# KushalChaudhari-16/Medical-Image-Denoising-Using-Diffusion

Measured on AMD Instinct MI355X. Metric: denoised images/sec, 256x256 x50 DDIM steps, higher is better.
Workload: dtype f32 (split-fp16 x3 MFMA, fp32 accumulate); 1 GPU; batch=8/GPU 256x256 grayscale, 50-iteration reverse loop (noise_steps=50, inference_steps=50), random-init 12.8M-param UNet (BASELINE.json configs[1]); batch_per_gpu=8, global_batch=8, parallelism=single, collective=none

## Files before the change

include/midd.h:

```cpp
#ifndef MIDD_H
#define MIDD_H

#include <stddef.h>
#include <stdint.h>

#ifdef __cplusplus
extern "C" {
#endif

#define MI_OK            0
#define MI_EINVAL       -1
#define MI_ESTATE       -2
#define MI_EHIP         -3
#define MI_ENOMEM       -4
#define MI_ERANGE       -5

#define MI_STATUS_NONFINITE   1
#define MI_STATUS_FP16_RANGE  2

#define MI_MAX_LEVELS    8

#define MI_VARIANT_DDIM  0
#define MI_VARIANT_CDDPM 1

#define MI_COMPUTE_F32   0
#define MI_COMPUTE_F16X3 1
#define MI_COMPUTE_F16   2
#define MI_COMPUTE_BATCH_INVARIANT 0x100

#define MI_CLAMP_EPS     1
#define MI_NO_SPLIT      2

typedef struct mi_plan mi_plan;

typedef struct mi_unet_cfg {
    int32_t in_channels;
    int32_t model_channels;
    int32_t num_levels;
    int32_t channel_mult[MI_MAX_LEVELS];
    int32_t num_res_blocks;
    int32_t num_attention_levels;
    int32_t attention_levels[MI_MAX_LEVELS];
    int32_t time_emb_dim;
    int32_t variant;
    int32_t compute_mode;
} mi_unet_cfg;

int mi_unet_plan_create(const mi_unet_cfg* cfg, mi_plan** out);

int mi_unet_load_weights(mi_plan* plan, const char* key, const float* data,
                         const int64_t* shape, int ndim);

int mi_unet_num_weights(const mi_plan* plan);
const char* mi_unet_weight_name(const mi_plan* plan, int index);

int mi_unet_finalize(mi_plan* plan, int time_rows);

size_t mi_workspace_bytes(mi_plan* plan, int B, int H, int W);

int mi_unet_forward(mi_plan* plan, const float* x, const float* condition, const int32_t* t,
                    float* eps, int B, int H, int W,
                    void* workspace, size_t workspace_bytes, void* stream);

int mi_denoise(mi_plan* plan, const float* noisy, float* x_out, int B, int H, int W,
               const int32_t* t_list, int n_iters,
               const float* beta, const float* alpha, const float* alpha_hat, int noise_steps,
               const float* step_noise, int flags,
               void* workspace, size_t workspace_bytes, void* stream);

int mi_denoise_seeded(mi_plan* plan, const float* noisy, float* x_out, int B, int H, int W,
                      const int32_t* t_list, int n_iters,
                      const float* beta, const float* alpha, const float* alpha_hat, int noise_steps,
                      uint64_t seed, int64_t sample_offset, int flags,
                      void* workspace, size_t workspace_bytes, void* stream);

int mi_denoise_slots(mi_plan* plan, const float* cond, float* x, int B, int H, int W,
                     const int32_t* t_rows, int n_rows, const int32_t* iter_base, const int64_t* sample_index,
                     const float* beta, const float* alpha, const float* alpha_hat, int noise_steps,
                     const float* step_noise, int seeded, uint64_t seed, int flags,
                     void* workspace, size_t workspace_bytes, void* stream);

int mi_denoise_slots_virtual(mi_plan* plan, const float* cond, float* x, int B, int H, int W,
                             const int32_t* t_rows, int n_rows, const int32_t* iter_base, const int64_t* sample_index,
                             const int64_t* member, const uint32_t* frame,
                             const float* beta, const float* alpha, const float* alpha_hat, int noise_steps,
                             const float* step_noise, int seeded, uint64_t seed, int flags,
                             void* workspace, size_t workspace_bytes, void* stream);

int mi_step_noise_fill(float* dst, int n_iters, int B, int C, int H, int W,
                       uint64_t seed, int64_t sample_offset, void* stream);
int mi_step_noise_fill_member(float* dst, int n_iters, int B, int C, int H, int W,
                              uint64_t seed, int64_t sample_offset, int64_t member, void* stream);

int mi_denoise_ensemble(mi_plan* plan, const float* noisy, float* mean_out, float* std_out, float* samples_out,
                        int B, int members, int H, int W,
                        const int32_t* t_list, int n_iters,
                        const float* beta, const float* alpha, const float* alpha_hat, int noise_steps,
                        uint64_t seed, int64_t sample_offset, int64_t member_offset, int pass_samples, int flags,
                        void* workspace, size_t workspace_bytes, void* stream);

size_t mi_ensemble_workspace_bytes(mi_plan* plan, int B, int members, int H, int W, int pass_samples, int samples_external);

int mi_ensemble_reduce(const float* samples, int B, int members, int64_t chw, float* mean_out, float* std_out, void* stream);

int mi_ensemble_quantiles(const float* samples, int B, int members, int64_t chw,
                          const double* q, int nq, float* out, void* stream);

size_t mi_ensemble_scores_workspace_bytes(int B, int members, int64_t chw);
int mi_ensemble_scores(const float* samples, const float* truth, int B, int members, int64_t chw,
                       const double* q, int nq,
                       double* sums, uint64_t* invalid, uint64_t* rank_hist, uint64_t* counts, float* crps_map,
                       void* workspace, size_t workspace_bytes, void* stream);

#define MI_NPS_DETREND_NONE  0
#define MI_NPS_DETREND_MEAN  1
#define MI_NPS_DETREND_PLANE 2
#define MI_NPS_EXCLUDE_AXES  1
size_t mi_noise_power_spectrum_workspace_bytes(int B, int K, int C, int H, int W, int roi, int step);
int mi_noise_power_spectrum(const float* a, const float* b, int B, int K, int C, int H, int W, int roi, int step, int detrend,
                            const float* window, double scale, int flags,
                            double* nps, double* radial, int64_t* radial_count, int64_t* rois_used, int64_t* rois_skipped,
                            void* workspace, size_t workspace_bytes, void* stream);

int mi_tile_geometry(int L, int T, int O, int* n, int* origins, int cap);

int mi_tile_extract(const float* noisy, int B, int C, int H, int W, int th, int tw, int oy, int ox, int v0, int n,
                    float* dst, void* stream);

int mi_tile_blend(const float* tiles, int B, int C, int H, int W, int th, int tw, int oy, int ox, float* out, void* stream);

int mi_denoise_tiled(mi_plan* plan, const float* noisy, float* image_out, float* tiles_out,
                     int B, int H, int W, int th, int tw, int oy, int ox,
                     const int32_t* t_list, int n_iters,
                     const float* beta, const float* alpha, const float* alpha_hat, int noise_steps,
                     int seeded, uint64_t seed, int64_t sample_offset, int pass_samples, int flags,
                     void* workspace, size_t workspace_bytes, void* stream);

size_t mi_tiled_workspace_bytes(mi_plan* plan, int B, int H, int W, int th, int tw, int oy, int ox, int pass_samples, int tiles_external);

int mi_denoise_tiled_ensemble(mi_plan* plan, const float* noisy, float* mean_out, float* std_out, float* samples_out, float* tiles_out,
                              int B, int members, int H, int W, int th, int tw, int oy, int ox,
                              const int32_t* t_list, int n_iters,
                              const float* beta, const float* alpha, const float* alpha_hat, int noise_steps,
                              uint64_t seed, int64_t sample_offset, int64_t member_offset, int pass_samples, int flags,
                              void* workspace, size_t workspace_bytes, void* stream);

size_t mi_tiled_ensemble_workspace_bytes(mi_plan* plan, int B, int members, int H, int W, int th, int tw, int oy, int ox,
                                         int pass_samples, int tiles_external);

int mi_tile_blend_reduce(const float* tiles, int B, int members, int C, int H, int W, int th, int tw, int oy, int ox,
                         float* mean_out, float* std_out, float* samples_out, void* stream);

int mi_tile_blend_quantiles(const float* tiles, int B, int members, int C, int H, int W, int th, int tw, int oy, int ox,
                            const double* q, int nq, float* out, void* stream);

int mi_dihedral_views(const float* images, int B, int C, int H, int W, const int32_t* views, int n_views,
                      int v0, int n, float* dst, void* stream);
int mi_dihedral_reduce(const float* views_out, int B, int C, int H, int W, const int32_t* views, int n_views,
                       float* mean_out, float* std_out, float* samples_out, void* stream);
int mi_dihedral_quantiles(const float* views_out, int B, int C, int H, int W, const int32_t* views, int n_views,
                          const double* q, int nq, float* out, void* stream);

int mi_denoise_self_ensemble(mi_plan* plan, const float* noisy, float* mean_out, float* std_out, float* samples_out,
                             int B, int H, int W, const int32_t* views, int n_views,
                             const int32_t* t_list, int n_iters,
                             const float* beta, const float* alpha, const float* alpha_hat, int noise_steps,
                             int seeded, uint64_t seed, int64_t sample_offset, int64_t member_offset, int pass_samples, int flags,
                             void* workspace, size_t workspace_bytes, void* stream);

size_t mi_self_ensemble_workspace_bytes(mi_plan* plan, int B, int n_views, int H, int W, int pass_samples, int samples_external);

#define MI_UPDATE_REFERENCE 0
#define MI_UPDATE_DDIM      1
typedef struct mi_update_rule {
    int32_t kind;
    double  eta;
    int32_t clip_x0;
} mi_update_rule;

int mi_ddim_coefficients(const int32_t* t_list, int n_iters, const float* alpha_hat, int noise_steps, double eta, float* out);

int mi_denoise_rule(mi_plan* plan, const float* noisy, float* x_out, int B, int H, int W,
                    const int32_t* t_list, int n_iters,
                    const float* beta, const float* alpha, const float* alpha_hat, int noise_steps,
                    const float* step_noise, int seeded, uint64_t seed, int64_t sample_offset, int flags,
                    const mi_update_rule* rule, void* workspace, size_t workspace_bytes, void* stream);

int mi_denoise_ensemble_rule(mi_plan* plan, const float* noisy, float* mean_out, float* std_out, float* samples_out,
                             int B, int members, int H, int W,
                             const int32_t* t_list, int n_iters,
                             const float* beta, const float* alpha, const float* alpha_hat, int noise_steps,
                             uint64_t seed, int64_t sample_offset, int64_t member_offset, int pass_samples, int flags,
                             const mi_update_rule* rule, void* workspace, size_t workspace_bytes, void* stream);

int mi_denoise_tiled_rule(mi_plan* plan, const float* noisy, float* image_out, float* tiles_out,
                          int B, int H, int W, int th, int tw, int oy, int ox,
                          const int32_t* t_list, int n_iters,
                          const float* beta, const float* alpha, const float* alpha_hat, int noise_steps,
                          int seeded, uint64_t seed, int64_t sample_offset, int pass_samples, int flags,
                          const mi_update_rule* rule, void* workspace, size_t workspace_bytes, void* stream);

#define MI_UPDATE_DPMPP2M   2

int mi_dpm_coefficients(const int32_t* t_list, int n_iters, const float* alpha_hat, int noise_steps, float* out);

int mi_denoise_dpm(mi_plan* plan, const float* noisy, float* x_out, float* x0_buf, int x0_slots, int B, int H, int W,
                   const int32_t* t_list, int n_iters,
                   const float* beta, const float* alpha, const float* alpha_hat, int noise_steps,
                   int flags, int clip_x0, void* workspace, size_t workspace_bytes, void* stream);

int mi_denoise_tiled_dpm(mi_plan* plan, const float* noisy, float* image_out, float* tiles_out, float* x0_hist,
                         int B, int H, int W, int th, int tw, int oy, int ox,
                         const int32_t* t_list, int n_iters,
                         const float* beta, const float* alpha, const float* alpha_hat, int noise_steps,
                         int pass_samples, int flags, int clip_x0, void* workspace, size_t workspace_bytes, void* stream);

int mi_update_row(int32_t t_before, int32_t t, int32_t t_after, const float* alpha_hat, int noise_steps, double eta, float out[8]);

int mi_tile_blend_unview_reduce(const float* tiles, int B, int C, int H, int W, int th, int tw, int oy, int ox,
                                const int32_t* views, int n_views, float* mean_out, float* std_out, float* samples_out, void* stream);
int mi_tile_blend_unview_quantiles(const float* tiles, int B, int C, int H, int W, int th, int tw, int oy, int ox,
                                   const int32_t* views, int n_views, const double* q, int nq, float* out, void* stream);

int mi_denoise_tiled_self_ensemble(mi_plan* plan, const float* noisy, float* mean_out, float* std_out, float* samples_out, float* tiles_out,
                                   int B, int H, int W, int th, int tw, int oy, int ox, const int32_t* views, int n_views,
                                   const int32_t* t_list, int n_iters,
                                   const float* beta, const float* alpha, const float* alpha_hat, int noise_steps,
                                   int seeded, uint64_t seed, int64_t sample_offset, int64_t member_offset, int pass_samples, int flags,
                                   const mi_update_rule* rule, void* workspace, size_t workspace_bytes, void* stream);

size_t mi_tiled_self_ensemble_workspace_bytes(mi_plan* plan, int B, int n_views, int H, int W, int th, int tw, int oy, int ox,
                                              int pass_samples, int tiles_external);

int mi_denoise_slots_rule(mi_plan* plan, const float* cond, float* x, int B, int H, int W,
                          const int32_t* t_rows, int n_rows, const int32_t* iter_base, const int64_t* sample_index,
                          const int64_t* member, const uint32_t* frame,
                          const int32_t* t_before, const int32_t* t_after, float* x0_hist,
                          const float* beta, const float* alpha, const float* alpha_hat, int noise_steps,
                          const float* step_noise, int seeded, uint64_t seed, int flags,
                          const mi_update_rule* rule, void* workspace, size_t workspace_bytes, void* stream);

int mi_status(const void* workspace, void* stream, int* flags);

int mi_debug_fetch(mi_plan* plan, const char* module_name, int B, int H, int W,
                   const void* workspace, float* dst, int* C, int* h, int* w, void* stream);

int mi_debug_attention_split(int N, int B, int* ksplit, int* tiles_per_split);

int mi_debug_plan_dump(mi_plan* plan, int B, int H, int W, int side_by_side, char* buf, size_t cap);

int mi_debug_conv16_geometry(int ks, int stride, int tw, int mt, int nt, int wm, int wn, int cb,
                             int* ring, int* ppw, int* apw, int* lds_bytes);
int mi_debug_conv16_geometry_planes(int ks, int stride, int tw, int mt, int nt, int wm, int wn, int cb, int planes,
                                    int* ring, int* ppw, int* apw, int* lds_bytes);
int mi_debug_conv16_steps(int Cin, int ks, int cb);

const char* mi_source_hash(void);

typedef struct mi_profile_entry {
    char   name[128];
    int64_t launches;
    double total_ms;
    double flops;
    double bytes;
} mi_profile_entry;
int mi_profile_begin(mi_plan* plan);
int mi_profile_end(mi_plan* plan, mi_profile_entry* out, int max_entries, int* n_entries);

int mi_noise_images(const float* clean, const int32_t* t, const float* alpha_hat, int noise_steps,
                    const float* eps, int seeded, uint64_t seed, int64_t sample_offset, int64_t draw,
                    const int64_t* sample_index, const int64_t* draws,
                    float* x_t, float* eps_out, int B, int C, int H, int W, void* stream);
size_t mi_loss_workspace_bytes(int B, int C, int H, int W);
int mi_loss_terms(const float* clean, const float* x_t, const float* eps, const float* eps_pred,
                  const int32_t* t, const float* alpha_hat, int noise_steps,
                  int seeded, uint64_t seed, int64_t sample_offset, int64_t draw,
                  const int64_t* sample_index, const int64_t* draws, int flags, double edge_weight,
                  double* out, float* maps, int B, int C, int H, int W,
                  void* workspace, size_t workspace_bytes, void* stream);
size_t mi_denoising_loss_workspace_bytes(mi_plan* plan, int B, int H, int W);
int mi_denoising_loss(mi_plan* plan, const float* clean, const float* cond, const int32_t* t,
                      const float* alpha_hat, int noise_steps,
                      const float* eps, int seeded, uint64_t seed, int64_t sample_offset, int64_t draw,
                      const int64_t* sample_index, const int64_t* draws, int flags, double edge_weight,
                      double* out, float* maps, int B, int H, int W,
                      void* workspace, size_t workspace_bytes, void* stream);

void mi_plan_destroy(mi_plan* plan);

size_t mi_resize_workspace_bytes(int n, int sw, int sh, int dw, int dh);
int mi_resize_bicubic_u8(const void* src_u8, int n, int sw, int sh, void* dst_u8, int dw, int dh,
                         void* workspace, size_t workspace_bytes, void* stream);
int mi_u8_to_unit_f32(const void* src_u8, void* dst_f32, size_t count, void* stream);
int mi_unit_f32_to_u8(const void* src_f32, void* dst_u8, size_t count, void* stream);
size_t mi_metrics_workspace_bytes(int n, int h);
int mi_image_metrics(const void* target_f32, const void* pred_f32, int n, int h, int w, void* out_f64,
                     void* workspace, size_t workspace_bytes, void* stream);

#define MI_PIX_U8  0
#define MI_PIX_U16 1
#define MI_PIX_F32 2
size_t mi_resize_f32_workspace_bytes(int n, int sw, int sh, int dw, int dh);
int mi_resize_bicubic_f32(const void* src, int src_type, int n, int sw, int sh,
                          void* dst, int dst_type, int dw, int dh, int clamp01,
                          void* workspace, size_t workspace_bytes, void* stream);
int mi_u16_to_unit_f32(const uint16_t* src, float* dst, size_t count, void* stream);
int mi_unit_f32_to_u16(const float* src, uint16_t* dst, size_t count, void* stream);

int mi_histogram_u16(const uint16_t* src, int n, size_t count, uint32_t* hist, void* stream);
int mi_window_levels(const uint32_t* hist, int n, double p_lo, double p_hi, int32_t* levels, void* stream);
int mi_window_u16_to_f32(const uint16_t* src, const int32_t* levels, int n, size_t count, float* dst, void* stream);
int mi_window_f32_to_u16(const float* src, const int32_t* levels, int n, size_t count, uint16_t* dst, void* stream);
int mi_resize_bicubic_f32_window(const void* src, int src_type, int n, int sw, int sh,
                                 void* dst, int dst_type, int dw, int dh, int clamp01, const int32_t* levels,
                                 void* workspace, size_t workspace_bytes, void* stream);

const char* mi_last_error(void);

const char* mi_version(void);

#ifdef __cplusplus
}
#endif
#endif
```

medical-image-denoising-using-diffusion_amd/csrc/conv_mfma_f16x3.hip:

```cpp
#include "f16x3_common.h"
#include <cstdlib>
#include <type_traits>
#ifdef MIDD_CONV_TIMING
#include <cstdio>
#include <cstring>
#include <string>
#include <vector>
#endif

namespace midd {

#ifndef MIDD_LDS_TARGET_KB
#define MIDD_LDS_TARGET_KB 52
#endif
#ifndef MIDD_RING_MAX
#define MIDD_RING_MAX 6
#endif
#ifndef MIDD_LDS_WIDE_KB
#define MIDD_LDS_WIDE_KB 78
#endif
struct Conv16Tile {
    int ks, stride, tw, mt, nt, wm, wn;
    int cbt = 0;
    int pl = 2;
    int nw = wm * wn;
    int nthreads = nw * 64;
    int th = wm * mt * 16 / tw;
    int ih = (th - 1) * stride + ks;
    int iw = (tw - 1) * stride + ks;
    int npix = ih * iw;
    int cb = cbt ? cbt : conv16_cb(ks);
    int qpp = 4 * cb;
    int nslot = npix * qpp;
    int apw = (nslot + nthreads - 1) / nthreads;
    int raw_bytes = apw * nthreads * 16;
    int plane = npix * 32;
    int img_bytes = pl * cb * plane;
    int wpieces = wn * nt * pl;
    int ppw = (wpieces + nw - 1) / nw;
    int wslice = wpieces * 1024;
    int stat_floats = nw * 2 * nt * 16;
    int add_floats = wn * nt * 16;
    static constexpr int NOMINAL_CIN = 384;
    int fixed_bytes = raw_bytes + img_bytes + (stat_floats + add_floats) * 4 + 2 * NOMINAL_CIN * 4 + 64;
    int lds_target = (stride == 2 ? 120 : (ks == 3 && cb == 2) ? MIDD_LDS_WIDE_KB : MIDD_LDS_TARGET_KB) * 1024;
    int ring_fit = (lds_target - fixed_bytes) / wslice;
    int ring = ring_fit < 2 ? 2 : (ring_fit > MIDD_RING_MAX ? MIDD_RING_MAX : ring_fit);
    int lds_nominal = fixed_bytes + ring * wslice;
    bool fits = lds_nominal <= 160 * 1024 && (ring - 2) * ppw + apw <= 60;
    constexpr int lds_bytes(int cin) const { return lds_nominal + 2 * (cin - NOMINAL_CIN) * 4; }
};

template <int KS, int STRIDE, int TW, int MT, int NT, int WM, int WN, int CBT = 0, int PL = 2>
struct Conv16Geom {
    static constexpr Conv16Tile g{KS, STRIDE, TW, MT, NT, WM, WN, CBT, PL};
    static constexpr int NW = g.nw, NTHREADS = g.nthreads, TH = g.th, IH = g.ih, IW = g.iw, CB = g.cb, QPP = g.qpp, NSLOT = g.nslot, APW = g.apw;
    static constexpr int RAW_BYTES = g.raw_bytes, PLANE = g.plane, IMG_BYTES = g.img_bytes, WPIECES = g.wpieces, PPW = g.ppw, WSLICE = g.wslice;
    static constexpr int STAT_FLOATS = g.stat_floats, ADD_FLOATS = g.add_floats, RING = g.ring;
    static_assert((WM * MT * 16) % TW == 0, "tile");
};

#ifdef MIDD_CONV_TIMING
enum { TS_WAIT, TS_ISSUE, TS_MFMA, TS_CHUNK_WAIT, TS_TRANSFORM, TS_EPILOGUE, TS_PROLOGUE, TS_FIRSTWAIT, TS_DMAWAIT, TS_RES, TS_PUBLISH, TS_TOTAL, TS_REAL, TS_WGS, TS_N };
__device__ unsigned long long g_conv_timing[64][TS_N];
__device__ __forceinline__ unsigned long long ts_stamp() {
    unsigned long long t;
    __builtin_amdgcn_sched_barrier(0);
    asm volatile("s_memtime %0\n\ts_waitcnt lgkmcnt(0)" : "=s"(t)::"memory");
    __builtin_amdgcn_sched_barrier(0);
    return t;
}
#define TS_DECL bool ts_after_epi = false; unsigned long long ts_acc[TS_N] = {}; unsigned long long ts_last = ts_stamp(); const unsigned long long ts_t0 = ts_last; const unsigned long long ts_r0 = __builtin_amdgcn_s_memrealtime();
#define TS(k) { const unsigned long long t_ = ts_stamp(); ts_acc[k] += t_ - ts_last; ts_last = t_; }
#else
#define TS_DECL
#define TS(k)
#endif

#ifndef MIDD_CONV16_WAVES_PER_SIMD
#define MIDD_CONV16_WAVES_PER_SIMD 3
#endif
#ifndef MIDD_RES_MT2_WAVES
#define MIDD_RES_MT2_WAVES 2
#endif
#define MIDD_CONV16_BOUNDS __launch_bounds__(WM * WN * 64, (WM * WN == 4 && STRIDE == 1) ? (CBT == 2 ? 2 : (RES && MT == 2) ? MIDD_RES_MT2_WAVES : MIDD_CONV16_WAVES_PER_SIMD) : 1)
#define MIDD_CONV16_KERNEL conv_mfma_f16x3_kernel
#define MIDD_CONV16_PL 2
#include "conv_mfma_f16x3_body.h"
#undef MIDD_CONV16_KERNEL
#undef MIDD_CONV16_PL
#define MIDD_CONV16_KERNEL conv_mfma_f16_kernel
#define MIDD_CONV16_PL 1
#include "conv_mfma_f16x3_body.h"
#undef MIDD_CONV16_KERNEL
#undef MIDD_CONV16_PL

#ifdef MIDD_CONV_TIMING
static std::vector<std::string> g_timing_names;
static int conv_timing_slot(int ks, int st, int tw, int mt, int nt, int wm, int wn, int oh, int cin, int cout, int B, int ring, int wgs) {
    char buf[160];
    snprintf(buf, sizeof buf, "k%d s%d tile(%d,%d,%d,%d,%d) ring%d out%d^2 %d->%d B%d wgs%d", ks, st, tw, mt, nt, wm, wn, ring, oh, cin, cout, B, wgs);
    for (size_t i = 0; i < g_timing_names.size(); ++i) if (g_timing_names[i] == buf) return (int)i;
    if (g_timing_names.size() >= 63) return 63;
    g_timing_names.push_back(buf);
    return (int)g_timing_names.size() - 1;
}
extern "C" __attribute__((visibility("default"))) void mi_debug_conv_timing_dump(void) {
    static unsigned long long h[64][TS_N];
    (void)hipDeviceSynchronize();
    (void)hipMemcpyFromSymbol(h, HIP_SYMBOL(g_conv_timing), sizeof h);
    static const char* names[] = {"barrier", "dma-issue", "frag+mfma", "chunk-wait", "transform", "epilogue", "prologue", "wait-after-epi", "dma-wait", "res-phase", "publish"};
    for (size_t i = 0; i < g_timing_names.size(); ++i) {
        const double tot = (double)h[i][TS_TOTAL], wgs = (double)h[i][TS_WGS];
        if (wgs == 0) continue;
        printf("%-70s cyc/wg %9.0f clk %.2f GHz |", g_timing_names[i].c_str(), tot / wgs, tot / (double)h[i][TS_REAL] * 0.1);
        for (int k = 0; k < 11; ++k) printf(" %s %4.1f%%", names[k], 100.0 * (double)h[i][k] / tot);
        printf("\n");
    }
    memset(h, 0, sizeof h);
    (void)hipMemcpyToSymbol(HIP_SYMBOL(g_conv_timing), h, sizeof h);
    fflush(stdout);
}
#endif
template <int KS, int STRIDE, int TW, int MT, int NT, int WM, int WN, bool RES, int CBT = 0, int PL = 2>
static hipError_t launch16(const ConvArgs& a0, hipStream_t s) {
    using G = Conv16Geom<KS, STRIDE, TW, MT, NT, WM, WN, CBT, PL>;
    ConvArgs a = a0;
    a.tiles_x = (a.OW + TW - 1) / TW;
    a.tiles_y = (a.OH + G::TH - 1) / G::TH;
    const int ny = a.Cout / (WN * NT * 16);
    a.wgs_per_img = conv16_wgs_per_img(a.tiles_x * a.tiles_y, a.B, ny, a.persist_wgs);
    dim3 grid(a.B * a.wgs_per_img, ny);
#ifdef MIDD_CONV_TIMING
    a.dbg_slot = conv_timing_slot(KS, STRIDE, TW, MT * 10 + G::CB, NT, WM, WN, a.OH, a.C0 + a.C1, a.Cout, a.B, G::RING, (int)grid.x * (int)grid.y);
#endif
    if constexpr (G::g.fits) {
        const int lds_bytes = G::g.lds_bytes(a.C0 + a.C1);
        if (lds_bytes > 160 * 1024) return hipErrorInvalidValue;
        {
            static int raised[MIDD_MAX_DEVICES] = {};
            hipError_t e = ensure_dynamic_lds(PL == 2 ? reinterpret_cast<const void*>(&conv_mfma_f16x3_kernel<KS, STRIDE, TW, MT, NT, WM, WN, RES, CBT>)
                                                      : reinterpret_cast<const void*>(&conv_mfma_f16_kernel<KS, STRIDE, TW, MT, NT, WM, WN, RES, CBT>), lds_bytes, raised);
            if (e != hipSuccess) return e;
        }
        if ((double)a.H * a.W * 64.0 >= 4294967296.0) return hipErrorInvalidValue;
        if constexpr (PL == 2) hipLaunchKernelGGL((conv_mfma_f16x3_kernel<KS, STRIDE, TW, MT, NT, WM, WN, RES, CBT>), grid, dim3(G::NTHREADS), lds_bytes, s, a);
        else hipLaunchKernelGGL((conv_mfma_f16_kernel<KS, STRIDE, TW, MT, NT, WM, WN, RES, CBT>), grid, dim3(G::NTHREADS), lds_bytes, s, a);
        return hipGetLastError();
    } else {
        return hipErrorInvalidValue;
    }
}

int conv16_wgs_per_img(int tiles, int B, int ny, int target) {
    const int target_wgs = target ? target : 768;
    int per_img = target_wgs / (B * ny);
    if (per_img < 1) per_img = 1;
    if (per_img > tiles) per_img = tiles;
    const int tiles_per_wg = (tiles + per_img - 1) / per_img;
    return (tiles + tiles_per_wg - 1) / tiles_per_wg;
}

#define MIDD_CONV16_TILES(X)                  \
                        \
    X(16, 2, 3, 4, 1) X(16, 1, 3, 4, 1) X(8, 1, 3, 2, 1) \
    X(16, 2, 3, 2, 2) X(16, 1, 3, 2, 2) X(8, 1, 3, 1, 2) \
    X(16, 2, 3, 1, 3) X(8, 1, 3, 1, 3)                   \
    X(16, 2, 3, 1, 4) X(8, 2, 3, 1, 4) X(8, 1, 3, 1, 4)  \
    X(16, 2, 2, 4, 1) X(8, 1, 2, 2, 1)                   \
    X(16, 2, 2, 2, 2) X(8, 1, 2, 1, 2)                   \
    X(16, 2, 1, 4, 1) X(8, 1, 1, 2, 1)

struct Tile16 { int tw, mt, nt, wm, wn; };
static const Tile16 kTiles16[] = {
#define X(tw, mt, nt, wm, wn) {tw, mt, nt, wm, wn},
    MIDD_CONV16_TILES(X)
#undef X
};

#define X(tw, mt, nt, wm, wn)                                                                                     \
    static_assert(Conv16Geom<3, 1, tw, mt, nt, wm, wn>::RING == Conv16Tile{3, 1, tw, mt, nt, wm, wn}.ring &&         \
                  Conv16Geom<3, 2, tw, mt, nt, wm, wn>::APW == Conv16Tile{3, 2, tw, mt, nt, wm, wn}.apw &&           \
                  Conv16Geom<1, 1, tw, mt, nt, wm, wn>::WSLICE == Conv16Tile{1, 1, tw, mt, nt, wm, wn}.wslice, "Conv16Geom");
MIDD_CONV16_TILES(X)
#undef X
#define X(tw, mt, nt, wm, wn)                                                                                                 \
    static_assert(Conv16Geom<3, 1, tw, mt, nt, wm, wn, 0, 1>::RING == Conv16Tile{3, 1, tw, mt, nt, wm, wn, 0, 1}.ring &&         \
                  Conv16Geom<3, 2, tw, mt, nt, wm, wn, 0, 1>::APW == Conv16Tile{3, 2, tw, mt, nt, wm, wn, 0, 1}.apw &&           \
                  Conv16Geom<1, 1, tw, mt, nt, wm, wn, 0, 1>::WSLICE * 2 == Conv16Tile{1, 1, tw, mt, nt, wm, wn}.wslice, "Conv16Geom, one plane");
MIDD_CONV16_TILES(X)
#undef X

static bool wide16_tile(const ConvTile& t) { return t.ks == 3 && t.stride == 1 && t.tw == 16 && t.nt == 3 && t.wm == 4 && t.wn == 1; }
#ifndef MIDD_WIDE_MAX_WGS
#define MIDD_WIDE_MAX_WGS 512
#endif
bool conv16_pick_tile(int Cin, int Cout, int B, int OH, int OW, int ks, int stride, ConvTile* t, bool allow_wide, int planes) {
    if (Cout % 16) return false;
    if (!((ks == 3 && (stride == 1 || stride == 2)) || (ks == 1 && stride == 1))) return false;
    if (ks == 1 && conv1x1_pick_tile(Cin, Cout, B, OH, OW, t)) { t->pl = planes; return true; }
    const int nt = (Cout % 48 == 0) ? 3 : (Cout % 32 == 0) ? 2 : 1;
    const Tile16* best = nullptr;
    long best_score = -(1L << 60), best_wgs = 0;
    constexpr long min_wgs = 192;
    for (const Tile16& d : kTiles16) {
        if (d.nt != nt) continue;
        const int nn_d = Cout / (16 * d.nt);
        if (nn_d % d.wn) continue;
        if (!Conv16Tile{ks, stride, d.tw, d.mt, d.nt, d.wm, d.wn, 0, planes}.fits) continue;
        const int bm = d.wm * d.mt * 16, th = bm / d.tw;
        const long tiles = (long)((OW + d.tw - 1) / d.tw) * ((OH + th - 1) / th);
        const long wgs = (long)B * tiles * (nn_d / d.wn);
        const long covered = tiles * d.tw * th;
        const bool wasteful = covered * 4 > (long)OH * OW * 5;
        const long share = (long)bm * 8 + d.wn;
        const long score = (wgs >= min_wgs ? 1000000 : wgs * (1000000 / min_wgs)) + share - (wasteful ? 500000 : 0);
        if (score > best_score) { best_score = score; best = &d; best_wgs = wgs; }
    }
    if (!best) return false;
    *t = ConvTile{ks, stride, best->tw, best->mt, best->nt, best->wm, best->wn, 0, planes};
    if (allow_wide && wide16_tile(*t) && Cin >= 32 &&
        best_wgs <= MIDD_WIDE_MAX_WGS && Conv16Tile{ks, stride, best->tw, best->mt, best->nt, best->wm, best->wn, 2, planes}.fits)
        t->cb = 2;
    return true;
}

bool conv16_launch_info(int Cin, int Cout, int B, int OH, int OW, const ConvTile& t, int persist_wgs, ConvLaunchInfo* o) {
    if (t.ks == 1 && t.tw == 0) return conv1x1_launch_info(Cin, Cout, B, OH, OW, t, persist_wgs, ATT_NONE, o);
    bool listed = false;
    if (t.cb == 2 ? wide16_tile(t) : ((t.ks == 3 && (t.stride == 1 || t.stride == 2)) || (t.ks == 1 && t.stride == 1)))
        for (const Tile16& d : kTiles16) listed = listed || (d.tw == t.tw && d.mt == t.mt && d.nt == t.nt && d.wm == t.wm && d.wn == t.wn);
    if (!listed) return false;
    if (t.pl != 1 && t.pl != 2) return false;
    const Conv16Tile g{t.ks, t.stride, t.tw, t.mt, t.nt, t.wm, t.wn, t.cb == 2 ? 2 : 0, t.pl};
    o->tiles_x = (OW + t.tw - 1) / t.tw; o->tiles_y = (OH + g.th - 1) / g.th;
    o->grid_y = Cout / (t.wn * t.nt * 16);
    o->wgs_per_img = conv16_wgs_per_img(o->tiles_x * o->tiles_y, B, o->grid_y, persist_wgs);
    o->grid_x = B * o->wgs_per_img;
    o->ring = g.ring; o->ppw = g.ppw; o->apw = g.apw; o->lds_bytes = g.lds_bytes(Cin);
    return true;
}

template <int PL>
static hipError_t conv16_dispatch(const ConvArgs& a, const ConvTile& t, hipStream_t s) {
    if (t.cb == 2) {
        if (!wide16_tile(t)) return hipErrorInvalidValue;
        if (t.mt == 2) return a.res_steps > 0 ? launch16<3, 1, 16, 2, 3, 4, 1, true, 2, PL>(a, s) : launch16<3, 1, 16, 2, 3, 4, 1, false, 2, PL>(a, s);
        if (t.mt == 1) return a.res_steps > 0 ? launch16<3, 1, 16, 1, 3, 4, 1, true, 2, PL>(a, s) : launch16<3, 1, 16, 1, 3, 4, 1, false, 2, PL>(a, s);
        return hipErrorInvalidValue;
    }
#define X(tw_, mt_, nt_, wm_, wn_)                                                            \
    if (t.tw == tw_ && t.mt == mt_ && t.nt == nt_ && t.wm == wm_ && t.wn == wn_) {           \
        if (t.ks == 3 && t.stride == 1 && a.res_steps > 0) return launch16<3, 1, tw_, mt_, nt_, wm_, wn_, true, 0, PL>(a, s); \
        if (t.ks == 3 && t.stride == 1) return launch16<3, 1, tw_, mt_, nt_, wm_, wn_, false, 0, PL>(a, s); \
        if (t.ks == 3 && t.stride == 2) return launch16<3, 2, tw_, mt_, nt_, wm_, wn_, false, 0, PL>(a, s); \
        if (t.ks == 1 && t.stride == 1) return launch16<1, 1, tw_, mt_, nt_, wm_, wn_, false, 0, PL>(a, s); \
    }
    MIDD_CONV16_TILES(X)
#undef X
    return hipErrorInvalidValue;
}

hipError_t conv16_launch(const ConvArgs& a, const ConvTile& t, hipStream_t s) {
    if (t.ks == 1 && t.tw == 0) return conv1x1_launch(a, t, s);
    if (t.pl == 2) return conv16_dispatch<2>(a, t, s);
    if (t.pl == 1) return conv16_dispatch<1>(a, t, s);
    return hipErrorInvalidValue;
}

}
```

medical-image-denoising-using-diffusion_amd/csrc/conv_mfma_f16x3_body.h:

```cpp
#if !defined(MIDD_CONV16_KERNEL) || !defined(MIDD_CONV16_PL)
#error "include from conv_mfma_f16x3.hip with MIDD_CONV16_KERNEL and MIDD_CONV16_PL defined"
#endif

template <int KS, int STRIDE, int TW, int MT, int NT, int WM, int WN, bool RES, int CBT>
__global__ MIDD_CONV16_BOUNDS void MIDD_CONV16_KERNEL(const ConvArgs a) {
    constexpr int PL = MIDD_CONV16_PL;
    static_assert(PL == 1 || PL == 2, "planes");
    using G = Conv16Geom<KS, STRIDE, TW, MT, NT, WM, WN, CBT, PL>;
    constexpr int NW = G::NW, NTHREADS = G::NTHREADS, TH = G::TH, IW = G::IW;
    constexpr int PAD = (KS == 3) ? 1 : 0;
    constexpr int NSLOT = G::NSLOT, APW = G::APW, PLANE = G::PLANE;
    constexpr int TAPS = KS * KS;
    constexpr int HSTEPS = (TAPS + 1) / 2;
    constexpr int PPW = G::PPW, WSLICE = G::WSLICE, RING = G::RING;

    extern __shared__ __attribute__((aligned(16))) char lds[];
    char* const raw = lds;
    char* const img = lds + G::RAW_BYTES;
    char* const wring = img + G::IMG_BYTES;
    float* const stat_lds = reinterpret_cast<float*>(wring + RING * WSLICE);
    float* const add_lds = stat_lds + G::STAT_FLOATS;
    float* const gnp = add_lds + G::ADD_FLOATS;

    const int tid = threadIdx.x;
    const int lane = tid & 63;
    const int wave = __builtin_amdgcn_readfirstlane(tid >> 6);
    const int wn = wave % WN;
    const int wm = wave / WN;
    const int p16 = lane & 15;
    const int kq = lane >> 4;

    const int tiles_per_img = a.tiles_x * a.tiles_y;
    const int b = blockIdx.x / a.wgs_per_img;
    int trem = blockIdx.x - b * a.wgs_per_img;
    int oy0 = (trem / a.tiles_x) * TH, ox0 = (trem % a.tiles_x) * TW;

    const int Cin = a.C0 + a.C1;
    const int nblk = Cin >> 4;
    constexpr int CB = G::CB, QPP = G::QPP;
    const int nchunks = (nblk + CB - 1) / CB;
    const int ntiles_total = a.Cout >> 4;
    const int ntile_wg = blockIdx.y * (WN * NT);
    const int res_steps = RES ? a.res_steps : 0;
    const int total_steps = conv16_num_steps(Cin, TAPS, G::CB) + res_steps;

    constexpr int WTILE = PL * 1024;
    const char* const wbase = reinterpret_cast<const char*>(a.wpack) + (size_t)ntile_wg * WTILE;
    const size_t wstep_bytes = (size_t)ntiles_total * WTILE;
    const int lane16 = lane * 16;
    int wr_step = 0, wr_slot = 0;
    const char* wr_src = wbase;
#ifdef MIDD_DMA_CHECK
    constexpr unsigned SENT_W = 0x7FFF7FFFu;
    constexpr unsigned SENT_A = 0x7FC0DEADu;
    unsigned dma_bad = 0;
    auto sent4 = [](unsigned v) { typedef unsigned u32x4_ __attribute__((ext_vector_type(4))); return __builtin_bit_cast(f32x4, (u32x4_){v, v, v, v}); };
    auto has_sent = [](const auto& q, unsigned v) {
        typedef unsigned u32x4_ __attribute__((ext_vector_type(4)));
        const u32x4_ u = __builtin_bit_cast(u32x4_, q);
        return (unsigned)((u[0] == v) | (u[1] == v) | (u[2] == v) | (u[3] == v));
    };
#endif
    auto issue_w = [&]() {
        char* slot = wring + wr_slot * WSLICE;
#ifdef MIDD_DMA_CHECK
#pragma unroll
        for (int i = 0; i < PPW; ++i) {
            int piece = (WM == 1) ? wave * PPW + i : wave + i * NW;
            if (piece >= G::WPIECES) piece -= G::WPIECES;
            if constexpr (PL == 1) piece %= G::WPIECES;
            lds_store_raw(slot + piece * 1024 + lane16, sent4(SENT_W));
        }
        asm volatile("s_waitcnt lgkmcnt(0)" ::: "memory");
#endif
#pragma unroll
        for (int i = 0; i < PPW; ++i) {
            int piece = (WM == 1) ? wave * PPW + i : wave + i * NW;
            if (piece >= G::WPIECES) piece -= G::WPIECES;
            if constexpr (PL == 1) piece %= G::WPIECES;
            dma16(wr_src + piece * 1024 + lane16, slot + piece * 1024);
        }
        ++wr_step; wr_src += wstep_bytes;
        if (wr_step == total_steps) { wr_step = 0; wr_src = wbase; }
        wr_slot = (wr_slot + 1 == RING) ? 0 : wr_slot + 1;
    };

    const int q8 = tid % QPP;
    const int sblk = q8 >> 2;
    int g_off[APW];
    bool tile_pad = true;
    auto set_tile = [&](int t) {
        const int iy0 = (t / a.tiles_x) * TH * STRIDE - PAD, ix0 = (t % a.tiles_x) * TW * STRIDE - PAD;
        tile_pad = iy0 < 0 || ix0 < 0 || iy0 + G::IH > a.H || ix0 + IW > a.W;
        int tid_ = tid;
        asm volatile("" : "+v"(tid_));
#pragma unroll
        for (int s = 0; s < APW; ++s) {
            const int slot = tid_ + s * NTHREADS;
            int off = -2;
            if (slot < NSLOT) {
                const int pix = slot / QPP;
                const int iy = pix / IW, ix = pix - iy * IW;
                const int gy = iy0 + iy, gx = ix0 + ix;
                off = (gy >= 0 && gy < a.H && gx >= 0 && gx < a.W) ? gy * a.W + gx : -1;
            }
            g_off[s] = off;
        }
    };
    set_tile(trem);
    auto issue_a = [&](int c) {
        const int blk = min(CB * c + sblk, nblk - 1);
        const float* src; int bsrc, nb;
        if ((blk << 4) < a.C0) { src = a.src0; bsrc = blk; nb = a.C0 >> 4; }
        else                   { src = a.src1; bsrc = blk - (a.C0 >> 4); nb = a.C1 >> 4; }
        const char* base = reinterpret_cast<const char*>(src) + ((size_t)(b * nb + bsrc) * (size_t)(a.H * a.W)) * 64 + (q8 & 3) * 16;
#ifdef MIDD_DMA_CHECK
#pragma unroll
        for (int s = 0; s < APW; ++s) lds_store_raw(raw + (wave + s * NW) * 1024 + lane16, sent4(SENT_A));
        asm volatile("s_waitcnt lgkmcnt(0)" ::: "memory");
#endif
#pragma unroll
        for (int s = 0; s < APW; ++s) {
            const unsigned byte_off = (unsigned)max(g_off[s], 0) * 64u;
            dma16(base + byte_off, raw + (wave + s * NW) * 1024);
        }
    };
    float rscale = RAW_PRESCALE;
    auto transform = [&](int c) {
        const int blk = CB * c + sblk;
        if (blk >= nblk) return;
        const int ch = (blk << 4) + (q8 & 3) * 4;
        f32x4 rq[APW];
#pragma unroll
        for (int s = 0; s < APW; ++s) rq[s] = *reinterpret_cast<const f32x4*>(raw + (tid + s * NTHREADS) * 16);
#ifdef MIDD_DMA_CHECK
#pragma unroll
        for (int s = 0; s < APW; ++s) dma_bad |= has_sent(rq[s], SENT_A);
#endif
        f32x4 sc = {rscale, rscale, rscale, rscale}, sh = {0.f, 0.f, 0.f, 0.f};
        if (a.prologue != PRO_RAW) {
            sc = *reinterpret_cast<const f32x4*>(gnp + ch);
            sh = *reinterpret_cast<const f32x4*>(gnp + Cin + ch);
        }
        char* base = img + sblk * PL * PLANE + (q8 & 3) * 8;
        typedef unsigned u32x2 __attribute__((ext_vector_type(2)));
        if (c == 0 && tile_pad) {
#pragma unroll
            for (int s = 0; s < APW; ++s) {
                const int slot = tid + s * NTHREADS;
                if (g_off[s] == -1) {
                    *reinterpret_cast<u32x2*>(base + (slot / QPP) * 32) = (u32x2){0u, 0u};
                    if constexpr (PL == 2) *reinterpret_cast<u32x2*>(base + PLANE + (slot / QPP) * 32) = (u32x2){0u, 0u};
                }
            }
        }
#pragma unroll
        for (int s = 0; s < APW; ++s) {
            const int slot = tid + s * NTHREADS;
            float v[4];
#pragma unroll
            for (int e = 0; e < 4; ++e) v[e] = __builtin_fmaf(rq[s][e], sc[e], sh[e]);
#if defined(C16_ABL) && C16_ABL == 4
            if (false) {
#else
            if (a.prologue == PRO_GN_SILU) {
#endif
#pragma unroll
                for (int e = 0; e < 4; ++e) {
                    const float d = __builtin_fmaf(__builtin_amdgcn_exp2f(v[e]), 1.0f / ACT_PRESCALE, 1.0f / ACT_PRESCALE);
                    v[e] = v[e] * __builtin_amdgcn_rcpf(d);
                }
            }
            unsigned h01, h23, l01, l23;
            planes_pair<PL>(v[0], v[1], h01, l01);
            planes_pair<PL>(v[2], v[3], h23, l23);
            if (g_off[s] >= 0) {
                const int pix = slot / QPP;
                *reinterpret_cast<u32x2*>(base + pix * 32) = (u32x2){h01, h23};
                if constexpr (PL == 2) *reinterpret_cast<u32x2*>(base + PLANE + pix * 32) = (u32x2){l01, l23};
            }
        }
    };

    int frag_base[MT];
#pragma unroll
    for (int mt = 0; mt < MT; ++mt) {
        const int pp = (wm * MT + mt) * 16 + p16;
        const int py = pp / TW, px = pp - py * TW;
        frag_base[mt] = ((py * STRIDE) * IW + px * STRIDE) * 32 + (kq & 1) * 16;
    }
    int frag_full[MT];
#pragma unroll
    for (int mt = 0; mt < MT; ++mt) frag_full[mt] = frag_base[mt] + (kq >> 1) * PL * PLANE;
    const int wfrag_off = (wn * NT) * WTILE + lane * 16;

    f32x4 acc[MT][NT];
#pragma unroll
    for (int mt = 0; mt < MT; ++mt)
#pragma unroll
        for (int nt = 0; nt < NT; ++nt) acc[mt][nt] = (f32x4){0.f, 0.f, 0.f, 0.f};

    constexpr int D = RING - 1;
    constexpr bool PAIR = conv16_pair_walk(TAPS, CB);
    static_assert(D <= 5, "the chunk-end wait has one arm per after = 1 .. 4 below D (MIDD_RING_MAX 6)");
    constexpr auto cmin = [](int x, int y) { return x < y ? x : y; };
    const int ntile0 = ntile_wg + wn * NT;
    TS_DECL
    issue_a(0);
#pragma unroll
    for (int i = 0; i < D; ++i) issue_w();
#if !(defined(C16_ABL) && C16_ABL == 6)
    if (a.prologue == PRO_GN || a.prologue == PRO_GN_SILU)
        gn_prologue_lds(a.gn_tot0, a.C0, a.gn_bs0, a.gn_tot1, a.C1, a.gn_bs1, a.stat_rep, a.gn_gamma, a.gn_beta, a.gn_eps, a.gn_inv_n, b,
                        (a.prologue == PRO_GN_SILU) ? SILU_ARG_FACTOR : ACT_PRESCALE, gnp, tid, NTHREADS, a.status);
#endif
    stat_word* const raw_acc = reinterpret_cast<stat_word*>(gnp);
    if (a.prologue == PRO_RAW && a.gn_tot0 != nullptr && wave == 0)
        raw_sumsq_lds(a.gn_tot0, a.C0, a.gn_bs0, a.gn_tot1, a.C1, a.gn_bs1, a.stat_rep, b, raw_acc, lane);
    stat_word* const res_acc = reinterpret_cast<stat_word*>(gnp + 2 * Cin);
    if (res_steps > 0 && a.res_tot0 != nullptr && wave == NW - 1)
        raw_sumsq_lds(a.res_tot0, a.res_C0, a.res_bs0, a.res_tot1, a.res_C1, a.res_bs1, a.stat_rep, b, res_acc, lane);
    {
        const int trow = (a.temb != nullptr) ? a.trow[b] : 0;
        for (int i = tid; i < G::ADD_FLOATS; i += NTHREADS) {
            const int co = ntile_wg * 16 + i;
            add_lds[i] = a.bias[co] + (a.temb != nullptr ? a.temb[(size_t)trow * a.temb_stride + co] : 0.f);
        }
    }
    wait_vm_and_barrier<0>();
    float oscale = a.out_scale;
    if (a.prologue == PRO_RAW) {
        rscale = a.raw_scale_fixed;
        if (a.gn_tot0 != nullptr) {
            bool bad;
            const int ex = __builtin_amdgcn_readfirstlane(raw_prescale_exp(raw_acc, &bad));
            rscale = pow2f(ex);
            if (bad && tid == 0 && a.status != nullptr) atomicOr(a.status, (int)STATUS_NONFINITE);
        }
        oscale = a.out_scale / rscale;
    }
    float res_in = 1.0f, res_rescale = 1.0f;
    if (res_steps > 0) {
        if (a.res_tot0 != nullptr) {
            bool bad;
            res_in = pow2f(__builtin_amdgcn_readfirstlane(raw_prescale_exp(res_acc, &bad)));
            if (bad && tid == 0 && a.status != nullptr) atomicOr(a.status, (int)STATUS_NONFINITE);
        }
        res_rescale = a.out_scale * res_in / a.res_scale;
        oscale = a.res_scale / res_in;
    }
    transform(0);
    if constexpr (WM == 1) {
        asm volatile("s_waitcnt lgkmcnt(0)" ::: "memory");
        __builtin_amdgcn_s_barrier();
        asm volatile("" ::: "memory");
    }

    TS(TS_PROLOGUE)
    int frag_next[MT], frag_wrap[MT];
#pragma unroll
    for (int mt = 0; mt < MT; ++mt) {
        frag_next[mt] = frag_base[mt] + (kq >> 1) * 32;
        frag_wrap[mt] = frag_base[mt] + (kq >> 1) * ((IW - KS + 1) * 32);
    }
    int rd_slot = 0;
    half8 xh[MT], xl[MT];
    auto load_x = [&](const int (&xo)[MT], int off) {
#pragma unroll
        for (int mt = 0; mt < MT; ++mt) {
            xh[mt] = *reinterpret_cast<const half8*>(img + xo[mt] + off);
            if constexpr (PL == 2) xl[mt] = *reinterpret_cast<const half8*>(img + xo[mt] + off + PLANE);
        }
    };
    auto tap_off = [](int t) { return ((t / KS) * IW + (t % KS)) * 32; };
    auto kill_x = [&]() {
        if constexpr (PAIR) {
#pragma unroll
            for (int mt = 0; mt < MT; ++mt) {
                asm volatile("" : "=v"(xh[mt]));
                if constexpr (PL == 2) asm volatile("" : "=v"(xl[mt]));
            }
        }
    };
    auto load_stash = [&]() {
        constexpr int T8 = (((TAPS - 1) / KS) * IW + (TAPS - 1) % KS) * 32;
        if constexpr (MT == 2) {
            const int so = (kq >> 1) ? frag_base[1] : frag_base[0];
            xh[0] = *reinterpret_cast<const half8*>(img + so + T8);
            if constexpr (PL == 2) xl[0] = *reinterpret_cast<const half8*>(img + so + T8 + PLANE);
        } else {
            load_x(frag_base, T8);
        }
    };
    auto unpack_stash = [&]() {
        if constexpr (MT == 2) {
            typedef unsigned u32x4_ __attribute__((ext_vector_type(4)));
            auto unpack = [](half8& lo, half8& hi) {
                u32x4_ a = __builtin_bit_cast(u32x4_, lo), b = __builtin_bit_cast(u32x4_, hi);
#pragma unroll
                for (int r = 0; r < 4; ++r) {
                    const auto sw = __builtin_amdgcn_permlane32_swap(a[r], b[r], false, false);
                    a[r] = sw[0]; b[r] = sw[1];
                }
                lo = __builtin_bit_cast(half8, a); hi = __builtin_bit_cast(half8, b);
            };
            unpack(xh[0], xh[1]);
            if constexpr (PL == 2) unpack(xl[0], xl[1]);
        }
    };
    auto mfma_step = [&]() {
        const char* wslot = wring + rd_slot * WSLICE + wfrag_off;
        rd_slot = (rd_slot + 1 == RING) ? 0 : rd_slot + 1;
        half8 wh[NT], wl[NT];
#pragma unroll
        for (int nt = 0; nt < NT; ++nt) {
            wh[nt] = *reinterpret_cast<const half8*>(wslot + nt * WTILE);
            if constexpr (PL == 2) wl[nt] = *reinterpret_cast<const half8*>(wslot + nt * WTILE + 1024);
        }
#ifdef MIDD_DMA_CHECK
#pragma unroll
        for (int nt = 0; nt < NT; ++nt) {
            dma_bad |= has_sent(wh[nt], SENT_W);
            if constexpr (PL == 2) dma_bad |= has_sent(wl[nt], SENT_W);
        }
#endif
#pragma unroll
        for (int mt = 0; mt < MT; ++mt)
#pragma unroll
            for (int nt = 0; nt < NT; ++nt)
                acc[mt][nt] = __builtin_amdgcn_mfma_f32_16x16x32_f16(wh[nt], xh[mt], acc[mt][nt], 0, 0, 0);
#if !(defined(C16_ABL) && C16_ABL == 8)
        if constexpr (PL == 2) {
#pragma unroll
            for (int mt = 0; mt < MT; ++mt)
#pragma unroll
                for (int nt = 0; nt < NT; ++nt)
                    acc[mt][nt] = __builtin_amdgcn_mfma_f32_16x16x32_f16(wh[nt], xl[mt], acc[mt][nt], 0, 0, 0);
#pragma unroll
            for (int mt = 0; mt < MT; ++mt)
#pragma unroll
                for (int nt = 0; nt < NT; ++nt)
                    acc[mt][nt] = __builtin_amdgcn_mfma_f32_16x16x32_f16(wl[nt], xh[mt], acc[mt][nt], 0, 0, 0);
        }
#endif
    };

    auto k_step = [&](auto with_a, auto merge, bool first, bool first_with_more, int next_chunk, const int (&xo)[MT], int xoff) {
        constexpr bool WITH_A = decltype(with_a)::value;
        constexpr bool MERGE = decltype(merge)::value;
        auto load_frag = [&]() {
            if constexpr (MERGE) { unpack_stash(); if (kq >= 2) load_x(xo, xoff); }
            else load_x(xo, xoff);
        };
#ifdef MIDD_DMA_CHECK_BREAK
        constexpr int N = D * PPW + (WITH_A ? APW : 0);
#else
        constexpr int N = (D - 1) * PPW + (WITH_A ? APW : 0);
#endif
        const bool early = (WM == 1) || !first;
        if (early) {
            if constexpr (PL == 1) __builtin_amdgcn_sched_barrier(0);
            load_frag();
            asm volatile("s_waitcnt vmcnt(%0) lgkmcnt(%1)" ::"n"(N), "n"(PL * MT) : "memory");
        } else {
            asm volatile("s_waitcnt vmcnt(%0) lgkmcnt(0)" ::"n"(N) : "memory");
        }
        TS(TS_DMAWAIT)
        if constexpr (WM != 1) {
            __builtin_amdgcn_s_barrier();
            asm volatile("" ::: "memory");
        }
#ifdef MIDD_CONV_TIMING
        if (ts_after_epi) { TS(TS_FIRSTWAIT) ts_after_epi = false; } else { TS(TS_WAIT) }
#endif
        if (!early) load_frag();
        issue_w();
        if (first_with_more) issue_a(next_chunk);
        TS(TS_ISSUE)
        mfma_step();
        TS(TS_MFMA)
    };

    constexpr int RL = 2 * MT;
    constexpr int RG = (MT == 1) ? 2 : 1;
    static_assert((D - 1) * PPW + APW <= 63 && D * PPW <= 63 && (D - 1) * PPW + RG * RL <= 63 && RG * PPW <= 63, "vmcnt immediate beyond 63");
    auto res_load = [&](int r, f32x4 (&dst)[MT][2]) {
        const int rc = a.res_C0 + a.res_C1;
        int ch = r * 32 + kq * 8;
        if (ch >= rc) ch = rc - 8;
        const float* src; int nb, cc;
        if (ch < a.res_C0) { src = a.res_src0; nb = a.res_C0 >> 4; cc = ch; } else { src = a.res_src1; nb = a.res_C1 >> 4; cc = ch - a.res_C0; }
        src += ((size_t)(b * nb + (cc >> 4)) * (size_t)(a.OH * a.OW)) * 16 + (cc & 15);
#pragma unroll
        for (int mt = 0; mt < MT; ++mt) {
            const int pp = (wm * MT + mt) * 16 + p16;
            const int py = pp / TW, px = pp - py * TW;
            const int oy = min(oy0 + py, a.OH - 1), ox = min(ox0 + px, a.OW - 1);
            const float* q = src + (size_t)(oy * a.OW + ox) * 16;
#ifdef MIDD_DMA_CHECK
            dst[mt][0] = sent4(SENT_A); dst[mt][1] = sent4(SENT_A);
            asm volatile("global_load_dwordx4 %0, %1, off" : "+v"(dst[mt][0]) : "v"(q) : "memory");
            asm volatile("global_load_dwordx4 %0, %1, off offset:16" : "+v"(dst[mt][1]) : "v"(q) : "memory");
#else
            asm volatile("global_load_dwordx4 %0, %1, off" : "=&v"(dst[mt][0]) : "v"(q) : "memory");
            asm volatile("global_load_dwordx4 %0, %1, off offset:16" : "=&v"(dst[mt][1]) : "v"(q) : "memory");
#endif
        }
    };
    auto res_wait = [&](f32x4 (&r)[RG][MT][2], auto n_t) {
        constexpr int N = decltype(n_t)::value;
        if constexpr (MT == 2) asm volatile("s_waitcnt vmcnt(%4) ; asm-loads-landed" : "+v"(r[0][0][0]), "+v"(r[0][0][1]), "+v"(r[0][1][0]), "+v"(r[0][1][1]) : "n"(N) : "memory");
        else asm volatile("s_waitcnt vmcnt(%4) ; asm-loads-landed" : "+v"(r[0][0][0]), "+v"(r[0][0][1]), "+v"(r[1][0][0]), "+v"(r[1][0][1]) : "n"(N) : "memory");
    };
    static_assert((MT == 2 && RG == 1) || (MT == 1 && RG == 2), "res_wait names exactly the registers of one group");
    half8 rxh[RG][MT], rxl[RG][MT];
    auto res_split = [&](int r, f32x4 (&ra)[MT][2], half8 (&oh)[MT], half8 (&ol)[MT]) {
        const bool valid = r * 32 + kq * 8 < a.res_C0 + a.res_C1;
#pragma unroll
        for (int mt = 0; mt < MT; ++mt) {
#ifdef MIDD_DMA_CHECK
            dma_bad |= has_sent(ra[mt][0], SENT_A) | has_sent(ra[mt][1], SENT_A);
#endif
            f32x4 v0 = ra[mt][0] * res_in, v1 = ra[mt][1] * res_in;
            if (!valid) { v0 = (f32x4){0.f, 0.f, 0.f, 0.f}; v1 = v0; }
            typedef unsigned u32x4 __attribute__((ext_vector_type(4)));
            u32x4 hw, lw;
            unsigned hh, ll;
            planes_pair<PL>(v0[0], v0[1], hh, ll); hw[0] = hh; lw[0] = ll;
            planes_pair<PL>(v0[2], v0[3], hh, ll); hw[1] = hh; lw[1] = ll;
            planes_pair<PL>(v1[0], v1[1], hh, ll); hw[2] = hh; lw[2] = ll;
            planes_pair<PL>(v1[2], v1[3], hh, ll); hw[3] = hh; lw[3] = ll;
            oh[mt] = __builtin_bit_cast(half8, hw);
            ol[mt] = __builtin_bit_cast(half8, lw);
        }
    };
    auto res_mfma = [&](auto in_flight, half8 (&oh)[MT], half8 (&ol)[MT]) {
        constexpr int N = (D - 1) * PPW + (decltype(in_flight)::value ? RG * RL : 0);
        asm volatile("s_waitcnt vmcnt(%0) lgkmcnt(0)" ::"n"(N) : "memory");
        if constexpr (WM != 1) {
            __builtin_amdgcn_s_barrier();
            asm volatile("" ::: "memory");
        }
        issue_w();
#pragma unroll
        for (int mt = 0; mt < MT; ++mt) { xh[mt] = oh[mt]; xl[mt] = ol[mt]; }
        mfma_step();
    };
    auto res_phase = [&]() {
        if constexpr (RES) {
            if (res_steps == 0) return;
#pragma unroll
            for (int mt = 0; mt < MT; ++mt)
#pragma unroll
                for (int nt = 0; nt < NT; ++nt) acc[mt][nt] *= res_rescale;
            {
                f32x4 ra[RG][MT][2];
#pragma unroll
                for (int i = 0; i < RG; ++i) res_load(min(i, res_steps - 1), ra[i]);
                res_wait(ra, std::integral_constant<int, 0>{});
#pragma unroll
                for (int i = 0; i < RG; ++i) res_split(i, ra[i], rxh[i], rxl[i]);
            }
            for (int r = 0; r < res_steps; r += RG) {
                const bool more = r + RG < res_steps;
                if (more) {
                    f32x4 ra[RG][MT][2];
#pragma unroll
                    for (int i = 0; i < RG; ++i) res_load(min(r + RG + i, res_steps - 1), ra[i]);
                    res_mfma(std::true_type{}, rxh[0], rxl[0]);
                    if constexpr (RG == 2) {
#ifdef MIDD_DMA_CHECK_OLD_RES
                        if (r + 1 < res_steps) res_mfma(std::true_type{}, rxh[1], rxl[1]);
#else
                        if (r + 1 < res_steps) res_mfma(std::integral_constant<bool, (1 < D)>{}, rxh[1], rxl[1]);
#endif
                    }
                    res_wait(ra, std::integral_constant<int, RG * PPW>{});
#pragma unroll
                    for (int i = 0; i < RG; ++i) res_split(r + RG + i, ra[i], rxh[i], rxl[i]);
                } else {
#pragma unroll
                    for (int i = 0; i < RG; ++i)
                        if (r + i < res_steps) res_mfma(std::false_type{}, rxh[i], rxl[i]);
                }
            }
            kill_x();
        }
    };

    f32x4 ssum[NT], ssq[NT];
#pragma unroll
    for (int nt = 0; nt < NT; ++nt) { ssum[nt] = (f32x4){0.f, 0.f, 0.f, 0.f}; ssq[nt] = (f32x4){0.f, 0.f, 0.f, 0.f}; }
    auto epilogue = [&]() {
        f32x4 rres[MT][NT];
        size_t obase[MT];
        bool rowok[MT];
        const size_t ohw = (size_t)a.OH * a.OW;
#pragma unroll
        for (int mt = 0; mt < MT; ++mt) {
            const int pp = (wm * MT + mt) * 16 + p16;
            const int py = pp / TW, px = pp - py * TW;
            const int oy = oy0 + py, ox = ox0 + px;
            rowok[mt] = oy < a.OH && ox < a.OW;
            obase[mt] = (((size_t)b * (a.Cout >> 4) + ntile0) * ohw + (size_t)(min(oy, a.OH - 1) * a.OW + min(ox, a.OW - 1))) * 16 + kq * 4;
        }
        if (a.resid != nullptr) {
#pragma unroll
            for (int mt = 0; mt < MT; ++mt)
#pragma unroll
                for (int nt = 0; nt < NT; ++nt) {
#ifdef MIDD_DMA_CHECK
                    rres[mt][nt] = sent4(SENT_A);
                    asm volatile("global_load_dwordx4 %0, %1, off" : "+v"(rres[mt][nt]) : "v"(a.resid + obase[mt] + nt * ohw * 16) : "memory");
#else
                    asm volatile("global_load_dwordx4 %0, %1, off" : "=&v"(rres[mt][nt]) : "v"(a.resid + obase[mt] + nt * ohw * 16) : "memory");
#endif
                }
            if constexpr (MT == 2 && NT == 3) asm volatile("s_waitcnt vmcnt(0) ; asm-loads-landed" : "+v"(rres[0][0]), "+v"(rres[0][1]), "+v"(rres[0][2]), "+v"(rres[1][0]), "+v"(rres[1][1]), "+v"(rres[1][2]) :: "memory");
            else if constexpr (MT == 2 && NT == 2) asm volatile("s_waitcnt vmcnt(0) ; asm-loads-landed" : "+v"(rres[0][0]), "+v"(rres[0][1]), "+v"(rres[1][0]), "+v"(rres[1][1]) :: "memory");
            else if constexpr (MT == 2 && NT == 1) asm volatile("s_waitcnt vmcnt(0) ; asm-loads-landed" : "+v"(rres[0][0]), "+v"(rres[1][0]) :: "memory");
            else if constexpr (MT == 1 && NT == 3) asm volatile("s_waitcnt vmcnt(0) ; asm-loads-landed" : "+v"(rres[0][0]), "+v"(rres[0][1]), "+v"(rres[0][2]) :: "memory");
            else if constexpr (MT == 1 && NT == 2) asm volatile("s_waitcnt vmcnt(0) ; asm-loads-landed" : "+v"(rres[0][0]), "+v"(rres[0][1]) :: "memory");
            else asm volatile("s_waitcnt vmcnt(0) ; asm-loads-landed" : "+v"(rres[0][0]) :: "memory");
        }
#pragma unroll
        for (int mt = 0; mt < MT; ++mt) {
            if (rowok[mt]) {
#pragma unroll
                for (int nt = 0; nt < NT; ++nt) {
                    const f32x4 add = *reinterpret_cast<const f32x4*>(add_lds + (wn * NT + nt) * 16 + kq * 4);
                    f32x4 v = acc[mt][nt] * oscale + add;
#ifdef MIDD_DMA_CHECK
                    if (a.resid != nullptr) dma_bad |= has_sent(rres[mt][nt], SENT_A);
#endif
                    if (a.resid != nullptr) v += rres[mt][nt];
                    *reinterpret_cast<f32x4*>(a.out + obase[mt] + nt * ohw * 16) = v;
#if !(defined(C16_ABL) && C16_ABL == 1)
                    ssum[nt] += v; ssq[nt] += v * v;
#endif
                }
            }
#pragma unroll
            for (int nt = 0; nt < NT; ++nt) acc[mt][nt] = (f32x4){0.f, 0.f, 0.f, 0.f};
        }
    };
    auto publish_stats = [&]() {
        if (a.stat_tot == nullptr) return;
#if defined(C16_ABL) && (C16_ABL == 1 || C16_ABL == 9)
        return;
#endif
        float* const my_stat = stat_lds + wave * (2 * NT * 16) + kq * 4;
#pragma unroll
        for (int nt = 0; nt < NT; ++nt) {
#pragma unroll
            for (int e = 0; e < 4; ++e) { ssum[nt][e] = row16_sum(ssum[nt][e]); ssq[nt][e] = row16_sum(ssq[nt][e]); }
            if (p16 == 0) {
                lds_store_raw(my_stat + nt * 16, ssum[nt]);
                lds_store_raw(my_stat + NT * 16 + nt * 16, ssq[nt]);
            }
        }
        constexpr int ROWF = 2 * NT * 16;
        constexpr int NCOL = WN * NT * 16;
        auto fold = [&](int i) {
            const int which = i / NCOL, col = i - which * NCOL;
            const int wn_i = col / (NT * 16), c = col - wn_i * (NT * 16);
            float t = 0.f;
#pragma unroll
            for (int m = 0; m < WM; ++m) t += stat_lds[(m * WN + wn_i) * ROWF + which * (NT * 16) + c];
            return t;
        };
        static_assert(G::RAW_BYTES + G::IMG_BYTES + RING * WSLICE >= (NCOL + 2) * STAT_WORDS * 8, "block accumulators in the staging buffers (raw, image, ring: contiguous, idle here)");
        if constexpr (G::RAW_BYTES < (NCOL + 2) * STAT_WORDS * 8) {
            asm volatile("s_waitcnt lgkmcnt(0)" ::: "memory");
            __builtin_amdgcn_s_barrier();
            asm volatile("" ::: "memory");
        }
        stat_publish(a.stat_tot, b, a.Cout, a.stat_bs, a.stat_rep, (blockIdx.x - b * a.wgs_per_img) % a.stat_rep, ntile_wg * 16, NCOL,
                     fold, reinterpret_cast<stat_word*>(raw), tid, NTHREADS);
    };

    for (;;) {
        const int next_tile = trem + a.wgs_per_img;
        const bool has_next_tile = next_tile < tiles_per_img;
        for (int c = 0; c < nchunks; ++c) {
            const bool more_in_tile = (c + 1 < nchunks);
            const bool more = more_in_tile || has_next_tile;
            const int next_chunk = more_in_tile ? c + 1 : 0;
            const bool full = (CB == 2) && (2 * c + 1 < nblk);
            if (!more_in_tile && has_next_tile) set_tile(next_tile);
            const int walk = !PAIR ? 0 : (c & 1) ? 2 : more_in_tile ? 1 : 0;
            auto run_chunk = [&](auto more_t, auto walk_t) {
                constexpr bool MORE = decltype(more_t)::value;
                constexpr int WALK = decltype(walk_t)::value;
                if constexpr (WALK != 0) {
#pragma unroll
                    for (int j = 0; j < (WALK == 1 ? HSTEPS - 1 : HSTEPS); ++j) {
                        const int t0 = (WALK == 1) ? 2 * j : 2 * j - 1;
                        if (j == 0 && WALK == 2)         k_step(std::false_type{}, std::true_type{}, true, MORE, next_chunk, frag_base, tap_off(0));
                        else if (MORE && j >= 1 && j <= D) k_step(std::true_type{}, std::false_type{}, false, false, next_chunk, t0 % KS == KS - 1 ? frag_wrap : frag_next, tap_off(t0));
                        else                             k_step(std::false_type{}, std::false_type{}, j == 0, MORE && j == 0, next_chunk, t0 % KS == KS - 1 ? frag_wrap : frag_next, tap_off(t0));
                    }
                    if constexpr (WALK == 1) {
                        load_stash();
                    }
                    if constexpr (WALK == 2) kill_x();
                    return;
                }
                if (full) {
#pragma unroll
                    for (int tap = 0; tap < TAPS; ++tap) {
                        const int dy = tap / KS, dx = tap - dy * KS;
                        const int xoff = (dy * IW + dx) * 32;
                        if (MORE && tap >= 1 && tap <= D) k_step(std::true_type{}, std::false_type{}, false, false, next_chunk, frag_full, xoff);
                        else                              k_step(std::false_type{}, std::false_type{}, tap == 0, MORE && tap == 0, next_chunk, frag_full, xoff);
                    }
                } else {
#pragma unroll
                    for (int hs = 0; hs < HSTEPS; ++hs) {
                        const int t0 = 2 * hs;
                        const int (&xb)[MT] = (t0 + 1 >= TAPS) ? frag_base : (t0 % KS == KS - 1) ? frag_wrap : frag_next;
                        if (MORE && hs >= 1 && hs <= D) k_step(std::true_type{}, std::false_type{}, false, false, next_chunk, xb, tap_off(t0));
                        else                            k_step(std::false_type{}, std::false_type{}, hs == 0, MORE && hs == 0, next_chunk, xb, tap_off(t0));
                    }
                }
                kill_x();
            };
            if (more) {
                if constexpr (PAIR) {
                    if (walk == 1)      run_chunk(std::true_type{}, std::integral_constant<int, 1>{});
                    else if (walk == 2) run_chunk(std::true_type{}, std::integral_constant<int, 2>{});
                    else                run_chunk(std::true_type{}, std::integral_constant<int, 0>{});
                } else {
                    run_chunk(std::true_type{}, std::integral_constant<int, 0>{});
                }
                if (!more_in_tile) { res_phase(); TS(TS_RES) }
                const int after = (full ? TAPS : walk == 1 ? HSTEPS - 1 : HSTEPS) - 1 + (more_in_tile ? 0 : res_steps);
                if (after >= D) wait_vm_and_barrier<D * PPW>();
                else if (after == 4) wait_vm_and_barrier<cmin(4, D) * PPW>();
                else if (after == 3) wait_vm_and_barrier<cmin(3, D) * PPW>();
                else if (after == 2) wait_vm_and_barrier<cmin(2, D) * PPW>();
                else if (after == 1) wait_vm_and_barrier<cmin(1, D) * PPW>();
                else wait_vm_and_barrier<0>();
                TS(TS_CHUNK_WAIT)
                if (!more_in_tile) {
                    epilogue();
                    trem = next_tile;
                    oy0 = (trem / a.tiles_x) * TH; ox0 = (trem % a.tiles_x) * TW;
                    TS(TS_EPILOGUE)
#ifdef MIDD_CONV_TIMING
                    ts_after_epi = true;
#endif
                }
#if !(defined(C16_ABL) && C16_ABL == 5)
                transform(next_chunk);
#endif
                TS(TS_TRANSFORM)
                if constexpr (WM == 1) {
                    asm volatile("s_waitcnt lgkmcnt(0)" ::: "memory");
                    __builtin_amdgcn_s_barrier();
                    asm volatile("" ::: "memory");
                }
            } else {
                if constexpr (PAIR) {
                    if (walk == 2) run_chunk(std::false_type{}, std::integral_constant<int, 2>{});
                    else           run_chunk(std::false_type{}, std::integral_constant<int, 0>{});
                } else {
                    run_chunk(std::false_type{}, std::integral_constant<int, 0>{});
                }
                res_phase();
                TS(TS_RES)
            }
        }
        if (!has_next_tile) break;
    }
    asm volatile("s_waitcnt vmcnt(0)" ::: "memory");
    TS(TS_CHUNK_WAIT)
    epilogue();
    TS(TS_EPILOGUE)
    publish_stats();
#ifdef MIDD_DMA_CHECK
    if (dma_bad && a.status != nullptr) atomicOr(a.status, (int)STATUS_DMA_EARLY);
#endif
    TS(TS_PUBLISH)
#ifdef MIDD_CONV_TIMING
    if (tid == 0) {
        ts_acc[TS_TOTAL] = ts_last - ts_t0;
        ts_acc[TS_REAL] = __builtin_amdgcn_s_memrealtime() - ts_r0;
        ts_acc[TS_WGS] = 1;
        for (int k = 0; k < TS_N; ++k) atomicAdd(&g_conv_timing[a.dbg_slot][k], ts_acc[k]);
    }
#endif
}
```

medical-image-denoising-using-diffusion_amd/csrc/midd_abi.hip:

```cpp
#include "midd_host.h"

using namespace midd;

static thread_local char g_err[512] = "";

int midd::fail(int code, const char* fmt, ...) {
    va_list ap;
    va_start(ap, fmt);
    vsnprintf(g_err, sizeof(g_err), fmt, ap);
    va_end(ap);
    return code;
}

extern "C" size_t mi_resize_workspace_bytes(int n, int sw, int sh, int dw, int dh) {
    if (n < 1 || sw < 1 || sh < 1 || dw < 1 || dh < 1) return 0;
    return resize_workspace_bytes(n, sw, sh, dw, dh);
}
extern "C" int mi_resize_bicubic_u8(const void* src, int n, int sw, int sh, void* dst, int dw, int dh,
                                    void* workspace, size_t workspace_bytes, void* stream) {
    if (!src || !dst || !workspace) return fail(MI_EINVAL, "null argument");
    if (n < 1 || sw < 1 || sh < 1 || dw < 1 || dh < 1) return fail(MI_EINVAL, "image sizes must be positive");
    if (reinterpret_cast<uintptr_t>(workspace) & 255) return fail(MI_EINVAL, "workspace must be 256-byte aligned");
    if (workspace_bytes < resize_workspace_bytes(n, sw, sh, dw, dh))
        return fail(MI_EINVAL, "workspace too small: %zu < %zu", workspace_bytes, resize_workspace_bytes(n, sw, sh, dw, dh));
    HIPCHK(resize_bicubic_u8_launch(static_cast<const unsigned char*>(src), n, sw, sh, static_cast<unsigned char*>(dst), dw, dh,
                                    workspace, static_cast<hipStream_t>(stream)));
    return MI_OK;
}
extern "C" int mi_u8_to_unit_f32(const void* src, void* dst, size_t count, void* stream) {
    if (!src || !dst) return fail(MI_EINVAL, "null argument");
    HIPCHK(u8_to_unit_launch(static_cast<const unsigned char*>(src), static_cast<float*>(dst), count, static_cast<hipStream_t>(stream)));
    return MI_OK;
}
extern "C" int mi_unit_f32_to_u8(const void* src, void* dst, size_t count, void* stream) {
    if (!src || !dst) return fail(MI_EINVAL, "null argument");
    HIPCHK(unit_to_u8_launch(static_cast<const float*>(src), static_cast<unsigned char*>(dst), count, static_cast<hipStream_t>(stream)));
    return MI_OK;
}
static bool resize_f32_fits(int n, int sw, int sh, int dw, int dh) {
    const long long lim = 1LL << 31;
    return (long long)n * sh * sw < lim && (long long)n * sh * dw < lim && (long long)n * dh * dw < lim;
}
extern "C" size_t mi_resize_f32_workspace_bytes(int n, int sw, int sh, int dw, int dh) {
    if (n < 1 || sw < 1 || sh < 1 || dw < 1 || dh < 1 || !resize_f32_fits(n, sw, sh, dw, dh)) return 0;
    return resize_f32_workspace_bytes(n, sw, sh, dw, dh);
}
static int resize_f32_args(const void* src, int src_type, int n, int sw, int sh, void* dst, int dst_type, int dw, int dh,
                           void* workspace, size_t workspace_bytes) {
    if (!src || !dst || !workspace) return fail(MI_EINVAL, "null argument");
    if (n < 1 || sw < 1 || sh < 1 || dw < 1 || dh < 1) return fail(MI_EINVAL, "image sizes must be positive");
    if (src_type != MI_PIX_U8 && src_type != MI_PIX_U16 && src_type != MI_PIX_F32)
        return fail(MI_EINVAL, "unknown source element type %d (MI_PIX_U8, MI_PIX_U16 or MI_PIX_F32)", src_type);
    if (dst_type == MI_PIX_U8)
        return fail(MI_EINVAL, "destination element type MI_PIX_U8: the 8-bit destination is mi_resize_bicubic_u8 (fixed-point arithmetic)");
    if (dst_type != MI_PIX_U16 && dst_type != MI_PIX_F32)
        return fail(MI_EINVAL, "unknown destination element type %d (MI_PIX_U16 or MI_PIX_F32)", dst_type);
    if (!resize_f32_fits(n, sw, sh, dw, dh)) return fail(MI_EINVAL, "too many pixels: n * height * width must stay below 2^31");
    if (reinterpret_cast<uintptr_t>(workspace) & 255) return fail(MI_EINVAL, "workspace must be 256-byte aligned");
    if (workspace_bytes < resize_f32_workspace_bytes(n, sw, sh, dw, dh))
        return fail(MI_EINVAL, "workspace too small: %zu < %zu", workspace_bytes, resize_f32_workspace_bytes(n, sw, sh, dw, dh));
    return MI_OK;
}
extern "C" int mi_resize_bicubic_f32(const void* src, int src_type, int n, int sw, int sh, void* dst, int dst_type, int dw, int dh,
                                     int clamp01, void* workspace, size_t workspace_bytes, void* stream) {
    if (const int rc = resize_f32_args(src, src_type, n, sw, sh, dst, dst_type, dw, dh, workspace, workspace_bytes)) return rc;
    HIPCHK(resize_bicubic_f32_launch(src, src_type, n, sw, sh, dst, dst_type, dw, dh, clamp01, workspace, static_cast<hipStream_t>(stream)));
    return MI_OK;
}
extern "C" int mi_u16_to_unit_f32(const uint16_t* src, float* dst, size_t count, void* stream) {
    if (!src || !dst) return fail(MI_EINVAL, "null argument");
    if (count >= ((size_t)1 << 40)) return fail(MI_EINVAL, "count must stay below 2^40");
    HIPCHK(u16_to_unit_launch(src, dst, count, static_cast<hipStream_t>(stream)));
    return MI_OK;
}
extern "C" int mi_unit_f32_to_u16(const float* src, uint16_t* dst, size_t count, void* stream) {
    if (!src || !dst) return fail(MI_EINVAL, "null argument");
    if (count >= ((size_t)1 << 40)) return fail(MI_EINVAL, "count must stay below 2^40");
    HIPCHK(unit_to_u16_launch(src, dst, count, static_cast<hipStream_t>(stream)));
    return MI_OK;
}
static int window_counts(int n, size_t count) {
    if (n < 1 || n > 65535) return fail(MI_EINVAL, "n must be in [1, 65535], got %d", n);
    if (count < 1 || count > 0xffffffffull) return fail(MI_EINVAL, "count must be in [1, 2^32), got %zu", count);
    return MI_OK;
}
extern "C" int mi_histogram_u16(const uint16_t* src, int n, size_t count, uint32_t* hist, void* stream) {
    if (!src || !hist) return fail(MI_EINVAL, "null argument");
    if (const int rc = window_counts(n, count)) return rc;
    if (reinterpret_cast<uintptr_t>(src) & 1) return fail(MI_EINVAL, "src must be 2-byte aligned");
    if (reinterpret_cast<uintptr_t>(hist) & 15) return fail(MI_EINVAL, "hist must be 16-byte aligned");
    HIPCHK(histogram_u16_launch(src, n, count, hist, static_cast<hipStream_t>(stream)));
    return MI_OK;
}
extern "C" int mi_window_levels(const uint32_t* hist, int n, double p_lo, double p_hi, int32_t* levels, void* stream) {
    if (!hist || !levels) return fail(MI_EINVAL, "null argument");
    if (n < 1 || n > 65535) return fail(MI_EINVAL, "n must be in [1, 65535], got %d", n);
    if (!std::isfinite(p_lo) || !std::isfinite(p_hi)) return fail(MI_EINVAL, "percentiles must be finite");
    if (!(0.0 <= p_lo && p_lo < p_hi && p_hi <= 100.0))
        return fail(MI_EINVAL, "percentiles must satisfy 0 <= p_lo < p_hi <= 100, got (%g, %g)", p_lo, p_hi);
    if (reinterpret_cast<uintptr_t>(hist) & 15) return fail(MI_EINVAL, "hist must be 16-byte aligned");
    HIPCHK(window_levels_launch(hist, n, p_lo, p_hi, levels, static_cast<hipStream_t>(stream)));
    return MI_OK;
}
extern "C" int mi_window_u16_to_f32(const uint16_t* src, const int32_t* levels, int n, size_t count, float* dst, void* stream) {
    if (!src || !levels || !dst) return fail(MI_EINVAL, "null argument");
    if (const int rc = window_counts(n, count)) return rc;
    HIPCHK(window_u16_to_f32_launch(src, levels, n, count, dst, static_cast<hipStream_t>(stream)));
    return MI_OK;
}
extern "C" int mi_window_f32_to_u16(const float* src, const int32_t* levels, int n, size_t count, uint16_t* dst, void* stream) {
    if (!src || !levels || !dst) return fail(MI_EINVAL, "null argument");
    if (const int rc = window_counts(n, count)) return rc;
    HIPCHK(window_f32_to_u16_launch(src, levels, n, count, dst, static_cast<hipStream_t>(stream)));
    return MI_OK;
}
extern "C" int mi_resize_bicubic_f32_window(const void* src, int src_type, int n, int sw, int sh, void* dst, int dst_type, int dw, int dh,
                                            int clamp01, const int32_t* levels, void* workspace, size_t workspace_bytes, void* stream) {
    if (!levels) return mi_resize_bicubic_f32(src, src_type, n, sw, sh, dst, dst_type, dw, dh, clamp01, workspace, workspace_bytes, stream);
    if (const int rc = resize_f32_args(src, src_type, n, sw, sh, dst, dst_type, dw, dh, workspace, workspace_bytes)) return rc;
    if (n > 65535) return fail(MI_EINVAL, "n must be in [1, 65535] under a window, got %d", n);
    if (src_type != MI_PIX_U16 && dst_type != MI_PIX_U16)
        return fail(MI_EINVAL, "levels given, but neither side is MI_PIX_U16: the window acts on 16-bit elements only");
    HIPCHK(resize_bicubic_f32_window_launch(src, src_type, n, sw, sh, dst, dst_type, dw, dh, clamp01, levels, workspace,
                                            static_cast<hipStream_t>(stream)));
    return MI_OK;
}
extern "C" size_t mi_metrics_workspace_bytes(int n, int h) { return (n < 1 || h < 1) ? 0 : metrics_workspace_bytes(n, h); }
extern "C" int mi_image_metrics(const void* target, const void* pred, int n, int h, int w, void* out,
                                void* workspace, size_t workspace_bytes, void* stream) {
    if (!target || !pred || !out || !workspace) return fail(MI_EINVAL, "null argument");
    if (n < 1 || h < 7 || w < 7) return fail(MI_EINVAL, "images must be at least 7x7 (SSIM window), got %dx%d", h, w);
    if (workspace_bytes < metrics_workspace_bytes(n, h)) return fail(MI_EINVAL, "workspace too small");
    HIPCHK(metrics_launch(static_cast<const float*>(target), static_cast<const float*>(pred), n, h, w, static_cast<double*>(out),
                          workspace, static_cast<hipStream_t>(stream)));
    return MI_OK;
}

extern "C" const char* mi_last_error(void) { return g_err; }
extern "C" const char* mi_version(void) { return "midd 0.4 gfx950 (fp32 MFMA | split-fp16 x3 MFMA | fp16 MFMA; GroupNorm statistics in the producers; device pre/post-processing)"; }

#ifndef MIDD_SOURCE_HASH
#define MIDD_SOURCE_HASH "unknown"
#endif
extern "C" const char* mi_source_hash(void) { return MIDD_SOURCE_HASH; }

extern "C" int mi_debug_attention_split(int N, int B, int* ksplit, int* tiles_per_split) {
    if (N < 1 || B < 1 || !ksplit || !tiles_per_split) return fail(MI_EINVAL, "N and B must be positive");
    attention16_split(N, ATTN_HEADS_ABI, B, ksplit, tiles_per_split);
    return MI_OK;
}

extern "C" int mi_unet_plan_create(const mi_unet_cfg* cfg, mi_plan** out) {
    if (!cfg || !out) return fail(MI_EINVAL, "null argument");
    if (cfg->num_levels < 1 || cfg->num_levels > MI_MAX_LEVELS) return fail(MI_EINVAL, "num_levels out of range");
    if (cfg->num_attention_levels < 0 || cfg->num_attention_levels > MI_MAX_LEVELS) return fail(MI_EINVAL, "num_attention_levels out of range");
    if (cfg->model_channels < 16 || cfg->model_channels % 16) return fail(MI_EINVAL, "model_channels must be a multiple of 16 (MFMA K-chunk), got %d", cfg->model_channels);
    if (cfg->in_channels < 1 || cfg->in_channels > 4) return fail(MI_EINVAL, "in_channels must be 1..4");
    if (cfg->num_res_blocks < 1) return fail(MI_EINVAL, "num_res_blocks must be >= 1");
    if (cfg->time_emb_dim < 1) return fail(MI_EINVAL, "time_emb_dim must be >= 1");
    if (cfg->variant != MI_VARIANT_DDIM && cfg->variant != MI_VARIANT_CDDPM) return fail(MI_EINVAL, "unknown variant %d", cfg->variant);
    const int arith = cfg->compute_mode & ~MI_COMPUTE_BATCH_INVARIANT;
    if (arith != MI_COMPUTE_F32 && arith != MI_COMPUTE_F16X3 && arith != MI_COMPUTE_F16) return fail(MI_EINVAL, "unknown compute_mode %d", cfg->compute_mode);
    for (int i = 0; i < cfg->num_levels; ++i)
        if (cfg->channel_mult[i] < 1) return fail(MI_EINVAL, "channel_mult[%d] must be >= 1", i);
    {
        const int ic = cfg->in_channels, mc = cfg->model_channels;
        const long long fc = (long long)mc * cfg->channel_mult[0];
        if (mc > (1 << 20)) return fail(MI_EINVAL, "model_channels %d is out of range", mc);
        if (!(ic == 1 && in_conv1_width(mc)) && in_conv_lds_bytes(ic, mc) > POINTWISE_LDS_LIMIT)
            return fail(MI_EINVAL, "in_channels %d with model_channels %d: in_conv needs %zu bytes of LDS, the limit is %zu bytes",
                        ic, mc, in_conv_lds_bytes(ic, mc), POINTWISE_LDS_LIMIT);
        if (fc > (1 << 20) || out_conv_lds_bytes(ic, (int)fc) > POINTWISE_LDS_LIMIT)
            return fail(MI_EINVAL, "in_channels %d with %lld channels into out_conv (model_channels * channel_mult[0]): out_conv needs more than the "
                        "limit of %zu bytes of LDS (%zu bytes of tile, %d bytes per channel)",
                        ic, fc, POINTWISE_LDS_LIMIT, out_conv_static_lds_bytes(), (int)out_conv_dynamic_lds_bytes(ic, 1));
    }
    for (int i = 0; i < cfg->num_attention_levels; ++i) {
        const int lv = cfg->attention_levels[i];
        if (lv >= 0 && lv < cfg->num_levels) {
            const int c = cfg->model_channels * cfg->channel_mult[lv];
            if (c % ATTN_HEADS_ABI || !attention_supported(c / 2))
                return fail(MI_EINVAL, "attention head_dim %d unsupported (32/64/96/128)", c / 2);
        }
    }
    std::unique_ptr<mi_plan> p(new mi_plan());
    p->cfg = *cfg;
    p->cfg.compute_mode = arith;
    p->batch_invariant = (cfg->compute_mode & MI_COMPUTE_BATCH_INVARIANT) != 0;
    int rc = build_topology(p.get());
    if (rc) return rc;
    *out = p.release();
    return MI_OK;
}

extern "C" int mi_unet_num_weights(const mi_plan* plan) { return plan ? (int)plan->expected.size() : 0; }
extern "C" const char* mi_unet_weight_name(const mi_plan* plan, int i) {
    if (!plan || i < 0 || i >= (int)plan->expected.size()) return nullptr;
    return plan->expected[i].c_str();
}

extern "C" int mi_unet_load_weights(mi_plan* plan, const char* key, const float* data, const int64_t* shape, int ndim) {
    if (!plan || !key || !data || !shape) return fail(MI_EINVAL, "null argument");
    auto it = plan->expected_shape.find(key);
    if (it == plan->expected_shape.end()) return fail(MI_EINVAL, "unexpected key in state_dict: \"%s\"", key);
    const std::vector<int64_t>& want = it->second;
    bool ok = (int)want.size() == ndim;
    for (int i = 0; ok && i < ndim; ++i) ok = want[i] == shape[i];
    if (!ok) return fail(MI_EINVAL, "size mismatch for %s", key);
    size_t n = 1;
    for (int i = 0; i < ndim; ++i) n *= (size_t)shape[i];
    std::lock_guard<std::mutex> lk(plan->mu);
    HostWeight& hw = plan->host[key];
    hw.shape.assign(shape, shape + ndim);
    hw.data.assign(data, data + n);
    hw.loaded = true;
    plan->finalized = false;
    return MI_OK;
}

extern "C" int mi_status(const void* workspace, void* stream, int* flags) {
    if (!workspace || !flags) return fail(MI_EINVAL, "null argument");
    int host = 0;
    HIPCHK(hipMemcpyAsync(&host, workspace, sizeof(int), hipMemcpyDeviceToHost, (hipStream_t)stream));
    HIPCHK(hipStreamSynchronize((hipStream_t)stream));
    *flags = host;
    if (host & ~(MI_STATUS_NONFINITE | MI_STATUS_FP16_RANGE))
        return fail(MI_ERANGE, "status word 0x%x (bit 4: a -DMIDD_DMA_CHECK build saw an operand that had not landed when its counted wait returned)", host);
    if (host & MI_STATUS_FP16_RANGE)
        return fail(MI_ERANGE, "an attention operand exceeds the split-fp16 range (|q|, |k| or |v| >= 4094, or not finite): use compute=\"f32\"%s",
                    (host & MI_STATUS_NONFINITE) ? "; non-finite values reached later statistics" : "");
    if (host & MI_STATUS_NONFINITE) return fail(MI_ERANGE, "non-finite activations (NaN / Inf) reached a GroupNorm statistic or a raw operand");
    return MI_OK;
}

extern "C" int mi_debug_conv16_geometry(int ks, int stride, int tw, int mt, int nt, int wm, int wn, int cb, int* ring, int* ppw, int* apw, int* lds_bytes) {
    if (!ring || !ppw || !apw || !lds_bytes) return fail(MI_EINVAL, "null argument");
    ConvTile t{ks, stride, tw, mt, nt, wm, wn, cb};
    ConvLaunchInfo li{};
    if (!conv16_launch_info(384, 16 * nt * wn, 1, 64, 64, t, 0, &li)) return fail(MI_EINVAL, "tile (%d,%d,%d,%d,%d) ks %d stride %d cb %d is not instantiated", tw, mt, nt, wm, wn, ks, stride, cb);
    *ring = li.ring; *ppw = li.ppw; *apw = li.apw; *lds_bytes = li.lds_bytes;
    return MI_OK;
}
extern "C" int mi_debug_conv16_geometry_planes(int ks, int stride, int tw, int mt, int nt, int wm, int wn, int cb, int planes,
                                               int* ring, int* ppw, int* apw, int* lds_bytes) {
    if (!ring || !ppw || !apw || !lds_bytes) return fail(MI_EINVAL, "null argument");
    if (planes != 1 && planes != 2) return fail(MI_EINVAL, "planes must be 1 (f16) or 2 (f16x3), got %d", planes);
    ConvTile t{ks, stride, tw, mt, nt, wm, wn, cb, planes};
    ConvLaunchInfo li{};
    if (!conv16_launch_info(384, 16 * nt * wn, 1, 64, 64, t, 0, &li)) return fail(MI_EINVAL, "tile (%d,%d,%d,%d,%d) ks %d stride %d cb %d is not instantiated", tw, mt, nt, wm, wn, ks, stride, cb);
    *ring = li.ring; *ppw = li.ppw; *apw = li.apw; *lds_bytes = li.lds_bytes;
    return MI_OK;
}
extern "C" int mi_debug_conv16_steps(int Cin, int ks, int cb) {
    if (Cin < 16 || Cin % 16) return fail(MI_EINVAL, "Cin %d: a positive multiple of 16", Cin);
    if (ks != 1 && ks != 3) return fail(MI_EINVAL, "ks %d: 1 or 3", ks);
    if (cb < 0 || cb > 2 || (ks == 1 && cb == 1)) return fail(MI_EINVAL, "cb %d: 0 (default), 1 (3x3) or 2", cb);
    return conv16_num_steps(Cin, ks * ks, cb);
}
extern "C" int mi_debug_plan_dump(mi_plan* plan, int B, int H, int W, int side_by_side, char* buf, size_t cap) {
    if (!plan) return fail(MI_EINVAL, "null plan");
    std::string text;
    int rc = dump_program(plan, B, H, W, side_by_side != 0, &text);
    if (rc) return rc;
    if (buf && cap) { snprintf(buf, cap, "%s", text.c_str()); }
    return (int)text.size();
}

extern "C" void mi_plan_destroy(mi_plan* plan) {
    if (!plan) return;
    for (auto& sp : plan->spans) { (void)hipEventDestroy(sp.a); (void)hipEventDestroy(sp.b); }
    for (hipEvent_t ev : plan->event_pool) (void)hipEventDestroy(ev);
    if (plan->sev_fork) (void)hipEventDestroy(plan->sev_fork);
    for (int i = 0; i < mi_plan::MAX_PARTS; ++i) {
        if (plan->sev_phase[i]) (void)hipEventDestroy(plan->sev_phase[i]);
        if (plan->sev_join[i]) (void)hipEventDestroy(plan->sev_join[i]);
        if (plan->sstream[i]) (void)hipStreamDestroy(plan->sstream[i]);
    }
    if (plan->wdev) (void)hipFree(plan->wdev);
    if (plan->ttab) (void)hipFree(plan->ttab);
    delete plan;
}
```

medical-image-denoising-using-diffusion_amd/csrc/midd_exec.hip:

```cpp
#include "midd_sampler.h"

using namespace midd;

int midd::run_program(mi_plan* p, Program* g, const StepIO& io, char* ws, int* status, hipStream_t s, hipEvent_t mid_event, int mid_div) {
    const float* wd = p->wdev;
    auto F = [&](size_t off) { return reinterpret_cast<float*>(ws + off); };
    const int B = g->B;
    auto T = [&](size_t off) { return reinterpret_cast<stat_word*>(ws + off); };
    if (hipMemsetAsync(ws + g->stats_off, 0, g->stats_bytes, s) != hipSuccess) return fail(MI_EHIP, "clearing the statistics arena failed");
    const int blocked = fp16_mfma(p->cfg) ? 1 : 0;
    const int planes = operand_planes(p->cfg);
    for (const Op& o : g->ops) {
        hipError_t e = hipSuccess;
        const char* out_symbol = nullptr;
        hipEvent_t ev_a = nullptr, ev_b = nullptr;
        if (p->profiling) {
            auto take = [&]() -> hipEvent_t {
                hipEvent_t ev = nullptr;
                if (!p->event_pool.empty()) { ev = p->event_pool.back(); p->event_pool.pop_back(); }
                else if (hipEventCreate(&ev) != hipSuccess) ev = nullptr;
                return ev;
            };
            ev_a = take(); ev_b = take();
            if (!ev_a || !ev_b) return fail(MI_EHIP, "hipEventCreate failed");
            (void)hipEventRecord(ev_a, s);
        }
        switch (o.kind) {
            case OP_IN_CONV:
                e = in_conv_launch(io.x, io.cond, wd + p->w_in, wd + p->b_in, F(o.dst.off), T(o.dst.tot_off), g->stat_rep, o.dst.stat_bs,
                                   B, p->cfg.in_channels, g->H, g->W, o.dst.C, blocked, s);
                break;
            case OP_CHAN_TOT:
                e = chan_total_launch(F(o.s0.off), T(o.s0.tot_off), g->stat_rep, o.s0.stat_bs, B, o.s0.H * o.s0.W, o.s0.C, o.stat_rows, blocked, s);
                break;
            case OP_CONV: {
                ConvArgs a{};
                a.src0 = F(o.s0.off); a.C0 = o.s0.C;
                a.src1 = o.has_s1 ? F(o.s1.off) : nullptr; a.C1 = o.has_s1 ? o.s1.C : 0;
                a.B = B; a.H = o.s0.H; a.W = o.s0.W; a.OH = o.dst.H; a.OW = o.dst.W;
                a.wpack = wd + o.w; a.bias = wd + o.b; a.Cout = o.dst.C;
                a.prologue = o.prologue; a.stat_rep = g->stat_rep;
                a.raw_scale_fixed = o.raw_scale_fixed; a.status = status;
                if (o.res_steps > 0) {
                    a.res_steps = o.res_steps; a.res_scale = o.res_scale;
                    a.res_src0 = F(o.res0.off); a.res_C0 = o.res0.C;
                    a.res_src1 = o.has_res1 ? F(o.res1.off) : nullptr; a.res_C1 = o.has_res1 ? o.res1.C : 0;
                    if (o.res0.stat_id >= 0 && (!o.has_res1 || o.res1.stat_id >= 0)) {
                        a.res_tot0 = T(o.res0.tot_off); a.res_bs0 = o.res0.stat_bs;
                        a.res_tot1 = o.has_res1 ? T(o.res1.tot_off) : T(o.res0.tot_off); a.res_bs1 = o.has_res1 ? o.res1.stat_bs : 1;
                    }
                }
                if (o.att_mode != ATT_NONE) {
                    const Att16Layout lay = attention16_layout(B, o.dst.H * o.dst.W, o.att_mode == ATT_QKV_OUT ? o.dst.C / 3 : o.dst.C, planes);
                    a.att_mode = o.att_mode; a.att_heads = ATTN_HEADS_ABI; a.att_D = (o.att_mode == ATT_QKV_OUT ? o.dst.C / 3 : o.dst.C) / ATTN_HEADS_ABI;
                    a.att_npad = lay.npad; a.att_ksplit = o.att_ksplit;
                    a.att_k = reinterpret_cast<_Float16*>(ws + o.partial_off + lay.k_off); a.att_v = reinterpret_cast<_Float16*>(ws + o.partial_off + lay.v_off);
                    a.att_ml = reinterpret_cast<const float*>(ws + o.partial_off + lay.ml_off);
                }
                if (o.gn.on || o.raw_stats) {
                    a.gn_tot0 = T(o.s0.tot_off); a.gn_bs0 = o.s0.stat_bs;
                    a.gn_tot1 = o.has_s1 ? T(o.s1.tot_off) : T(o.s0.tot_off); a.gn_bs1 = o.has_s1 ? o.s1.stat_bs : 1;
                }
                if (o.gn.on) {
                    a.gn_gamma = wd + o.gn.gamma; a.gn_beta = wd + o.gn.beta; a.gn_eps = 1e-5f;
                    a.gn_inv_n = 1.0 / ((double)o.s0.H * o.s0.W * ((a.C0 + a.C1) / GN_GROUPS_));
                }
                if (o.temb_col >= 0) { a.temb = p->ttab + o.temb_col; a.temb_stride = p->temb_cols; a.trow = reinterpret_cast<const int*>(ws + g->trow_off); }
                a.resid = o.has_resid ? F(o.resid.off) : nullptr;
                a.out = F(o.dst.off); a.out_scale = o.out_scale;
                if (o.want_stats) { a.stat_tot = T(o.dst.tot_off); a.stat_bs = o.dst.stat_bs; }
                a.persist_wgs = g->persist_wgs;
                e = fp16_mfma(p->cfg) ? conv16_launch(a, o.tile, s) : conv_launch(a, o.tile, s);
                break;
            }
            case OP_ATTN:
                if (fp16_mfma(p->cfg)) {
                    const int N = o.dst.H * o.dst.W, C = o.dst.C;
                    const Att16Layout lay = attention16_layout(B, N, C, planes);
                    char* sc = ws + o.partial_off;
                    e = attention16_launch(F(o.s0.off), reinterpret_cast<const _Float16*>(sc + lay.k_off), reinterpret_cast<const _Float16*>(sc + lay.v_off),
                                           reinterpret_cast<float*>(sc + lay.po_off), reinterpret_cast<float*>(sc + lay.ml_off),
                                           B, o.att_ksplit, o.att_tps, N, C, ATTN_HEADS_ABI, s, planes);
                } else {
                    e = attention_launch(F(o.s0.off), F(o.dst.off), B, o.dst.H * o.dst.W, o.dst.C, 2, s);
                }
                break;
            case OP_RESIZE:
                e = resize_bilinear_launch(F(o.s0.off), F(o.dst.off), T(o.dst.tot_off), g->stat_rep, o.dst.stat_bs, B, o.s0.H, o.s0.W, o.s0.C, o.dst.H, o.dst.W, blocked, s);
                break;
            case OP_CONVT:
                e = conv_transpose_launch(F(o.s0.off), wd + o.w, wd + o.b, F(o.dst.off), B, o.s0.H, o.s0.W, o.s0.C, o.dst.C, blocked, s);
                break;
            case OP_OUT: {
                OutConvArgs a{};
                a.src = F(o.s0.off); a.blocked = blocked; a.gn_tot = T(o.s0.tot_off); a.stat_rep = g->stat_rep; a.gn_bs = o.s0.stat_bs; a.gn_gamma = wd + o.gn.gamma; a.gn_beta = wd + o.gn.beta; a.gn_eps = 1e-5f;
                a.w = wd + p->w_out; a.bias = wd + p->b_out;
                a.B = B; a.H = g->H; a.W = g->W; a.C = o.s0.C; a.ic = p->cfg.in_channels;
                a.eps_out = io.eps_out; a.x = io.x_update; a.noise = io.noise;
                a.clamp_eps = io.clamp_eps;
                const StepNoise& n = io.sn;
                a.seeded = n.seeded; a.iter = io.iter; a.seed = n.seed; a.sample_offset = n.sample_offset;
                a.v0 = n.v0; a.members = n.members > 0 ? n.members : 1; a.member_offset = n.member_offset;
                a.tiles_x = n.tiles_x; a.tiles_y = n.tiles_y; a.img_H = n.img_H; a.img_W = n.img_W;
                e = out_conv_launch(a, io.update, s);
                out_symbol = out_conv_symbol(io.update, a.seeded);
                break;
            }
        }
        if (e != hipSuccess) return fail(MI_EHIP, "kernel launch (op kind %d) failed: %s", (int)o.kind, hipGetErrorString(e));
        const size_t mid_at = g->ops.size() / (2 * (size_t)mid_div);
        if (mid_event && (size_t)(&o - g->ops.data()) == mid_at) (void)hipEventRecord(mid_event, s);
        if (p->profiling) {
            (void)hipEventRecord(ev_b, s);
            mi_plan::Span sp; sp.a = ev_a; sp.b = ev_b;
            op_work(p, g, o, &sp.name, &sp.flops, &sp.bytes);
            const size_t oc_at = out_symbol ? sp.name.find("out_conv_kernel") : std::string::npos;
            if (oc_at != std::string::npos) sp.name.replace(oc_at, 15, out_symbol);
            static const bool per_op = getenv("MIDD_PROFILE_PER_OP") != nullptr;
            if (per_op) {
                char tag[96];
                snprintf(tag, sizeof(tag), "op%03d %dx%d c%d+%d->%d k%d s%d | ", (int)(&o - g->ops.data()), o.dst.H, o.dst.W,
                         o.s0.C, o.has_s1 ? o.s1.C : 0, o.dst.C, o.ks, o.stride);
                sp.name = std::string(tag) + sp.name;
            }
            p->spans.push_back(std::move(sp));
        }
    }
    return MI_OK;
}

int midd::check_device(mi_plan* plan) {
    int dev = -1;
    if (hipGetDevice(&dev) != hipSuccess || dev != plan->device)
        return fail(MI_ESTATE, "plan was finalized on device %d but current device is %d", plan->device, dev);
    return MI_OK;
}

int midd::check_finalized(mi_plan* plan) {
    return plan->finalized ? MI_OK : fail(MI_ESTATE, "mi_unet_finalize has not been called (or weights changed since)");
}

int midd::check_workspace(const void* ws, size_t got, size_t need) {
    if (!ws || got < need) return fail(MI_ENOMEM, "workspace too small: need %zu bytes, got %zu", need, got);
    if (((uintptr_t)ws) & 255) return fail(MI_EINVAL, "workspace must be 256-byte aligned");
    return MI_OK;
}

int midd::check_call(mi_plan* plan, int B, int H, int W, void* ws, size_t ws_bytes, Program** g) {
    if (!plan) return fail(MI_EINVAL, "null plan");
    if (int rc = get_program(plan, B, H, W, g)) return rc;
    if (int rc = check_workspace(ws, ws_bytes, (*g)->bytes)) return rc;
    return check_device(plan);
}

extern "C" int mi_unet_forward(mi_plan* plan, const float* x, const float* condition, const int32_t* t, float* eps,
                               int B, int H, int W, void* workspace, size_t workspace_bytes, void* stream) {
    Program* g = nullptr;
    int rc = check_call(plan, B, H, W, workspace, workspace_bytes, &g);
    if (rc) return rc;
    if (!x || !condition || !t || !eps) return fail(MI_EINVAL, "null argument");
    for (int i = 0; i < B; ++i)
        if (t[i] < 0 || t[i] >= plan->time_rows) return fail(MI_EINVAL, "timestep %d outside the precomputed table [0,%d)", t[i], plan->time_rows);
    hipStream_t s = (hipStream_t)stream;
    char* ws = (char*)workspace;
    HIPCHK(hipMemsetAsync(ws, 0, 256, s));
    if ((rc = launched(fill_i32_launch(reinterpret_cast<int*>(ws + g->trow_off), t, B, s), "fill timesteps"))) return rc;
    StepIO io{};
    io.x = x; io.cond = condition; io.eps_out = eps;
    return run_program(plan, g, io, ws, reinterpret_cast<int*>(ws), s);
}

extern "C" int mi_debug_fetch(mi_plan* plan, const char* module_name, int B, int H, int W, const void* workspace,
                              float* dst, int* C, int* h, int* w, void* stream) {
    if (!plan || !module_name) return fail(MI_EINVAL, "null argument");
    Program* g = nullptr;
    int rc = get_program(plan, B, H, W, &g);
    if (rc) return rc;
    auto it = g->outputs.find(module_name);
    if (it == g->outputs.end()) return fail(MI_EINVAL, "module \"%s\" has no materialised output in this plan", module_name);
    const TensorRef& t = it->second;
    if (C) *C = t.C; if (h) *h = t.H; if (w) *w = t.W;
    if (dst) {
        if (!workspace) return fail(MI_EINVAL, "null workspace");
        return launched(nhwc_to_nchw_launch(reinterpret_cast<const float*>((const char*)workspace + t.off), dst, B, t.H, t.W, t.C,
                                            fp16_mfma(plan->cfg) ? 1 : 0, (hipStream_t)stream), "nhwc_to_nchw");
    }
    return MI_OK;
}

extern "C" int mi_profile_begin(mi_plan* plan) {
    if (!plan) return fail(MI_EINVAL, "null plan");
    for (auto& sp : plan->spans) { plan->event_pool.push_back(sp.a); plan->event_pool.push_back(sp.b); }
    plan->spans.clear();
    plan->profiling = true;
    return MI_OK;
}

extern "C" int mi_profile_end(mi_plan* plan, mi_profile_entry* out, int max_entries, int* n_entries) {
    if (!plan || !n_entries) return fail(MI_EINVAL, "null argument");
    plan->profiling = false;
    std::map<std::string, mi_profile_entry> agg;
    std::vector<std::string> order;
    for (auto& sp : plan->spans) {
        HIPCHK(hipEventSynchronize(sp.b));
        float ms = 0.f;
        HIPCHK(hipEventElapsedTime(&ms, sp.a, sp.b));
        auto it = agg.find(sp.name);
        if (it == agg.end()) {
            mi_profile_entry e{};
            snprintf(e.name, sizeof(e.name), "%s", sp.name.c_str());
            it = agg.emplace(sp.name, e).first;
            order.push_back(sp.name);
        }
        it->second.launches += 1; it->second.total_ms += ms; it->second.flops += sp.flops; it->second.bytes += sp.bytes;
        plan->event_pool.push_back(sp.a); plan->event_pool.push_back(sp.b);
    }
    plan->spans.clear();
    *n_entries = (int)order.size();
    for (int i = 0; i < (int)order.size() && i < max_entries && out; ++i) out[i] = agg[order[i]];
    if ((int)order.size() > max_entries) *n_entries = max_entries;
    return MI_OK;
}
```

medical-image-denoising-using-diffusion_amd/csrc/midd_host.h:

```cpp
#pragma once
#include "../../include/midd.h"
#include "midd_internal.h"

#include <cmath>
#include <cstdarg>
#include <cstdio>
#include <cstring>
#include <map>
#include <memory>
#include <mutex>
#include <string>
#include <vector>

namespace midd {

constexpr int ATTN_HEADS_ABI = 2;
constexpr float ACT_PRESCALE_H = 16.0f;

int fail(int code, const char* fmt, ...) __attribute__((format(printf, 2, 3)));
#define HIPCHK(expr)                                                                           \
    do {                                                                                       \
        hipError_t e_ = (expr);                                                                \
        if (e_ != hipSuccess) return fail(MI_EHIP, "%s failed: %s", #expr, hipGetErrorString(e_)); \
    } while (0)

enum ModKind { MOD_RB, MOD_ATTN, MOD_DOWN, MOD_UP };
struct Mod {
    ModKind kind;
    std::string name;
    int in_c, out_c;
    int temb_col = -1;
    size_t w1 = 0, b1 = 0, w2 = 0, b2 = 0, wr = 0, br = 0;
    size_t w1x = (size_t)-1, w2x = (size_t)-1, wcx = (size_t)-1;
    size_t b2r = 0;
    size_t g1 = 0, be1 = 0, g2 = 0, be2 = 0;
    size_t wq = 0, bq = 0, wp = 0, bp = 0;
    size_t wc = 0, bc = 0, wt = 0;
    float s1 = 1.f, s2 = 1.f, sr = 1.f, sq = 1.f, sp = 1.f, sc = 1.f;
};

struct HostWeight { std::vector<int64_t> shape; std::vector<float> data; bool loaded = false; };

struct TensorRef {
    size_t off = 0; int C = 0, H = 0, W = 0;
    size_t tot_off = (size_t)-1; int stat_id = -1, stat_bs = 0;
};

struct GnRef { size_t gamma = 0, beta = 0; bool on = false; };

enum OpKind { OP_IN_CONV, OP_CONV, OP_ATTN, OP_RESIZE, OP_CONVT, OP_OUT, OP_CHAN_TOT };
struct Op {
    OpKind kind;
    TensorRef s0, s1, dst, resid;
    bool has_s1 = false, has_resid = false;
    GnRef gn;
    size_t partial_off = 0;
    int att_mode = ATT_NONE, att_ksplit = 1, att_tps = 1;
    int stat_rows = 0;
    size_t w = 0, b = 0;
    int prologue = PRO_RAW, temb_col = -1;
    ConvTile tile{};
    int stride = 1, ks = 3;
    bool want_stats = false;
    TensorRef res0, res1;
    bool has_res1 = false; int res_steps = 0; float res_scale = 1.f;
    bool raw_stats = false;
    float raw_scale_fixed = 1.f;
    float out_scale = 1.f;
};

constexpr int INVARIANT_B = 4;

struct Program {
    int B, H, W;
    int persist_wgs = 0;
    bool wide_chunks = false;
    std::vector<Op> ops;
    size_t bytes = 0, trow_off = 0;
    size_t slot_off = 0;
    size_t stats_off = 0, stats_bytes = 0;
    int stat_rep = 1;
    std::map<std::string, TensorRef> outputs;
};

inline bool packs_wide_copy(const mi_unet_cfg& cfg, int Cin) { return cfg.compute_mode != MI_COMPUTE_F32 && Cin >= 32; }
inline bool fp16_mfma(const mi_unet_cfg& cfg) { return cfg.compute_mode == MI_COMPUTE_F16X3 || cfg.compute_mode == MI_COMPUTE_F16; }
inline int operand_planes(const mi_unet_cfg& cfg) { return cfg.compute_mode == MI_COMPUTE_F16 ? 1 : 2; }

int build_topology(mi_plan* p);
int get_program(mi_plan* p, int B, int H, int W, Program** out, bool side_by_side = false);
int split_parts(int B);
void op_work(mi_plan* p, Program* g, const Op& o, std::string* name, double* flops, double* bytes);
int dump_program(mi_plan* p, int B, int H, int W, bool side_by_side, std::string* out);
struct EnsembleLayout { int pass, tail; size_t run_bytes, cond_off, samples_off, bytes; };
int ensemble_layout(mi_plan* p, int B, int members, int H, int W, int pass_samples, bool samples_external, EnsembleLayout* L);
int check_ensemble_args(mi_plan* p, int B, int members, int H, int W, int64_t sample_offset, int64_t member_offset, int pass_samples);
int check_tiled_args(mi_plan* p, int B, int H, int W, int th, int tw, int oy, int ox, int64_t sample_offset, int pass_samples, TileGeom* g);
int check_tiled_ensemble_args(mi_plan* p, int B, int members, int H, int W, int th, int tw, int oy, int ox, int64_t sample_offset,
                              int64_t member_offset, int pass_samples, TileGeom* g);
int tiled_ensemble_layout(mi_plan* p, int B, int members, int tiles, int th, int tw, int pass_samples, bool tiles_external, EnsembleLayout* L);
int tiled_self_ensemble_layout(mi_plan* p, int B, int n_views, int tiles, int H, int W, int th, int tw, int pass_samples, bool tiles_external,
                               EnsembleLayout* L, size_t* view_off);
}

struct mi_plan {
    mi_unet_cfg cfg{};
    bool batch_invariant = false;
    std::vector<midd::Mod> downs, mid, ups;
    int final_c = 0, temb_cols = 0, levels = 0;
    std::vector<std::string> expected;
    std::map<std::string, std::vector<int64_t>> expected_shape;
    std::map<std::string, midd::HostWeight> host;
    float* wdev = nullptr;
    float* ttab = nullptr; int time_rows = 0;
    size_t w_in = 0, b_in = 0, g_out = 0, be_out = 0, w_out = 0, b_out = 0;
    bool finalized = false;
    int device = -1;
    std::mutex mu;
    std::map<uint64_t, std::unique_ptr<midd::Program>> programs;
    static const int MAX_PARTS = 4;
    hipStream_t sstream[MAX_PARTS] = {nullptr, nullptr, nullptr, nullptr};
    hipEvent_t sev_fork = nullptr, sev_phase[MAX_PARTS] = {nullptr, nullptr, nullptr, nullptr},
               sev_join[MAX_PARTS] = {nullptr, nullptr, nullptr, nullptr};
    std::mutex side_mu;
    bool profiling = false;
    struct Span { hipEvent_t a, b; std::string name; double flops, bytes; };
    std::vector<Span> spans;
    std::vector<hipEvent_t> event_pool;
};
```

medical-image-denoising-using-diffusion_amd/csrc/midd_internal.h:

```cpp
#pragma once
#include <hip/hip_runtime.h>
#include <stdint.h>
#include "stats_common.h"

namespace midd {

constexpr int MIDD_MAX_DEVICES = 64;
inline hipError_t ensure_dynamic_lds(const void* kernel, int bytes, int (&raised)[MIDD_MAX_DEVICES]) {
    if (bytes <= 64 * 1024) return hipSuccess;
    int dev = 0;
    hipError_t e = hipGetDevice(&dev);
    if (e != hipSuccess) return e;
    if (dev < 0 || dev >= MIDD_MAX_DEVICES) return hipErrorInvalidDevice;
    if (bytes > raised[dev]) {
        e = hipFuncSetAttribute(kernel, hipFuncAttributeMaxDynamicSharedMemorySize, bytes);
        if (e != hipSuccess) return e;
        raised[dev] = bytes;
    }
    return hipSuccess;
}

enum Prologue { PRO_RAW = 0, PRO_GN = 1, PRO_GN_SILU = 2 };

__host__ __device__ inline size_t act_index(int blocked, int b, int C, int HW, int pix, int ch) {
    return blocked ? (((size_t)b * (C >> 4) + (ch >> 4)) * HW + pix) * 16 + (ch & 15) : ((size_t)b * HW + pix) * C + ch;
}

struct ConvArgs {
    const float* src0;
    const float* src1;
    int C0, C1;
    int B, H, W;
    int OH, OW;
    const float* wpack;
    const float* bias;
    int Cout;
    const stat_word* gn_tot0; const stat_word* gn_tot1;
    int gn_bs0, gn_bs1;
    float raw_scale_fixed;
    int* status;
    const float* gn_gamma; const float* gn_beta; float gn_eps; double gn_inv_n;
    int prologue;
    const float* temb;
    int temb_stride;
    const int* trow;
    const float* resid;
    float* out;
    float out_scale;
    stat_word* stat_tot;
    int stat_rep;
    int stat_bs;
    const float* res_src0; const float* res_src1;
    int res_C0, res_C1, res_steps;
    float res_scale;
    const stat_word* res_tot0; const stat_word* res_tot1;
    int res_bs0, res_bs1;
    int att_mode;
    _Float16* att_k; _Float16* att_v;
    const float* att_ml;
    int att_heads, att_D, att_npad, att_ksplit;
    int tiles_x, tiles_y;
    int wgs_per_img;
    int persist_wgs;
#ifdef MIDD_CONV_TIMING
    int dbg_slot;
#endif
};

struct ConvTile {
    int ks, stride, tw, mt, nt, wm, wn;
    int cb = 0;
    int pl = 2;
};

enum AttMode { ATT_NONE = 0, ATT_QKV_OUT = 1, ATT_PART_IN = 2 };
enum StatusBits { STATUS_NONFINITE = 1, STATUS_FP16_RANGE = 2,
                  STATUS_DMA_EARLY = 4 };

bool conv_pick_tile(int Cout, int B, int OH, int OW, int ks, int stride, ConvTile* t);
hipError_t conv_launch(const ConvArgs& a, const ConvTile& t, hipStream_t s);

bool conv16_pick_tile(int Cin, int Cout, int B, int OH, int OW, int ks, int stride, ConvTile* t, bool allow_wide = false, int planes = 2);
int conv16_wgs_per_img(int tiles, int B, int ny, int target = 0);
bool conv1x1_pick_tile(int Cin, int Cout, int B, int OH, int OW, ConvTile* t);
hipError_t conv1x1_launch(const ConvArgs& a, const ConvTile& t, hipStream_t s);
hipError_t conv16_launch(const ConvArgs& a, const ConvTile& t, hipStream_t s);
struct ConvLaunchInfo { int grid_x, grid_y, wgs_per_img, tiles_x, tiles_y, ring, ppw, apw, lds_bytes; };
bool conv16_launch_info(int Cin, int Cout, int B, int OH, int OW, const ConvTile& t, int persist_wgs, ConvLaunchInfo* out);
bool conv1x1_launch_info(int Cin, int Cout, int B, int OH, int OW, const ConvTile& t, int persist_wgs, int att_mode, ConvLaunchInfo* out);
__host__ __device__ constexpr int conv16_cb(int ks) { return ks == 1 ? 2 : 1; }
__host__ __device__ constexpr bool conv16_pair_walk(int taps, int cb) { return cb == 1 && taps == 9; }
__host__ __device__ inline int conv16_num_steps(int Cin, int taps, int cb = 0) {
    const int nblk = Cin / 16;
    if (cb == 0) cb = conv16_cb(taps == 1 ? 1 : 3);
    const int full = nblk / 2, half = nblk & 1;
    return full * taps + half * ((taps + 1) / 2);
}

constexpr int GN_GROUPS_ = 8;
hipError_t chan_total_launch(const float* src, stat_word* tot, int rep, int bs, int B, int HW, int C, int rows, int blocked, hipStream_t s);
int chan_partial_rows(int HW, int C);
constexpr size_t CHAN_TOTAL_LDS_LIMIT = 64 * 1024;
inline size_t chan_total_lds_bytes(int C) {
    if (C < 4 || C % 4 || C / 4 > 256) return 0;
    const int ppi = 256 / (C / 4);
    return (size_t)ppi * C * 2 * sizeof(double) + (size_t)(C + 2) * STAT_WORDS * sizeof(stat_word);
}

size_t resize_workspace_bytes(int n, int sw, int sh, int dw, int dh);
hipError_t resize_bicubic_u8_launch(const unsigned char* src, int n, int sw, int sh, unsigned char* dst, int dw, int dh, void* ws, hipStream_t s);
hipError_t u8_to_unit_launch(const unsigned char* src, float* dst, size_t count, hipStream_t s);
hipError_t unit_to_u8_launch(const float* src, unsigned char* dst, size_t count, hipStream_t s);
size_t resize_f32_workspace_bytes(int n, int sw, int sh, int dw, int dh);
hipError_t resize_bicubic_f32_launch(const void* src, int src_type, int n, int sw, int sh, void* dst, int dst_type, int dw, int dh,
                                     int clamp, void* ws, hipStream_t s);
hipError_t u16_to_unit_launch(const uint16_t* src, float* dst, size_t count, hipStream_t s);
hipError_t unit_to_u16_launch(const float* src, uint16_t* dst, size_t count, hipStream_t s);
hipError_t histogram_u16_launch(const uint16_t* src, int n, size_t count, uint32_t* hist, hipStream_t s);
hipError_t window_levels_launch(const uint32_t* hist, int n, double p_lo, double p_hi, int32_t* levels, hipStream_t s);
hipError_t window_u16_to_f32_launch(const uint16_t* src, const int32_t* levels, int n, size_t count, float* dst, hipStream_t s);
hipError_t window_f32_to_u16_launch(const float* src, const int32_t* levels, int n, size_t count, uint16_t* dst, hipStream_t s);
hipError_t resize_bicubic_f32_window_launch(const void* src, int src_type, int n, int sw, int sh, void* dst, int dst_type, int dw, int dh,
                                            int clamp, const int32_t* levels, void* ws, hipStream_t s);
size_t metrics_workspace_bytes(int n, int h);
hipError_t metrics_launch(const float* target, const float* pred, int n, int h, int w, double* out, void* ws, hipStream_t s);

hipError_t attention_launch(const float* qkv, float* out, int B, int N, int C, int heads, hipStream_t s);
struct Att16Layout { size_t k_off, v_off, po_off, ml_off, bytes; int npad; };
Att16Layout attention16_layout(int B, int N, int C, int planes = 2);
hipError_t attention16_launch(const float* q, const _Float16* Kp, const _Float16* Vp, float* part_o, float* part_ml,
                              int B, int ksplit, int tiles_per_split, int N, int C, int heads, hipStream_t s, int planes = 2);
void attention16_split(int N, int heads, int split_B, int* ksplit, int* tiles_per_split);
bool attention_supported(int head_dim);

hipError_t in_conv_launch(const float* x, const float* cond, const float* w , const float* bias,
                          float* out, stat_word* tot, int rep, int bs, int B, int ic, int H, int W, int Cout, int blocked, hipStream_t s);
constexpr size_t POINTWISE_LDS_LIMIT = 64 * 1024;
__host__ __device__ constexpr bool in_conv1_width(int Cout) { return Cout == 32 || Cout == 48 || Cout == 64; }
__host__ __device__ inline size_t in_conv_lds_bytes(int ic, int Cout) {
    const int ppi = 256 / (Cout / 16);
    return (size_t)(9 * 2 * ic * Cout + Cout + 2 * Cout * ppi + 2) * sizeof(float) + (size_t)(Cout + 2) * STAT_WORDS * sizeof(stat_word);
}
constexpr int OC_T = 16;
constexpr int OC_I = OC_T + 2;
constexpr int OC_PS = 20;
__host__ __device__ constexpr size_t out_conv_static_lds_bytes() { return (size_t)OC_I * OC_I * OC_PS * sizeof(float); }
__host__ __device__ inline size_t out_conv_dynamic_lds_bytes(int ic, int C) { return ((size_t)ic * 9 * C + 2 * (size_t)C) * sizeof(float); }
__host__ __device__ inline size_t out_conv_lds_bytes(int ic, int C) { return out_conv_static_lds_bytes() + out_conv_dynamic_lds_bytes(ic, C); }

struct OutConvArgs {
    const float* src;
    int blocked;
    const stat_word* gn_tot; int stat_rep, gn_bs; const float* gn_gamma; const float* gn_beta; float gn_eps;
    const float* w;
    const float* bias;
    int B, H, W, C, ic;
    float* eps_out;
    float* x;
    const float* noise;
    float c1, c2, c3;
    int clamp_eps;
    int seeded;
    int iter;
    unsigned long long seed;
    long long sample_offset;
    int v0;
    int members;
    unsigned member_offset;
    int tiles_x, tiles_y, img_H, img_W;
};
enum SlotBits { SLOT_ACTIVE = 1, SLOT_NOISE = 2 };
struct alignas(16) SlotRec {
    float c1, c2, c3;
    int active;
    unsigned iter;
    unsigned image;
    int trow;
    unsigned member;
    unsigned pitch, plane, origin;
    int pad;
};
static_assert(sizeof(SlotRec) == 48, "out_conv_slots_kernel reads a record as 12 words");
constexpr int SLOTS_PER_LAUNCH = 32;
struct SlotRecs { SlotRec v[SLOTS_PER_LAUNCH]; };
hipError_t slot_fill_launch(int* trow, SlotRec* dst, const SlotRecs& recs, int n, hipStream_t s);
enum SlotRuleBits { SLOT_LAST = 4, SLOT_HIST = 8 };
struct alignas(16) SlotRuleRec {
    int active;
    int trow;
    unsigned iter;
    unsigned image;
    float k0, k1, r0, r1;
    float a, b, s, g;
    unsigned member;
    unsigned pitch, plane, origin;
};
static_assert(sizeof(SlotRuleRec) == 64, "out_conv_slots_rule_kernel reads a record as 16 words");
struct SlotRuleRecs { SlotRuleRec v[SLOTS_PER_LAUNCH]; };
hipError_t slot_rule_fill_launch(int* trow, SlotRuleRec* dst, const SlotRuleRecs& recs, int n, hipStream_t s);
struct DdimCoef {
    float k0, k1, r0, r1, a, b, s;
    int clip_x0;
    int last;
};
struct DpmCoef {
    float k0, k1, r0, r1, a, b;
    float g;
    int clip_x0;
    int last;
};
enum OutUpdateKind { OUT_FORWARD, OUT_REFERENCE, OUT_DDIM, OUT_DPM, OUT_SLOTS, OUT_SLOTS_RULE };
struct RefCoef { float c1, c2, c3; };
struct DpmStep { DpmCoef k; const float* x0_prev; float* x0_out; };
struct SlotRuleStep { const SlotRuleRec* recs; int clip_x0; float* x0_hist; };
struct OutUpdate {
    OutUpdateKind kind;
    union { RefCoef ref; DdimCoef ddim; DpmStep dpm; const SlotRec* slots; SlotRuleStep slots_rule; };
};
hipError_t out_conv_launch(const OutConvArgs& a, const OutUpdate& u, hipStream_t s);
const char* out_conv_symbol(const OutUpdate& u, int seeded);
hipError_t step_noise_fill_launch(float* dst, int n_iters, int B, unsigned long long chw, unsigned long long seed, long long sample_offset,
                                  unsigned member, hipStream_t s);
struct alignas(16) LossRec { float a, s; uint32_t sample; uint32_t draw; };
constexpr int LOSS_RECS_PER_LAUNCH = 32;
struct LossRecs { LossRec v[LOSS_RECS_PER_LAUNCH]; };
constexpr int LOSS_PATCH = 32;
constexpr int LOSS_MAX_SIDE = 1 << 30;
inline int loss_tiles(int H, int W) { return ((H + LOSS_PATCH - 1) / LOSS_PATCH) * ((W + LOSS_PATCH - 1) / LOSS_PATCH); }
hipError_t noise_images_launch(const float* clean, const float* eps, float* x_t, float* eps_out, const LossRec* recs, int B,
                               unsigned long long chw, int seeded, unsigned long long seed, hipStream_t s);
size_t loss_partials_bytes(int B, int C, int H, int W);
hipError_t loss_terms_launch(const float* clean, const float* x_t, const float* eps, const float* eps_pred, const LossRec* recs,
                             int B, int C, int H, int W, int seeded, unsigned long long seed, int clamp_eps,
                             double edge_weight, double* out, float* maps, double* part, hipStream_t s);

hipError_t ensemble_reduce_launch(const float* samples, int B, int K, unsigned long long chw, float* mean, float* std, hipStream_t s);
hipError_t ensemble_broadcast_launch(const float* noisy, float* dst, int v0, int n, int K, unsigned long long chw, hipStream_t s);

struct TileGeom { int C, H, W, th, tw, oy, ox, ny, nx; };
hipError_t tile_extract_launch(const float* noisy, float* dst, const TileGeom& g, int v0, int n, hipStream_t s);
hipError_t tile_blend_launch(const float* tiles, float* out, int B, const TileGeom& g, hipStream_t s);
hipError_t tile_blend_reduce_launch(const float* tiles, int B, int M, const TileGeom& g, float* mean, float* std, float* samples, hipStream_t s);

constexpr int QUANTILE_MAX_MEMBERS = 64, QUANTILE_MAX_LEVELS = 8;
struct QuantileLevels { double q[QUANTILE_MAX_LEVELS]; int nq; };
hipError_t ensemble_quantiles_launch(const float* samples, int B, int K, unsigned long long chw, const QuantileLevels& ql, float* out, hipStream_t s);
hipError_t tile_blend_quantiles_launch(const float* tiles, int B, int M, const TileGeom& g, const QuantileLevels& ql, float* out, hipStream_t s);

size_t ensemble_scores_partials_bytes(int B, unsigned long long chw);
hipError_t ensemble_scores_launch(const float* samples, const float* truth, int B, int K, unsigned long long chw, const QuantileLevels& ql,
                                  double* sums, unsigned long long* invalid, unsigned long long* rank_hist, unsigned long long* counts,
                                  float* crps_map, double* part, hipStream_t s);

constexpr int NPS_CHUNK = 16;
struct NpsTables { float tc[64]; float ts[64]; float w[128]; };
unsigned long long nps_chunks(int K, int H, int W, int R, int S);
size_t nps_workspace_bytes(int groups, int K, int H, int W, int R, int S);
hipError_t nps_launch(const float* a, const float* b, int B, int K, int C, int H, int W, int R, int S, int detrend, const float* window,
                      double scale, int exclude_axes, double* nps, double* radial, long long* radial_count, long long* rois_used,
                      long long* rois_skipped, void* ws, hipStream_t s);

constexpr int DIHEDRAL_MAX_VIEWS = 8;
struct DihedralViews { int n; uint8_t code[DIHEDRAL_MAX_VIEWS]; };
hipError_t dihedral_views_launch(const float* images, float* dst, const DihedralViews& dv, int C, int H, int W, int v0, int n, hipStream_t s);
hipError_t dihedral_reduce_launch(const float* views_out, int B, const DihedralViews& dv, int C, int H, int W,
                                  float* mean, float* std, float* samples, hipStream_t s);
hipError_t dihedral_quantiles_launch(const float* views_out, int B, const DihedralViews& dv, int C, int H, int W,
                                     const QuantileLevels& ql, float* out, hipStream_t s);

hipError_t plane_view_launch(const float* images, float* dst, int code, int B, int C, int H, int W, hipStream_t s);
hipError_t tile_blend_unview_reduce_launch(const float* tiles, int B, const DihedralViews& dv, const TileGeom& g,
                                           float* mean, float* std, float* samples, hipStream_t s);
hipError_t tile_blend_unview_quantiles_launch(const float* tiles, int B, const DihedralViews& dv, const TileGeom& g,
                                              const QuantileLevels& ql, float* out, hipStream_t s);

hipError_t resize_bilinear_launch(const float* src, float* dst, stat_word* tot, int rep, int bs, int B, int H, int W, int C, int OH, int OW, int blocked, hipStream_t s);
hipError_t conv_transpose_launch(const float* src, const float* w , const float* bias, float* dst,
                                 int B, int H, int W, int Cin, int Cout, int blocked, hipStream_t s);
hipError_t nhwc_to_nchw_launch(const float* src, float* dst, int B, int H, int W, int C, int blocked, hipStream_t s);
hipError_t fill_i32_launch(int* dst, const int* host_vals, int n, hipStream_t s);

}
```

medical-image-denoising-using-diffusion_amd/csrc/midd_planner.hip:

```cpp
#include "midd_host.h"

using namespace midd;

struct ConvSpec {
    const TensorRef* s0; const TensorRef* s1;
    TensorRef* dst;
    size_t w, b; float wscale;
    bool wide = false; size_t w_wide = 0;
    int ks = 3, stride = 1, temb_col = -1;
    int prologue = PRO_RAW; GnRef gn{};
    const TensorRef* resid = nullptr;
    bool want_stats = true;
    float raw_scale_fixed = 1.0f;
    int att_mode = ATT_NONE; size_t att_scratch = 0; int att_ksplit = 1;
    const TensorRef* res0 = nullptr; const TensorRef* res1 = nullptr; float res_wscale = 1.f;
};

struct Builder {
    mi_plan* p; Program* g; int B;
    size_t cur = 0;
    size_t take(size_t bytes) { size_t o = (cur + 255) & ~(size_t)255; cur = o + bytes; return o; }
    TensorRef alloc(int C, int H, int W) {
        TensorRef t; t.C = C; t.H = H; t.W = W;
        t.off = take((size_t)B * H * W * C * sizeof(float));
        return t;
    }
    struct StatInfo { int C, bs; size_t off; };
    std::vector<StatInfo> stats;
    static int gcd(int a, int b) { while (b) { const int t = a % b; a = b; b = t; } return a; }
    void alloc_stats(TensorRef& t) { t.stat_id = (int)stats.size(); stats.push_back(StatInfo{t.C, t.C, 0}); }
    int gn_consumer(const TensorRef& s0, const TensorRef* s1) {
        if (s0.stat_id < 0 || (s1 && s1->stat_id < 0)) return fail(MI_EINVAL, "internal: GroupNorm input without statistics");
        const int cg = (s0.C + (s1 ? s1->C : 0)) / GN_GROUPS_;
        stats[s0.stat_id].bs = gcd(stats[s0.stat_id].bs, cg);
        if (s1) stats[s1->stat_id].bs = gcd(gcd(stats[s1->stat_id].bs, cg), s0.C % cg);
        return MI_OK;
    }
    void ensure_stats(TensorRef& t) {
        if (t.stat_id >= 0) return;
        alloc_stats(t);
        Op o{}; o.kind = OP_CHAN_TOT; o.s0 = t; o.stat_rows = chan_partial_rows(t.H * t.W, t.C); g->ops.push_back(o);
    }
    int conv(const ConvSpec& c) {
        const TensorRef &s0 = *c.s0, *s1 = c.s1; TensorRef& dst = *c.dst;
        const int cin = s0.C + (s1 ? s1->C : 0);
        const bool f16 = fp16_mfma(p->cfg);
        Op o{}; o.kind = OP_CONV; o.att_mode = c.att_mode; o.partial_off = c.att_scratch; o.att_ksplit = c.att_ksplit; o.s0 = s0; if (s1) { o.s1 = *s1; o.has_s1 = true; }
        o.out_scale = (c.prologue == PRO_RAW && f16) ? c.wscale * ACT_PRESCALE_H : c.wscale;
        o.raw_scale_fixed = c.raw_scale_fixed;
        o.raw_stats = c.prologue == PRO_RAW && s0.stat_id >= 0 && (!s1 || s1->stat_id >= 0);
        o.w = c.w; o.b = c.b; o.ks = c.ks; o.stride = c.stride; o.prologue = c.prologue; o.temb_col = c.temb_col; o.gn = c.gn;
        if (c.gn.on) { if (int rcg = gn_consumer(s0, s1)) return rcg; }
        if (c.resid) { o.resid = *c.resid; o.has_resid = true; }
        if (c.res0) {
            o.res0 = *c.res0; if (c.res1) { o.res1 = *c.res1; o.has_res1 = true; }
            o.res_steps = (c.res0->C + (c.res1 ? c.res1->C : 0) + 31) / 32;
            o.res_scale = c.res_wscale * ACT_PRESCALE_H;
        }
        const int Bp = p->batch_invariant ? INVARIANT_B : B;
        const bool ok = f16 ? conv16_pick_tile(cin, dst.C, Bp, dst.H, dst.W, c.ks, c.stride, &o.tile, g->wide_chunks && c.wide && packs_wide_copy(p->cfg, cin), operand_planes(p->cfg))
                            : conv_pick_tile(dst.C, Bp, dst.H, dst.W, c.ks, c.stride, &o.tile);
        if (!ok) return fail(MI_EINVAL, "no conv tile for Cout=%d ks=%d stride=%d", dst.C, c.ks, c.stride);
        if (o.tile.cb == 2) o.w = c.w_wide;
        if (c.att_mode == ATT_PART_IN) o.tile.mt = 1;
        if (c.want_stats) { alloc_stats(dst); o.want_stats = true; }
        o.dst = dst;
        g->ops.push_back(o);
        return MI_OK;
    }
};

static int build_program(mi_plan* p, int B, int H, int W, Program* g) {
    const mi_unet_cfg& c = p->cfg;
    const int div = 1 << (p->levels - 1);
    if (B < 1 || H < div || W < div || H % div || W % div)
        return fail(MI_EINVAL, "H and W must be positive multiples of %d (got %dx%d), B >= 1", div, H, W);
    g->B = B; g->H = H; g->W = W;
    g->stat_rep = (640 / B + 47) / 48;
    if (g->stat_rep < 1) g->stat_rep = 1;
    if (g->stat_rep > STAT_MAX_REPLICAS) g->stat_rep = STAT_MAX_REPLICAS;
    Builder bld{p, g, B};
    (void)bld.take(256);
    g->trow_off = bld.take((size_t)B * sizeof(int));
    g->slot_off = bld.take((size_t)B * sizeof(SlotRuleRec));
    int rc;

    auto run_rb = [&](const Mod& m, const TensorRef& s0, const TensorRef* s1, TensorRef* out) -> int {
        const int cin = s0.C + (s1 ? s1->C : 0);
        if (cin != m.in_c) return fail(MI_EINVAL, "%s: expected %d input channels, graph provides %d", m.name.c_str(), m.in_c, cin);
        TensorRef h1 = bld.alloc(m.out_c, s0.H, s0.W);
        TensorRef o = bld.alloc(m.out_c, s0.H, s0.W), acc;
        ConvSpec c1{&s0, s1, &h1, m.w1, m.b1, m.s1};
        c1.wide = true; c1.w_wide = m.w1x; c1.prologue = PRO_GN_SILU; c1.gn = GnRef{m.g1, m.be1, true}; c1.temb_col = m.temb_col;
        if ((rc = bld.conv(c1))) return rc;
        ConvSpec c2{&h1, nullptr, &o, m.w2, m.b2, m.s2};
        c2.wide = true; c2.w_wide = m.w2x; c2.prologue = PRO_GN_SILU; c2.gn = GnRef{m.g2, m.be2, true};
        if (m.in_c != m.out_c && fp16_mfma(p->cfg)) {
            c2.b = m.b2r; c2.res0 = &s0; c2.res1 = s1; c2.res_wscale = m.sr;
        } else if (m.in_c != m.out_c) {
            ConvSpec cr{&s0, s1, &o, m.wr, m.br, m.sr};
            cr.ks = 1; cr.want_stats = false;
            if ((rc = bld.conv(cr))) return rc;
            acc = o; c2.resid = &acc;
        } else {
            if (s1) return fail(MI_EINVAL, "%s: identity residual over a concatenated input", m.name.c_str());
            c2.resid = &s0;
        }
        if ((rc = bld.conv(c2))) return rc;
        *out = o;
        return MI_OK;
    };
    auto run_attn = [&](const Mod& m, const TensorRef& x, TensorRef* out) -> int {
        const int C = x.C, N = x.H * x.W;
        const bool f16 = fp16_mfma(p->cfg);
        TensorRef y = bld.alloc(C, x.H, x.W);
        const Att16Layout lay = attention16_layout(B, N, C, operand_planes(p->cfg));
        const size_t scratch = f16 ? bld.take(lay.bytes) : 0;
        int ksplit = 1, tps = 1;
        if (f16) attention16_split(N, ATTN_HEADS_ABI, p->batch_invariant ? INVARIANT_B : B, &ksplit, &tps);
        TensorRef qkv = bld.alloc(3 * C, x.H, x.W);
        ConvSpec cq{&x, nullptr, &qkv, m.wq, m.bq, m.sq};
        cq.ks = 1; cq.prologue = PRO_GN; cq.gn = GnRef{m.g1, m.be1, true}; cq.want_stats = false;
        if (f16) { cq.att_mode = ATT_QKV_OUT; cq.att_scratch = scratch; cq.att_ksplit = ksplit; }
        if ((rc = bld.conv(cq))) return rc;
        TensorRef att{}; att.off = scratch + lay.po_off; att.C = C; att.H = x.H; att.W = x.W;
        if (!f16) att = bld.alloc(C, x.H, x.W);
        Op o{}; o.kind = OP_ATTN; o.s0 = qkv; o.dst = f16 ? y : att; o.partial_off = scratch; o.att_ksplit = ksplit; o.att_tps = tps;
        g->ops.push_back(o);
        ConvSpec cp{&att, nullptr, &y, m.wp, m.bp, m.sp};
        cp.ks = 1; cp.resid = &x;
        if (f16) { cp.raw_scale_fixed = ACT_PRESCALE_H; cp.att_mode = ATT_PART_IN; cp.att_scratch = scratch; cp.att_ksplit = ksplit; }
        if ((rc = bld.conv(cp))) return rc;
        *out = y;
        return MI_OK;
    };

    TensorRef h = bld.alloc(c.model_channels, H, W);
    { Op o{}; o.kind = OP_IN_CONV; bld.alloc_stats(h); o.dst = h; g->ops.push_back(o); }
    g->outputs["in_conv"] = h;
    std::vector<TensorRef> skips;
    auto run_block = [&](const Mod& m) -> int {
        TensorRef o;
        if ((rc = m.kind == MOD_RB ? run_rb(m, h, nullptr, &o) : run_attn(m, h, &o))) return rc;
        h = o; g->outputs[m.name] = h;
        return MI_OK;
    };
    for (const Mod& m : p->downs) {
        if (m.kind == MOD_DOWN) {
            TensorRef o = bld.alloc(m.out_c, h.H / 2, h.W / 2);
            ConvSpec cd{&h, nullptr, &o, m.wc, m.bc, m.sc};
            cd.stride = 2;
            if ((rc = bld.conv(cd))) return rc;
            h = o; g->outputs[m.name] = h;
        } else if ((rc = run_block(m))) return rc;
        skips.push_back(h);
    }
    for (const Mod& m : p->mid) if ((rc = run_block(m))) return rc;
    const Mod* pending_up = nullptr;
    auto flush_up = [&]() -> int {
        if (!pending_up) return MI_OK;
        const size_t tot_lds = chan_total_lds_bytes(pending_up->out_c);
        if (!tot_lds)
            return fail(MI_EINVAL, "%s: an unfolded ConvTranspose of %d channels: chan_total takes a multiple of 4 channels, at most 1024",
                        pending_up->name.c_str(), pending_up->out_c);
        if (tot_lds > CHAN_TOTAL_LDS_LIMIT)
            return fail(MI_EINVAL, "%s: an unfolded ConvTranspose of %d channels: chan_total needs %zu bytes of LDS for its output, the limit is %zu bytes",
                        pending_up->name.c_str(), pending_up->out_c, tot_lds, CHAN_TOTAL_LDS_LIMIT);
        TensorRef o = bld.alloc(pending_up->out_c, h.H * 2, h.W * 2);
        Op op{}; op.kind = OP_CONVT; op.s0 = h; op.dst = o; op.w = pending_up->wt; op.b = pending_up->bc;
        g->ops.push_back(op);
        bld.ensure_stats(o);
        g->outputs[pending_up->name] = o;
        h = o; pending_up = nullptr;
        return MI_OK;
    };
    for (const Mod& m : p->ups) {
        if (m.kind == MOD_UP) { if ((rc = flush_up())) return rc; pending_up = &m; continue; }
        if (m.kind == MOD_ATTN) { if ((rc = flush_up()) || (rc = run_block(m))) return rc; continue; }
        if (skips.empty()) return fail(MI_EINVAL, "%s: skip stack empty", m.name.c_str());
        TensorRef skip = skips.back(); skips.pop_back();
        if (pending_up) {
            if (skip.H == h.H && skip.W == h.W) {
                TensorRef o = bld.alloc(pending_up->out_c, h.H, h.W);
                ConvSpec cu{&h, nullptr, &o, pending_up->wc, pending_up->bc, pending_up->sc};
                cu.wide = true; cu.w_wide = pending_up->wcx;
                if ((rc = bld.conv(cu))) return rc;
                h = o; pending_up = nullptr;
            } else if ((rc = flush_up())) return rc;
        }
        if (h.H != skip.H || h.W != skip.W) {
            TensorRef o = bld.alloc(h.C, skip.H, skip.W);
            bld.alloc_stats(o);
            Op op{}; op.kind = OP_RESIZE; op.s0 = h; op.dst = o; g->ops.push_back(op);
            h = o;
        }
        TensorRef o; if ((rc = run_rb(m, h, &skip, &o))) return rc;
        h = o; g->outputs[m.name] = h;
    }
    if ((rc = flush_up())) return rc;
    if (h.H != H || h.W != W) return fail(MI_EINVAL, "network output is %dx%d for a %dx%d input", h.H, h.W, H, W);
    if ((rc = bld.gn_consumer(h, nullptr))) return rc;
    { Op o{}; o.kind = OP_OUT; o.s0 = h; o.gn = GnRef{p->g_out, p->be_out, true}; g->ops.push_back(o); }
    size_t cur = 0;
    for (auto& st : bld.stats) {
        st.off = cur;
        cur += ((size_t)B * (st.C / st.bs) * g->stat_rep * STAT_WORDS * sizeof(stat_word) + 255) & ~(size_t)255;
    }
    g->stats_bytes = cur;
    g->stats_off = bld.take(g->stats_bytes);
    auto resolve = [&](TensorRef& t) {
        if (t.stat_id >= 0) { t.tot_off = g->stats_off + bld.stats[t.stat_id].off; t.stat_bs = bld.stats[t.stat_id].bs; }
    };
    for (Op& o : g->ops) for (TensorRef* t : {&o.s0, &o.s1, &o.dst, &o.resid, &o.res0, &o.res1}) resolve(*t);
    for (auto& kv : g->outputs) resolve(kv.second);
    g->bytes = (bld.cur + 255) & ~(size_t)255;
    return MI_OK;
}

static void setup_program(const mi_plan* p, int B, bool side_by_side, Program* g) {
    g->persist_wgs = side_by_side ? 640 : 0;
    if (p->batch_invariant) g->persist_wgs = 640 / INVARIANT_B * B;
    g->wide_chunks = !side_by_side && !p->batch_invariant;
}

static bool plan_as_side() {
    static const bool on = getenv("MIDD_PLAN_AS_SIDE") != nullptr;
    return on;
}

int midd::get_program(mi_plan* p, int B, int H, int W, Program** out, bool side_by_side) {
    if (!p->finalized) return fail(MI_ESTATE, "mi_unet_finalize has not been called (or weights changed since)");
    side_by_side = side_by_side || plan_as_side();
    const uint64_t key = ((uint64_t)(side_by_side ? 1 : 0) << 63) ^ ((uint64_t)B << 40) ^ ((uint64_t)H << 20) ^ (uint64_t)W;
    std::lock_guard<std::mutex> lk(p->mu);
    auto it = p->programs.find(key);
    if (it == p->programs.end()) {
        std::unique_ptr<Program> g(new Program());
        setup_program(p, B, side_by_side, g.get());
        int rc = build_program(p, B, H, W, g.get());
        if (rc) return rc;
        it = p->programs.emplace(key, std::move(g)).first;
    }
    *out = it->second.get();
    return MI_OK;
}

int midd::split_parts(int B) {
    static const int want = getenv("MIDD_SPLIT") ? atoi(getenv("MIDD_SPLIT")) : 2;
    int parts = (want >= 4) ? 4 : (want >= 2 ? 2 : 1);
    while (parts > 1 && (B % parts || B / parts < 2)) parts /= 2;
    return parts;
}

static size_t sampler_bytes(mi_plan* p, int B, int H, int W) {
    auto bytes_of = [&](int b, bool side) -> size_t {
        if (p->finalized) { Program* g = nullptr; return get_program(p, b, H, W, &g, side) ? 0 : g->bytes; }
        Program g;
        setup_program(p, b, side || plan_as_side(), &g);
        std::lock_guard<std::mutex> lk(p->mu);
        return build_program(p, b, H, W, &g) ? 0 : g.bytes;
    };
    size_t need = bytes_of(B, false);
    const int parts = split_parts(B);
    if (need && parts > 1) {
        const size_t part = bytes_of(B / parts, true);
        if (!part) return 0;
        if (parts * part > need) need = parts * part;
    }
    return need;
}

extern "C" size_t mi_workspace_bytes(mi_plan* plan, int B, int H, int W) {
    Program* g = nullptr;
    if (!plan || get_program(plan, B, H, W, &g)) return 0;
    return sampler_bytes(plan, B, H, W);
}

int midd::ensemble_layout(mi_plan* p, int B, int members, int H, int W, int pass_samples, bool samples_external, EnsembleLayout* L) {
    auto round256 = [](size_t v) { return (v + 255) & ~(size_t)255; };
    const int64_t V = (int64_t)B * members;
    L->pass = (int)(V < pass_samples ? V : pass_samples);
    if (L->pass > 65535) L->pass = 65535;
    L->tail = (int)(V % L->pass);
    L->run_bytes = sampler_bytes(p, L->pass, H, W);
    if (!L->run_bytes) return MI_EINVAL;
    if (L->tail) {
        const size_t t = sampler_bytes(p, L->tail, H, W);
        if (!t) return MI_EINVAL;
        if (t > L->run_bytes) L->run_bytes = t;
    }
    const size_t chw = (size_t)p->cfg.in_channels * H * W;
    L->cond_off = round256(L->run_bytes);
    L->samples_off = L->cond_off + round256((size_t)L->pass * chw * sizeof(float));
    L->bytes = L->samples_off + (samples_external ? 0 : (size_t)V * chw * sizeof(float));
    return MI_OK;
}

extern "C" size_t mi_ensemble_workspace_bytes(mi_plan* plan, int B, int members, int H, int W, int pass_samples, int samples_external) {
    if (check_ensemble_args(plan, B, members, H, W, 0, 0, pass_samples)) return 0;
    EnsembleLayout L{};
    if (ensemble_layout(plan, B, members, H, W, pass_samples, samples_external != 0, &L)) return 0;
    return L.bytes;
}

extern "C" size_t mi_self_ensemble_workspace_bytes(mi_plan* plan, int B, int n_views, int H, int W, int pass_samples, int samples_external) {
    (void)samples_external;
    if (n_views < 1 || n_views > DIHEDRAL_MAX_VIEWS) {
        fail(MI_EINVAL, "n_views %d outside [1, %d]: a view list holds 1 to 8 distinct view codes (limit: 1 <= n_views <= %d)", n_views,
             DIHEDRAL_MAX_VIEWS, DIHEDRAL_MAX_VIEWS);
        return 0;
    }
    if (check_ensemble_args(plan, B, n_views, H, W, 0, 0, pass_samples)) return 0;
    EnsembleLayout L{};
    if (ensemble_layout(plan, B, n_views, H, W, pass_samples, false, &L)) return 0;
    return L.bytes;
}

extern "C" size_t mi_tiled_workspace_bytes(mi_plan* plan, int B, int H, int W, int th, int tw, int oy, int ox, int pass_samples, int tiles_external) {
    TileGeom g{};
    if (check_tiled_args(plan, B, H, W, th, tw, oy, ox, 0, pass_samples, &g)) return 0;
    EnsembleLayout L{};
    if (ensemble_layout(plan, B, g.ny * g.nx, th, tw, pass_samples, tiles_external != 0, &L)) return 0;
    return L.bytes;
}

int midd::tiled_ensemble_layout(mi_plan* p, int B, int members, int tiles, int th, int tw, int pass_samples, bool tiles_external, EnsembleLayout* L) {
    if (int rc = ensemble_layout(p, B, tiles, th, tw, pass_samples, true, L)) return rc;
    if (!tiles_external) L->bytes += (size_t)members * B * tiles * p->cfg.in_channels * th * tw * sizeof(float);
    return MI_OK;
}

extern "C" size_t mi_tiled_ensemble_workspace_bytes(mi_plan* plan, int B, int members, int H, int W, int th, int tw, int oy, int ox,
                                                    int pass_samples, int tiles_external) {
    TileGeom g{};
    if (check_tiled_ensemble_args(plan, B, members, H, W, th, tw, oy, ox, 0, 0, pass_samples, &g)) return 0;
    EnsembleLayout L{};
    if (tiled_ensemble_layout(plan, B, members, g.ny * g.nx, th, tw, pass_samples, tiles_external != 0, &L)) return 0;
    return L.bytes;
}

int midd::tiled_self_ensemble_layout(mi_plan* p, int B, int n_views, int tiles, int H, int W, int th, int tw, int pass_samples, bool tiles_external,
                                     EnsembleLayout* L, size_t* view_off) {
    if (int rc = ensemble_layout(p, B, tiles, th, tw, pass_samples, true, L)) return rc;
    const size_t C = (size_t)p->cfg.in_channels;
    *view_off = L->samples_off;
    L->samples_off += ((size_t)B * C * H * W * sizeof(float) + 255) & ~(size_t)255;
    L->bytes = L->samples_off + (tiles_external ? 0 : (size_t)n_views * B * tiles * C * th * tw * sizeof(float));
    return MI_OK;
}

void midd::op_work(mi_plan* p, Program* g, const Op& o, std::string* name, double* flops, double* bytes) {
    const double B = g->B;
    char buf[128];
    auto elems = [&](const TensorRef& t) { return B * t.H * t.W * t.C; };
    switch (o.kind) {
        case OP_IN_CONV:
            *name = p->cfg.in_channels == 1 ? "midd::in_conv1_kernel" : "midd::in_conv_kernel";
            *flops = 2.0 * B * g->H * g->W * o.dst.C * 9 * 2 * p->cfg.in_channels;
            *bytes = 4.0 * (2.0 * B * p->cfg.in_channels * g->H * g->W + elems(o.dst));
            break;
        case OP_CHAN_TOT: *name = "midd::chan_total_kernel"; *flops = 0; *bytes = 4.0 * elems(o.s0); break;
        case OP_CONV: {
            const char* mode = p->cfg.compute_mode == MI_COMPUTE_F16X3 ? "f16x3" : p->cfg.compute_mode == MI_COMPUTE_F16 ? "f16" : "f32";
            if (fp16_mfma(p->cfg) && o.tile.ks == 1 && o.tile.tw == 0)
                snprintf(buf, sizeof(buf), "midd::conv1x1_%s_kernel<%d, %d, %d>", mode, o.tile.mt, o.tile.nt, o.att_mode);
            else {
                char tail[32] = "";
                if (fp16_mfma(p->cfg))
                    snprintf(tail, sizeof(tail), ", %s, %d", (o.res_steps > 0 && o.tile.stride == 1 && o.tile.ks == 3) ? "true" : "false", o.tile.cb);
                snprintf(buf, sizeof(buf), "midd::conv_mfma_%s_kernel<%d, %d, %d, %d, %d, %d, %d%s>",
                         mode, o.tile.ks, o.tile.stride,
                         o.tile.tw, o.tile.mt, o.tile.nt, o.tile.wm, o.tile.wn, tail);
            }
            *name = buf;
            const double cin = o.s0.C + (o.has_s1 ? o.s1.C : 0);
            const double res_cin = o.res_steps > 0 ? o.res0.C + (o.has_res1 ? o.res1.C : 0) : 0;
            *flops = 2.0 * elems(o.dst) * (cin * o.ks * o.ks + res_cin);
            *bytes = 4.0 * (elems(o.s0) + (o.has_s1 ? elems(o.s1) : 0) + elems(o.dst) + (o.has_resid ? elems(o.resid) : 0)
                            + (o.res_steps > 0 ? elems(o.res0) + (o.has_res1 ? elems(o.res1) : 0) : 0)
                            + (double)o.dst.C * (cin * o.ks * o.ks + res_cin));
            break;
        }
        case OP_ATTN: {
            const double N = (double)o.dst.H * o.dst.W;
            snprintf(buf, sizeof(buf), "midd::attention_%s_kernel<%d>", p->cfg.compute_mode == MI_COMPUTE_F16X3 ? "f16x3" : p->cfg.compute_mode == MI_COMPUTE_F16 ? "f16" : "f32", o.dst.C / 2);
            *name = buf;
            *flops = 4.0 * B * N * N * o.dst.C;
            *bytes = 4.0 * (elems(o.s0) + elems(o.dst));
            break;
        }
        case OP_RESIZE: *name = "midd::resize_bilinear_kernel"; *flops = 0; *bytes = 4.0 * (elems(o.s0) + elems(o.dst)); break;
        case OP_CONVT:
            *name = "midd::conv_transpose_kernel";
            *flops = 2.0 * elems(o.s0) * o.dst.C * 16; *bytes = 4.0 * (elems(o.s0) + elems(o.dst));
            break;
        case OP_OUT:
            *name = p->cfg.in_channels == 1 ? "midd::out_conv_kernel<1>" : "midd::out_conv_kernel<0>";
            *flops = 2.0 * B * g->H * g->W * o.s0.C * 9 * p->cfg.in_channels;
            *bytes = 4.0 * (elems(o.s0) + 3.0 * B * p->cfg.in_channels * g->H * g->W);
            break;
    }
}

int midd::dump_program(mi_plan* p, int B, int H, int W, bool side_by_side, std::string* out) {
    Program g;
    setup_program(p, B, side_by_side, &g);
    auto appendf = [out](const char* fmt, auto... v) {
        const size_t at = out->size(), n = snprintf(nullptr, 0, fmt, v...);
        out->resize(at + n + 1);
        snprintf(&(*out)[at], n + 1, fmt, v...);
        out->resize(at + n);
    };
    {
        std::lock_guard<std::mutex> lk(p->mu);
        if (int rc = build_program(p, B, H, W, &g)) return rc;
    }
    appendf("program B=%d %dx%d side=%d bytes=%zu stats_off=%zu stats_bytes=%zu stat_rep=%d persist_wgs=%d wide=%d ops=%zu\n",
            B, H, W, (int)side_by_side, g.bytes, g.stats_off, g.stats_bytes, g.stat_rep, g.persist_wgs, (int)g.wide_chunks, g.ops.size());
    static const char* kinds[] = {"in_conv", "conv", "attn", "resize", "convT", "out", "chan_tot"};
    for (const Op& o : g.ops) {
        std::string name; double fl, by;
        op_work(p, &g, o, &name, &fl, &by);
        appendf("op%03d %-8s %dx%d c%d+%d->%d k%d s%d pro%d res_steps%d att%d ksplit%d tps%d bs(in %d,%d out %d) | %s",
                (int)(&o - g.ops.data()), kinds[o.kind], o.dst.H ? o.dst.H : H, o.dst.W ? o.dst.W : W, o.s0.C, o.has_s1 ? o.s1.C : 0, o.dst.C, o.ks, o.stride,
                o.prologue, o.res_steps, o.att_mode, o.att_ksplit, o.att_tps, o.s0.stat_bs, o.has_s1 ? o.s1.stat_bs : 0, o.dst.stat_bs, name.c_str());
        ConvLaunchInfo li{};
        if (o.kind == OP_CONV && fp16_mfma(p->cfg) &&
            conv16_launch_info(o.s0.C + (o.has_s1 ? o.s1.C : 0), o.dst.C, B, o.dst.H, o.dst.W, o.tile, g.persist_wgs, &li))
            appendf(" | grid %dx%d wgs/img %d tiles %dx%d ring %d ppw %d apw %d lds %d", li.grid_x, li.grid_y, li.wgs_per_img,
                    li.tiles_x, li.tiles_y, li.ring, li.ppw, li.apw, li.lds_bytes);
        *out += '\n';
    }
    return MI_OK;
}
```

medical-image-denoising-using-diffusion_amd/native.py:

```python
from __future__ import annotations

import ctypes as C
import os
import threading

_HERE = os.path.dirname(os.path.abspath(__file__))
LIB_PATH = os.environ.get("MIDD_LIBRARY") or os.path.join(_HERE, "libmidd.so")

MI_MAX_LEVELS = 8
MI_VARIANT = {"ddim": 0, "cddpm": 1}
MI_CLAMP_EPS = 1
MI_NO_SPLIT = 2
MI_COMPUTE = {"f32": 0, "f16x3": 1, "f16": 2}
MI_STATUS_NONFINITE, MI_STATUS_FP16_RANGE = 1, 2
MI_COMPUTE_BATCH_INVARIANT = 0x100
MI_UPDATE = {"reference": 0, "ddim": 1, "dpmpp2m": 2}
MI_PIX_U8, MI_PIX_U16, MI_PIX_F32 = 0, 1, 2


class NativeLibraryError(RuntimeError):
    pass


class MiddError(RuntimeError):
    def __init__(self, code: int, message: str):
        super().__init__(f"libmidd error {code}: {message}")
        self.code = code


class UNetCfg(C.Structure):
    _fields_ = [("in_channels", C.c_int32), ("model_channels", C.c_int32), ("num_levels", C.c_int32),
                ("channel_mult", C.c_int32 * MI_MAX_LEVELS), ("num_res_blocks", C.c_int32),
                ("num_attention_levels", C.c_int32), ("attention_levels", C.c_int32 * MI_MAX_LEVELS),
                ("time_emb_dim", C.c_int32), ("variant", C.c_int32), ("compute_mode", C.c_int32)]


class UpdateRule(C.Structure):
    _fields_ = [("kind", C.c_int32), ("eta", C.c_double), ("clip_x0", C.c_int32)]


class ProfileEntry(C.Structure):
    _fields_ = [("name", C.c_char * 128), ("launches", C.c_int64), ("total_ms", C.c_double),
                ("flops", C.c_double), ("bytes", C.c_double)]


SYMBOLS = [
    ("mi_unet_plan_create", C.c_int, [C.POINTER(UNetCfg), C.POINTER(C.c_void_p)]),
    ("mi_unet_load_weights", C.c_int, [C.c_void_p, C.c_char_p, C.c_void_p, C.POINTER(C.c_int64), C.c_int]),
    ("mi_unet_num_weights", C.c_int, [C.c_void_p]),
    ("mi_unet_weight_name", C.c_char_p, [C.c_void_p, C.c_int]),
    ("mi_unet_finalize", C.c_int, [C.c_void_p, C.c_int]),
    ("mi_workspace_bytes", C.c_size_t, [C.c_void_p, C.c_int, C.c_int, C.c_int]),
    ("mi_unet_forward", C.c_int, [C.c_void_p, C.c_void_p, C.c_void_p, C.POINTER(C.c_int32), C.c_void_p,
                                  C.c_int, C.c_int, C.c_int, C.c_void_p, C.c_size_t, C.c_void_p]),
    ("mi_denoise", C.c_int, [C.c_void_p, C.c_void_p, C.c_void_p, C.c_int, C.c_int, C.c_int,
                             C.POINTER(C.c_int32), C.c_int, C.POINTER(C.c_float), C.POINTER(C.c_float),
                             C.POINTER(C.c_float), C.c_int, C.c_void_p, C.c_int, C.c_void_p, C.c_size_t, C.c_void_p]),
    ("mi_denoise_seeded", C.c_int, [C.c_void_p, C.c_void_p, C.c_void_p, C.c_int, C.c_int, C.c_int,
                                    C.POINTER(C.c_int32), C.c_int, C.POINTER(C.c_float), C.POINTER(C.c_float),
                                    C.POINTER(C.c_float), C.c_int, C.c_uint64, C.c_int64, C.c_int, C.c_void_p, C.c_size_t,
                                    C.c_void_p]),
    ("mi_denoise_slots", C.c_int, [C.c_void_p, C.c_void_p, C.c_void_p, C.c_int, C.c_int, C.c_int,
                                   C.POINTER(C.c_int32), C.c_int, C.POINTER(C.c_int32), C.POINTER(C.c_int64),
                                   C.POINTER(C.c_float), C.POINTER(C.c_float), C.POINTER(C.c_float), C.c_int,
                                   C.c_void_p, C.c_int, C.c_uint64, C.c_int, C.c_void_p, C.c_size_t, C.c_void_p]),
    ("mi_denoise_slots_virtual", C.c_int, [C.c_void_p, C.c_void_p, C.c_void_p, C.c_int, C.c_int, C.c_int,
                                           C.POINTER(C.c_int32), C.c_int, C.POINTER(C.c_int32), C.POINTER(C.c_int64),
                                           C.POINTER(C.c_int64), C.POINTER(C.c_uint32),
                                           C.POINTER(C.c_float), C.POINTER(C.c_float), C.POINTER(C.c_float), C.c_int,
                                           C.c_void_p, C.c_int, C.c_uint64, C.c_int, C.c_void_p, C.c_size_t, C.c_void_p]),
    ("mi_step_noise_fill", C.c_int, [C.c_void_p, C.c_int, C.c_int, C.c_int, C.c_int, C.c_int, C.c_uint64, C.c_int64,
                                     C.c_void_p]),
    ("mi_step_noise_fill_member", C.c_int, [C.c_void_p, C.c_int, C.c_int, C.c_int, C.c_int, C.c_int, C.c_uint64, C.c_int64,
                                            C.c_int64, C.c_void_p]),
    ("mi_denoise_ensemble", C.c_int, [C.c_void_p, C.c_void_p, C.c_void_p, C.c_void_p, C.c_void_p, C.c_int, C.c_int, C.c_int, C.c_int,
                                      C.POINTER(C.c_int32), C.c_int, C.POINTER(C.c_float), C.POINTER(C.c_float),
                                      C.POINTER(C.c_float), C.c_int, C.c_uint64, C.c_int64, C.c_int64, C.c_int, C.c_int,
                                      C.c_void_p, C.c_size_t, C.c_void_p]),
    ("mi_ensemble_workspace_bytes", C.c_size_t, [C.c_void_p, C.c_int, C.c_int, C.c_int, C.c_int, C.c_int, C.c_int]),
    ("mi_ensemble_reduce", C.c_int, [C.c_void_p, C.c_int, C.c_int, C.c_int64, C.c_void_p, C.c_void_p, C.c_void_p]),
    ("mi_ensemble_quantiles", C.c_int, [C.c_void_p, C.c_int, C.c_int, C.c_int64, C.POINTER(C.c_double), C.c_int, C.c_void_p, C.c_void_p]),
    ("mi_ensemble_scores_workspace_bytes", C.c_size_t, [C.c_int, C.c_int, C.c_int64]),
    ("mi_ensemble_scores", C.c_int, [C.c_void_p, C.c_void_p, C.c_int, C.c_int, C.c_int64, C.POINTER(C.c_double), C.c_int] +
                                    [C.c_void_p] * 5 + [C.c_void_p, C.c_size_t, C.c_void_p]),
    ("mi_noise_power_spectrum_workspace_bytes", C.c_size_t, [C.c_int] * 7),
    ("mi_noise_power_spectrum", C.c_int, [C.c_void_p, C.c_void_p] + [C.c_int] * 8 + [C.POINTER(C.c_float), C.c_double, C.c_int] +
                                         [C.c_void_p] * 5 + [C.c_void_p, C.c_size_t, C.c_void_p]),
    ("mi_tile_geometry", C.c_int, [C.c_int, C.c_int, C.c_int, C.POINTER(C.c_int), C.POINTER(C.c_int), C.c_int]),
    ("mi_tile_extract", C.c_int, [C.c_void_p] + [C.c_int] * 10 + [C.c_void_p, C.c_void_p]),
    ("mi_tile_blend", C.c_int, [C.c_void_p] + [C.c_int] * 8 + [C.c_void_p, C.c_void_p]),
    ("mi_denoise_tiled", C.c_int, [C.c_void_p, C.c_void_p, C.c_void_p, C.c_void_p] + [C.c_int] * 7 +
                                  [C.POINTER(C.c_int32), C.c_int, C.POINTER(C.c_float), C.POINTER(C.c_float), C.POINTER(C.c_float), C.c_int,
                                   C.c_int, C.c_uint64, C.c_int64, C.c_int, C.c_int, C.c_void_p, C.c_size_t, C.c_void_p]),
    ("mi_tiled_workspace_bytes", C.c_size_t, [C.c_void_p] + [C.c_int] * 9),
    ("mi_denoise_tiled_ensemble", C.c_int, [C.c_void_p] * 6 + [C.c_int] * 8 +
                                           [C.POINTER(C.c_int32), C.c_int, C.POINTER(C.c_float), C.POINTER(C.c_float), C.POINTER(C.c_float), C.c_int,
                                            C.c_uint64, C.c_int64, C.c_int64, C.c_int, C.c_int, C.c_void_p, C.c_size_t, C.c_void_p]),
    ("mi_tiled_ensemble_workspace_bytes", C.c_size_t, [C.c_void_p] + [C.c_int] * 10),
    ("mi_tile_blend_reduce", C.c_int, [C.c_void_p] + [C.c_int] * 9 + [C.c_void_p] * 4),
    ("mi_tile_blend_quantiles", C.c_int, [C.c_void_p] + [C.c_int] * 9 + [C.POINTER(C.c_double), C.c_int, C.c_void_p, C.c_void_p]),
    ("mi_dihedral_views", C.c_int, [C.c_void_p] + [C.c_int] * 4 + [C.POINTER(C.c_int32), C.c_int, C.c_int, C.c_int, C.c_void_p, C.c_void_p]),
    ("mi_dihedral_reduce", C.c_int, [C.c_void_p] + [C.c_int] * 4 + [C.POINTER(C.c_int32), C.c_int] + [C.c_void_p] * 4),
    ("mi_dihedral_quantiles", C.c_int, [C.c_void_p] + [C.c_int] * 4 + [C.POINTER(C.c_int32), C.c_int, C.POINTER(C.c_double), C.c_int,
                                        C.c_void_p, C.c_void_p]),
    ("mi_denoise_self_ensemble", C.c_int, [C.c_void_p] * 5 + [C.c_int] * 3 + [C.POINTER(C.c_int32), C.c_int] +
                                          [C.POINTER(C.c_int32), C.c_int, C.POINTER(C.c_float), C.POINTER(C.c_float), C.POINTER(C.c_float), C.c_int,
                                           C.c_int, C.c_uint64, C.c_int64, C.c_int64, C.c_int, C.c_int, C.c_void_p, C.c_size_t, C.c_void_p]),
    ("mi_self_ensemble_workspace_bytes", C.c_size_t, [C.c_void_p] + [C.c_int] * 6),
    ("mi_tile_blend_unview_reduce", C.c_int, [C.c_void_p] + [C.c_int] * 8 + [C.POINTER(C.c_int32), C.c_int] + [C.c_void_p] * 4),
    ("mi_tile_blend_unview_quantiles", C.c_int, [C.c_void_p] + [C.c_int] * 8 + [C.POINTER(C.c_int32), C.c_int, C.POINTER(C.c_double), C.c_int,
                                                 C.c_void_p, C.c_void_p]),
    ("mi_denoise_tiled_self_ensemble", C.c_int, [C.c_void_p] * 6 + [C.c_int] * 7 + [C.POINTER(C.c_int32), C.c_int] +
                                                [C.POINTER(C.c_int32), C.c_int, C.POINTER(C.c_float), C.POINTER(C.c_float), C.POINTER(C.c_float), C.c_int,
                                                 C.c_int, C.c_uint64, C.c_int64, C.c_int64, C.c_int, C.c_int, C.POINTER(UpdateRule),
                                                 C.c_void_p, C.c_size_t, C.c_void_p]),
    ("mi_tiled_self_ensemble_workspace_bytes", C.c_size_t, [C.c_void_p] + [C.c_int] * 10),
    ("mi_ddim_coefficients", C.c_int, [C.POINTER(C.c_int32), C.c_int, C.POINTER(C.c_float), C.c_int, C.c_double, C.POINTER(C.c_float)]),
    ("mi_denoise_rule", C.c_int, [C.c_void_p, C.c_void_p, C.c_void_p, C.c_int, C.c_int, C.c_int,
                                  C.POINTER(C.c_int32), C.c_int, C.POINTER(C.c_float), C.POINTER(C.c_float),
                                  C.POINTER(C.c_float), C.c_int, C.c_void_p, C.c_int, C.c_uint64, C.c_int64, C.c_int,
                                  C.POINTER(UpdateRule), C.c_void_p, C.c_size_t, C.c_void_p]),
    ("mi_denoise_ensemble_rule", C.c_int, [C.c_void_p, C.c_void_p, C.c_void_p, C.c_void_p, C.c_void_p, C.c_int, C.c_int, C.c_int, C.c_int,
                                           C.POINTER(C.c_int32), C.c_int, C.POINTER(C.c_float), C.POINTER(C.c_float),
                                           C.POINTER(C.c_float), C.c_int, C.c_uint64, C.c_int64, C.c_int64, C.c_int, C.c_int,
                                           C.POINTER(UpdateRule), C.c_void_p, C.c_size_t, C.c_void_p]),
    ("mi_denoise_tiled_rule", C.c_int, [C.c_void_p, C.c_void_p, C.c_void_p, C.c_void_p] + [C.c_int] * 7 +
                                       [C.POINTER(C.c_int32), C.c_int, C.POINTER(C.c_float), C.POINTER(C.c_float), C.POINTER(C.c_float), C.c_int,
                                        C.c_int, C.c_uint64, C.c_int64, C.c_int, C.c_int, C.POINTER(UpdateRule), C.c_void_p, C.c_size_t, C.c_void_p]),
    ("mi_dpm_coefficients", C.c_int, [C.POINTER(C.c_int32), C.c_int, C.POINTER(C.c_float), C.c_int, C.POINTER(C.c_float)]),
    ("mi_denoise_dpm", C.c_int, [C.c_void_p, C.c_void_p, C.c_void_p, C.c_void_p, C.c_int, C.c_int, C.c_int, C.c_int,
                                 C.POINTER(C.c_int32), C.c_int, C.POINTER(C.c_float), C.POINTER(C.c_float),
                                 C.POINTER(C.c_float), C.c_int, C.c_int, C.c_int, C.c_void_p, C.c_size_t, C.c_void_p]),
    ("mi_denoise_tiled_dpm", C.c_int, [C.c_void_p, C.c_void_p, C.c_void_p, C.c_void_p, C.c_void_p] + [C.c_int] * 7 +
                                      [C.POINTER(C.c_int32), C.c_int, C.POINTER(C.c_float), C.POINTER(C.c_float), C.POINTER(C.c_float), C.c_int,
                                       C.c_int, C.c_int, C.c_int, C.c_void_p, C.c_size_t, C.c_void_p]),
    ("mi_update_row", C.c_int, [C.c_int32, C.c_int32, C.c_int32, C.POINTER(C.c_float), C.c_int, C.c_double, C.POINTER(C.c_float)]),
    ("mi_denoise_slots_rule", C.c_int, [C.c_void_p, C.c_void_p, C.c_void_p, C.c_int, C.c_int, C.c_int,
                                        C.POINTER(C.c_int32), C.c_int, C.POINTER(C.c_int32), C.POINTER(C.c_int64),
                                        C.POINTER(C.c_int64), C.POINTER(C.c_uint32),
                                        C.POINTER(C.c_int32), C.POINTER(C.c_int32), C.c_void_p,
                                        C.POINTER(C.c_float), C.POINTER(C.c_float), C.POINTER(C.c_float), C.c_int,
                                        C.c_void_p, C.c_int, C.c_uint64, C.c_int, C.POINTER(UpdateRule), C.c_void_p, C.c_size_t, C.c_void_p]),
    ("mi_debug_fetch", C.c_int, [C.c_void_p, C.c_char_p, C.c_int, C.c_int, C.c_int, C.c_void_p, C.c_void_p,
                                 C.POINTER(C.c_int), C.POINTER(C.c_int), C.POINTER(C.c_int), C.c_void_p]),
    ("mi_status", C.c_int, [C.c_void_p, C.c_void_p, C.POINTER(C.c_int)]),
    ("mi_debug_attention_split", C.c_int, [C.c_int, C.c_int, C.POINTER(C.c_int), C.POINTER(C.c_int)]),
    ("mi_debug_plan_dump", C.c_int, [C.c_void_p, C.c_int, C.c_int, C.c_int, C.c_int, C.c_char_p, C.c_size_t]),
    ("mi_debug_conv16_geometry", C.c_int, [C.c_int] * 8 + [C.POINTER(C.c_int)] * 4),
    ("mi_debug_conv16_geometry_planes", C.c_int, [C.c_int] * 9 + [C.POINTER(C.c_int)] * 4),
    ("mi_debug_conv16_steps", C.c_int, [C.c_int] * 3),
    ("mi_source_hash", C.c_char_p, []),
    ("mi_profile_begin", C.c_int, [C.c_void_p]),
    ("mi_profile_end", C.c_int, [C.c_void_p, C.POINTER(ProfileEntry), C.c_int, C.POINTER(C.c_int)]),
    ("mi_resize_workspace_bytes", C.c_size_t, [C.c_int, C.c_int, C.c_int, C.c_int, C.c_int]),
    ("mi_resize_bicubic_u8", C.c_int, [C.c_void_p, C.c_int, C.c_int, C.c_int, C.c_void_p, C.c_int, C.c_int,
                                       C.c_void_p, C.c_size_t, C.c_void_p]),
    ("mi_u8_to_unit_f32", C.c_int, [C.c_void_p, C.c_void_p, C.c_size_t, C.c_void_p]),
    ("mi_unit_f32_to_u8", C.c_int, [C.c_void_p, C.c_void_p, C.c_size_t, C.c_void_p]),
    ("mi_resize_f32_workspace_bytes", C.c_size_t, [C.c_int, C.c_int, C.c_int, C.c_int, C.c_int]),
    ("mi_resize_bicubic_f32", C.c_int, [C.c_void_p, C.c_int, C.c_int, C.c_int, C.c_int, C.c_void_p, C.c_int, C.c_int, C.c_int, C.c_int,
                                        C.c_void_p, C.c_size_t, C.c_void_p]),
    ("mi_u16_to_unit_f32", C.c_int, [C.c_void_p, C.c_void_p, C.c_size_t, C.c_void_p]),
    ("mi_unit_f32_to_u16", C.c_int, [C.c_void_p, C.c_void_p, C.c_size_t, C.c_void_p]),
    ("mi_histogram_u16", C.c_int, [C.c_void_p, C.c_int, C.c_size_t, C.c_void_p, C.c_void_p]),
    ("mi_window_levels", C.c_int, [C.c_void_p, C.c_int, C.c_double, C.c_double, C.c_void_p, C.c_void_p]),
    ("mi_window_u16_to_f32", C.c_int, [C.c_void_p, C.c_void_p, C.c_int, C.c_size_t, C.c_void_p, C.c_void_p]),
    ("mi_window_f32_to_u16", C.c_int, [C.c_void_p, C.c_void_p, C.c_int, C.c_size_t, C.c_void_p, C.c_void_p]),
    ("mi_resize_bicubic_f32_window", C.c_int, [C.c_void_p, C.c_int, C.c_int, C.c_int, C.c_int, C.c_void_p, C.c_int, C.c_int, C.c_int,
                                               C.c_int, C.c_void_p, C.c_void_p, C.c_size_t, C.c_void_p]),
    ("mi_metrics_workspace_bytes", C.c_size_t, [C.c_int, C.c_int]),
    ("mi_image_metrics", C.c_int, [C.c_void_p, C.c_void_p, C.c_int, C.c_int, C.c_int, C.c_void_p,
                                   C.c_void_p, C.c_size_t, C.c_void_p]),
    ("mi_noise_images", C.c_int, [C.c_void_p, C.POINTER(C.c_int32), C.POINTER(C.c_float), C.c_int, C.c_void_p, C.c_int, C.c_uint64, C.c_int64,
                                  C.c_int64, C.POINTER(C.c_int64), C.POINTER(C.c_int64), C.c_void_p, C.c_void_p] + [C.c_int] * 4 + [C.c_void_p]),
    ("mi_loss_workspace_bytes", C.c_size_t, [C.c_int] * 4),
    ("mi_loss_terms", C.c_int, [C.c_void_p] * 4 + [C.POINTER(C.c_int32), C.POINTER(C.c_float), C.c_int, C.c_int, C.c_uint64, C.c_int64, C.c_int64,
                                C.POINTER(C.c_int64), C.POINTER(C.c_int64), C.c_int, C.c_double, C.c_void_p, C.c_void_p] + [C.c_int] * 4 + [C.c_void_p, C.c_size_t, C.c_void_p]),
    ("mi_denoising_loss_workspace_bytes", C.c_size_t, [C.c_void_p, C.c_int, C.c_int, C.c_int]),
    ("mi_denoising_loss", C.c_int, [C.c_void_p] * 3 + [C.POINTER(C.c_int32), C.POINTER(C.c_float), C.c_int, C.c_void_p, C.c_int, C.c_uint64, C.c_int64,
                                    C.c_int64, C.POINTER(C.c_int64), C.POINTER(C.c_int64), C.c_int, C.c_double, C.c_void_p, C.c_void_p] + [C.c_int] * 3 + [C.c_void_p, C.c_size_t, C.c_void_p]),
    ("mi_plan_destroy", None, [C.c_void_p]),
    ("mi_last_error", C.c_char_p, []),
    ("mi_version", C.c_char_p, []),
]

_lib = None
_lock = threading.Lock()


def lib() -> C.CDLL:
    global _lib
    if _lib is not None:
        return _lib
    with _lock:
        if _lib is None:
            if not os.path.exists(LIB_PATH):
                raise NativeLibraryError(
                    f"{LIB_PATH} not found: build it with `python -c 'import __graft_entry__ as g; g.build()'` "
                    "(or `make -C medical-image-denoising-using-diffusion_amd/csrc`). "
                    "This package has no CPU fallback.")
            try:
                handle = C.CDLL(LIB_PATH)
            except OSError as exc:
                raise NativeLibraryError(f"cannot load {LIB_PATH}: {exc}") from exc
            for name, restype, argtypes in SYMBOLS:
                fn = getattr(handle, name)
                fn.restype = restype
                fn.argtypes = argtypes
            _lib = handle
    return _lib


def check(rc: int) -> None:
    if rc != 0:
        raise MiddError(rc, lib().mi_last_error().decode("utf-8", "replace"))


def tree_source_hash() -> str:
    import glob
    import hashlib
    h = hashlib.sha256()
    for path in sorted(glob.glob(os.path.join(_HERE, "csrc", "*.h*"))):
        with open(path, "rb") as f:
            h.update(os.path.basename(path).encode() + b"\0" + f.read())
    return h.hexdigest()[:16]


def kernel_source_hash() -> str:
    return lib().mi_source_hash().decode()
```

Measured before the change: 51.44 images/s.

## Split 3x3 conv reduction across two workgroups with ticketed partial-sum handoff

Adds a split-K mode for stride-1 3x3 fp16 MFMA convolutions. Two workgroups each cover half of the input-channel chunks and write fp32 partial accumulators to a global slab. An atomic ticket picks the second arrival, which adds the other half's partials and runs the epilogue and stats publish. The planner turns this on by default for small grids (at most 256 WGs) in the non-side-by-side, non-batch-invariant plan, so launches that underfill the GPU get twice the workgroups. The cost is extra global traffic, an atomic, and duplicated prologue work per slice.

```diff
diff --git a/include/midd.h b/include/midd.h
--- a/include/midd.h
+++ b/include/midd.h
@@ -254,6 +254,7 @@
 int mi_debug_conv16_geometry_planes(int ks, int stride, int tw, int mt, int nt, int wm, int wn, int cb, int planes,
                                     int* ring, int* ppw, int* apw, int* lds_bytes);
 int mi_debug_conv16_steps(int Cin, int ks, int cb);
+int mi_debug_conv16_kslice(int Cin, int cb, int slice, int* c_begin, int* c_end);
 
 const char* mi_source_hash(void);
 
diff --git a/medical-image-denoising-using-diffusion_amd/csrc/conv_mfma_f16x3.hip b/medical-image-denoising-using-diffusion_amd/csrc/conv_mfma_f16x3.hip
--- a/medical-image-denoising-using-diffusion_amd/csrc/conv_mfma_f16x3.hip
+++ b/medical-image-denoising-using-diffusion_amd/csrc/conv_mfma_f16x3.hip
@@ -61,7 +61,7 @@
 };
 
 #ifdef MIDD_CONV_TIMING
-enum { TS_WAIT, TS_ISSUE, TS_MFMA, TS_CHUNK_WAIT, TS_TRANSFORM, TS_EPILOGUE, TS_PROLOGUE, TS_FIRSTWAIT, TS_DMAWAIT, TS_RES, TS_PUBLISH, TS_TOTAL, TS_REAL, TS_WGS, TS_N };
+enum { TS_WAIT, TS_ISSUE, TS_MFMA, TS_CHUNK_WAIT, TS_TRANSFORM, TS_EPILOGUE, TS_PROLOGUE, TS_FIRSTWAIT, TS_DMAWAIT, TS_RES, TS_PUBLISH, TS_HANDOFF, TS_TOTAL, TS_REAL, TS_WGS, TS_N };
 __device__ unsigned long long g_conv_timing[64][TS_N];
 __device__ __forceinline__ unsigned long long ts_stamp() {
     unsigned long long t;
@@ -86,6 +86,7 @@
 #define MIDD_CONV16_BOUNDS __launch_bounds__(WM * WN * 64, (WM * WN == 4 && STRIDE == 1) ? (CBT == 2 ? 2 : (RES && MT == 2) ? MIDD_RES_MT2_WAVES : MIDD_CONV16_WAVES_PER_SIMD) : 1)
 #define MIDD_CONV16_KERNEL conv_mfma_f16x3_kernel
 #define MIDD_CONV16_PL 2
+#define MIDD_CONV16_KSL 0
 #include "conv_mfma_f16x3_body.h"
 #undef MIDD_CONV16_KERNEL
 #undef MIDD_CONV16_PL
@@ -94,6 +95,19 @@
 #include "conv_mfma_f16x3_body.h"
 #undef MIDD_CONV16_KERNEL
 #undef MIDD_CONV16_PL
+#undef MIDD_CONV16_KSL
+#define MIDD_CONV16_KSL 1
+#define MIDD_CONV16_KERNEL conv_mfma_f16x3_ks_kernel
+#define MIDD_CONV16_PL 2
+#include "conv_mfma_f16x3_body.h"
+#undef MIDD_CONV16_KERNEL
+#undef MIDD_CONV16_PL
+#define MIDD_CONV16_KERNEL conv_mfma_f16_ks_kernel
+#define MIDD_CONV16_PL 1
+#include "conv_mfma_f16x3_body.h"
+#undef MIDD_CONV16_KERNEL
+#undef MIDD_CONV16_PL
+#undef MIDD_CONV16_KSL
 
 #ifdef MIDD_CONV_TIMING
 static std::vector<std::string> g_timing_names;
@@ -109,12 +123,12 @@
     static unsigned long long h[64][TS_N];
     (void)hipDeviceSynchronize();
     (void)hipMemcpyFromSymbol(h, HIP_SYMBOL(g_conv_timing), sizeof h);
-    static const char* names[] = {"barrier", "dma-issue", "frag+mfma", "chunk-wait", "transform", "epilogue", "prologue", "wait-after-epi", "dma-wait", "res-phase", "publish"};
+    static const char* names[] = {"barrier", "dma-issue", "frag+mfma", "chunk-wait", "transform", "epilogue", "prologue", "wait-after-epi", "dma-wait", "res-phase", "publish", "k-handoff"};
     for (size_t i = 0; i < g_timing_names.size(); ++i) {
         const double tot = (double)h[i][TS_TOTAL], wgs = (double)h[i][TS_WGS];
         if (wgs == 0) continue;
         printf("%-70s cyc/wg %9.0f clk %.2f GHz |", g_timing_names[i].c_str(), tot / wgs, tot / (double)h[i][TS_REAL] * 0.1);
-        for (int k = 0; k < 11; ++k) printf(" %s %4.1f%%", names[k], 100.0 * (double)h[i][k] / tot);
+        for (int k = 0; k < 12; ++k) printf(" %s %4.1f%%", names[k], 100.0 * (double)h[i][k] / tot);
         printf("\n");
     }
     memset(h, 0, sizeof h);
@@ -131,6 +145,14 @@
     const int ny = a.Cout / (WN * NT * 16);
     a.wgs_per_img = conv16_wgs_per_img(a.tiles_x * a.tiles_y, a.B, ny, a.persist_wgs);
     dim3 grid(a.B * a.wgs_per_img, ny);
+    if (a.kslices == 2) {
+        const int nchunks = ((a.C0 + a.C1) / 16 + G::CB - 1) / G::CB;
+        if (KS != 3 || STRIDE != 1 || a.wgs_per_img != a.tiles_x * a.tiles_y || !conv16_kslices_legal(nchunks) || !a.kslab || !a.ktickets)
+            return hipErrorInvalidValue;
+        grid.x *= 2;
+    } else if (a.kslices != 0 && a.kslices != 1) {
+        return hipErrorInvalidValue;
+    }
 #ifdef MIDD_CONV_TIMING
     a.dbg_slot = conv_timing_slot(KS, STRIDE, TW, MT * 10 + G::CB, NT, WM, WN, a.OH, a.C0 + a.C1, a.Cout, a.B, G::RING, (int)grid.x * (int)grid.y);
 #endif
@@ -144,6 +166,17 @@
             if (e != hipSuccess) return e;
         }
         if ((double)a.H * a.W * 64.0 >= 4294967296.0) return hipErrorInvalidValue;
+        if constexpr (KS == 3 && STRIDE == 1) {
+            if (a.kslices == 2) {
+                static int raised_ks[MIDD_MAX_DEVICES] = {};
+                hipError_t e = ensure_dynamic_lds(PL == 2 ? reinterpret_cast<const void*>(&conv_mfma_f16x3_ks_kernel<KS, STRIDE, TW, MT, NT, WM, WN, RES, CBT>)
+                                                          : reinterpret_cast<const void*>(&conv_mfma_f16_ks_kernel<KS, STRIDE, TW, MT, NT, WM, WN, RES, CBT>), lds_bytes, raised_ks);
+                if (e != hipSuccess) return e;
+                if constexpr (PL == 2) hipLaunchKernelGGL((conv_mfma_f16x3_ks_kernel<KS, STRIDE, TW, MT, NT, WM, WN, RES, CBT>), grid, dim3(G::NTHREADS), lds_bytes, s, a);
+                else hipLaunchKernelGGL((conv_mfma_f16_ks_kernel<KS, STRIDE, TW, MT, NT, WM, WN, RES, CBT>), grid, dim3(G::NTHREADS), lds_bytes, s, a);
+                return hipGetLastError();
+            }
+        }
         if constexpr (PL == 2) hipLaunchKernelGGL((conv_mfma_f16x3_kernel<KS, STRIDE, TW, MT, NT, WM, WN, RES, CBT>), grid, dim3(G::NTHREADS), lds_bytes, s, a);
         else hipLaunchKernelGGL((conv_mfma_f16_kernel<KS, STRIDE, TW, MT, NT, WM, WN, RES, CBT>), grid, dim3(G::NTHREADS), lds_bytes, s, a);
         return hipGetLastError();
@@ -241,6 +274,16 @@
     return true;
 }
 
+bool conv16_kslices_ok(int Cin, const ConvTile& t, const ConvLaunchInfo& li) {
+    if (t.ks != 3 || t.stride != 1 || t.tw == 0) return false;
+    const int cb = t.cb == 2 ? 2 : conv16_cb(3);
+    return li.wgs_per_img == li.tiles_x * li.tiles_y && conv16_kslices_legal((Cin / 16 + cb - 1) / cb);
+}
+
+size_t conv16_kslab_bytes(const ConvTile& t, const ConvLaunchInfo& li) {
+    return (size_t)li.grid_x * li.grid_y * 2 * t.mt * t.nt * (t.wm * t.wn * 64) * 16;
+}
+
 template <int PL>
 static hipError_t conv16_dispatch(const ConvArgs& a, const ConvTile& t, hipStream_t s) {
     if (t.cb == 2) {
diff --git a/medical-image-denoising-using-diffusion_amd/csrc/conv_mfma_f16x3_body.h b/medical-image-denoising-using-diffusion_amd/csrc/conv_mfma_f16x3_body.h
--- a/medical-image-denoising-using-diffusion_amd/csrc/conv_mfma_f16x3_body.h
+++ b/medical-image-denoising-using-diffusion_amd/csrc/conv_mfma_f16x3_body.h
@@ -1,10 +1,11 @@
-#if !defined(MIDD_CONV16_KERNEL) || !defined(MIDD_CONV16_PL)
-#error "include from conv_mfma_f16x3.hip with MIDD_CONV16_KERNEL and MIDD_CONV16_PL defined"
+#if !defined(MIDD_CONV16_KERNEL) || !defined(MIDD_CONV16_PL) || !defined(MIDD_CONV16_KSL)
+#error "include from conv_mfma_f16x3.hip with MIDD_CONV16_KERNEL, MIDD_CONV16_PL and MIDD_CONV16_KSL defined"
 #endif
 
 template <int KS, int STRIDE, int TW, int MT, int NT, int WM, int WN, bool RES, int CBT>
 __global__ MIDD_CONV16_BOUNDS void MIDD_CONV16_KERNEL(const ConvArgs a) {
     constexpr int PL = MIDD_CONV16_PL;
+    constexpr bool KSL = MIDD_CONV16_KSL != 0;
     static_assert(PL == 1 || PL == 2, "planes");
     using G = Conv16Geom<KS, STRIDE, TW, MT, NT, WM, WN, CBT, PL>;
     constexpr int NW = G::NW, NTHREADS = G::NTHREADS, TH = G::TH, IW = G::IW;
@@ -31,8 +32,11 @@
     const int kq = lane >> 4;
 
     const int tiles_per_img = a.tiles_x * a.tiles_y;
-    const int b = blockIdx.x / a.wgs_per_img;
-    int trem = blockIdx.x - b * a.wgs_per_img;
+    const int gx0 = a.B * a.wgs_per_img;
+    const int ksl = (KSL && a.kslices == 2 && (int)blockIdx.x >= gx0) ? 1 : 0;
+    const int bx = blockIdx.x - ksl * gx0;
+    const int b = bx / a.wgs_per_img;
+    int trem = bx - b * a.wgs_per_img;
     int oy0 = (trem / a.tiles_x) * TH, ox0 = (trem % a.tiles_x) * TW;
 
     const int Cin = a.C0 + a.C1;
@@ -41,12 +45,16 @@
     const int nchunks = (nblk + CB - 1) / CB;
     const int ntiles_total = a.Cout >> 4;
     const int ntile_wg = blockIdx.y * (WN * NT);
-    const int res_steps = RES ? a.res_steps : 0;
-    const int total_steps = conv16_num_steps(Cin, TAPS, G::CB) + res_steps;
+    int c_begin = 0, c_end = nchunks;
+    if (KSL && a.kslices == 2) conv16_kslice_range(nchunks, 2, ksl, &c_begin, &c_end);
+    const int res_all = RES ? a.res_steps : 0;
+    const int res_steps = (c_end == nchunks) ? res_all : 0;
+    const int step0 = KSL ? conv16_steps_before(Cin, TAPS, G::CB, c_begin) : 0;
+    const int total_steps = (KSL ? conv16_steps_before(Cin, TAPS, G::CB, c_end) - step0 : conv16_num_steps(Cin, TAPS, G::CB)) + res_steps;
 
     constexpr int WTILE = PL * 1024;
-    const char* const wbase = reinterpret_cast<const char*>(a.wpack) + (size_t)ntile_wg * WTILE;
     const size_t wstep_bytes = (size_t)ntiles_total * WTILE;
+    const char* const wbase = reinterpret_cast<const char*>(a.wpack) + (size_t)ntile_wg * WTILE + (size_t)step0 * wstep_bytes;
     const int lane16 = lane * 16;
     int wr_step = 0, wr_slot = 0;
     const char* wr_src = wbase;
@@ -144,7 +152,7 @@
         }
         char* base = img + sblk * PL * PLANE + (q8 & 3) * 8;
         typedef unsigned u32x2 __attribute__((ext_vector_type(2)));
-        if (c == 0 && tile_pad) {
+        if (c == c_begin && tile_pad) {
 #pragma unroll
             for (int s = 0; s < APW; ++s) {
                 const int slot = tid + s * NTHREADS;
@@ -206,7 +214,7 @@
     constexpr auto cmin = [](int x, int y) { return x < y ? x : y; };
     const int ntile0 = ntile_wg + wn * NT;
     TS_DECL
-    issue_a(0);
+    issue_a(c_begin);
 #pragma unroll
     for (int i = 0; i < D; ++i) issue_w();
 #if !(defined(C16_ABL) && C16_ABL == 6)
@@ -218,7 +226,7 @@
     if (a.prologue == PRO_RAW && a.gn_tot0 != nullptr && wave == 0)
         raw_sumsq_lds(a.gn_tot0, a.C0, a.gn_bs0, a.gn_tot1, a.C1, a.gn_bs1, a.stat_rep, b, raw_acc, lane);
     stat_word* const res_acc = reinterpret_cast<stat_word*>(gnp + 2 * Cin);
-    if (res_steps > 0 && a.res_tot0 != nullptr && wave == NW - 1)
+    if (res_all > 0 && a.res_tot0 != nullptr && wave == NW - 1)
         raw_sumsq_lds(a.res_tot0, a.res_C0, a.res_bs0, a.res_tot1, a.res_C1, a.res_bs1, a.stat_rep, b, res_acc, lane);
     {
         const int trow = (a.temb != nullptr) ? a.trow[b] : 0;
@@ -240,7 +248,7 @@
         oscale = a.out_scale / rscale;
     }
     float res_in = 1.0f, res_rescale = 1.0f;
-    if (res_steps > 0) {
+    if (res_all > 0) {
         if (a.res_tot0 != nullptr) {
             bool bad;
             res_in = pow2f(__builtin_amdgcn_readfirstlane(raw_prescale_exp(res_acc, &bad)));
@@ -249,7 +257,7 @@
         res_rescale = a.out_scale * res_in / a.res_scale;
         oscale = a.res_scale / res_in;
     }
-    transform(0);
+    transform(c_begin);
     if constexpr (WM == 1) {
         asm volatile("s_waitcnt lgkmcnt(0)" ::: "memory");
         __builtin_amdgcn_s_barrier();
@@ -448,11 +456,12 @@
     };
     auto res_phase = [&]() {
         if constexpr (RES) {
+            if (res_all == 0) return;
+#pragma unroll
+            for (int mt = 0; mt < MT; ++mt)
+#pragma unroll
+                for (int nt = 0; nt < NT; ++nt) acc[mt][nt] *= res_rescale;
             if (res_steps == 0) return;
-#pragma unroll
-            for (int mt = 0; mt < MT; ++mt)
-#pragma unroll
-                for (int nt = 0; nt < NT; ++nt) acc[mt][nt] *= res_rescale;
             {
                 f32x4 ra[RG][MT][2];
 #pragma unroll
@@ -575,17 +584,17 @@
             __builtin_amdgcn_s_barrier();
             asm volatile("" ::: "memory");
         }
-        stat_publish(a.stat_tot, b, a.Cout, a.stat_bs, a.stat_rep, (blockIdx.x - b * a.wgs_per_img) % a.stat_rep, ntile_wg * 16, NCOL,
+        stat_publish(a.stat_tot, b, a.Cout, a.stat_bs, a.stat_rep, (bx - b * a.wgs_per_img) % a.stat_rep, ntile_wg * 16, NCOL,
                      fold, reinterpret_cast<stat_word*>(raw), tid, NTHREADS);
     };
 
     for (;;) {
         const int next_tile = trem + a.wgs_per_img;
         const bool has_next_tile = next_tile < tiles_per_img;
-        for (int c = 0; c < nchunks; ++c) {
-            const bool more_in_tile = (c + 1 < nchunks);
+        for (int c = c_begin; c < c_end; ++c) {
+            const bool more_in_tile = (c + 1 < c_end);
             const bool more = more_in_tile || has_next_tile;
-            const int next_chunk = more_in_tile ? c + 1 : 0;
+            const int next_chunk = more_in_tile ? c + 1 : c_begin;
             const bool full = (CB == 2) && (2 * c + 1 < nblk);
             if (!more_in_tile && has_next_tile) set_tile(next_tile);
             const int walk = !PAIR ? 0 : (c & 1) ? 2 : more_in_tile ? 1 : 0;
@@ -675,9 +684,60 @@
     }
     asm volatile("s_waitcnt vmcnt(0)" ::: "memory");
     TS(TS_CHUNK_WAIT)
-    epilogue();
-    TS(TS_EPILOGUE)
-    publish_stats();
+    bool finish = true;
+    if (KSL && a.kslices == 2) {
+        const int tile_id = blockIdx.y * gx0 + bx;
+        constexpr int SLAB = MT * NT * NTHREADS;
+        f32x4* const slab = reinterpret_cast<f32x4*>(a.kslab) + (size_t)tile_id * (2 * SLAB) + tid;
+#pragma unroll
+        for (int mt = 0; mt < MT; ++mt)
+#pragma unroll
+            for (int nt = 0; nt < NT; ++nt) {
+#ifdef MIDD_KSLICE_FENCES
+                slab[ksl * SLAB + (mt * NT + nt) * NTHREADS] = acc[mt][nt];
+#else
+                asm volatile("global_store_dwordx4 %0, %1, off sc1\n\ts_nop 1" :: "v"(slab + ksl * SLAB + (mt * NT + nt) * NTHREADS), "v"(acc[mt][nt]) : "memory");
+#endif
+            }
+        asm volatile("s_waitcnt vmcnt(0)" ::: "memory");
+        __builtin_amdgcn_s_barrier();
+        asm volatile("" ::: "memory");
+        volatile int* const draw_lds = reinterpret_cast<volatile int*>(gnp + 2 * Cin);
+        if (tid == 0) {
+#ifdef MIDD_KSLICE_FENCES
+            __builtin_amdgcn_fence(__ATOMIC_RELEASE, "agent");
+            asm volatile("s_waitcnt vmcnt(0)" ::: "memory");
+#endif
+            const int d = __hip_atomic_fetch_add(a.ktickets + tile_id, 1, __ATOMIC_RELAXED, __HIP_MEMORY_SCOPE_AGENT);
+            if (d != 0) {
+                __builtin_amdgcn_fence(__ATOMIC_ACQUIRE, "agent");
+                asm volatile("s_waitcnt vmcnt(0)" ::: "memory");
+            }
+            *draw_lds = d;
+        }
+        asm volatile("s_waitcnt lgkmcnt(0)" ::: "memory");
+        __builtin_amdgcn_s_barrier();
+        asm volatile("" ::: "memory");
+        finish = __builtin_amdgcn_readfirstlane(*draw_lds) != 0;
+        if (finish) {
+            const f32x4* const theirs = slab + (ksl ^ 1) * SLAB;
+            f32x4 part[MT][NT];
+#pragma unroll
+            for (int mt = 0; mt < MT; ++mt)
+#pragma unroll
+                for (int nt = 0; nt < NT; ++nt) part[mt][nt] = theirs[(mt * NT + nt) * NTHREADS];
+#pragma unroll
+            for (int mt = 0; mt < MT; ++mt)
+#pragma unroll
+                for (int nt = 0; nt < NT; ++nt) acc[mt][nt] += part[mt][nt];
+        }
+        TS(TS_HANDOFF)
+    }
+    if (finish) {
+        epilogue();
+        TS(TS_EPILOGUE)
+        publish_stats();
+    }
 #ifdef MIDD_DMA_CHECK
     if (dma_bad && a.status != nullptr) atomicOr(a.status, (int)STATUS_DMA_EARLY);
 #endif
diff --git a/medical-image-denoising-using-diffusion_amd/csrc/midd_abi.hip b/medical-image-denoising-using-diffusion_amd/csrc/midd_abi.hip
--- a/medical-image-denoising-using-diffusion_amd/csrc/midd_abi.hip
+++ b/medical-image-denoising-using-diffusion_amd/csrc/midd_abi.hip
@@ -257,6 +257,17 @@
     if (cb < 0 || cb > 2 || (ks == 1 && cb == 1)) return fail(MI_EINVAL, "cb %d: 0 (default), 1 (3x3) or 2", cb);
     return conv16_num_steps(Cin, ks * ks, cb);
 }
+extern "C" int mi_debug_conv16_kslice(int Cin, int cb, int slice, int* c_begin, int* c_end) {
+    if (Cin < 16 || Cin % 16) return fail(MI_EINVAL, "Cin %d: a positive multiple of 16", Cin);
+    if (cb < 0 || cb > 2) return fail(MI_EINVAL, "cb %d: 0 (default), 1 or 2", cb);
+    if (slice != 0 && slice != 1) return fail(MI_EINVAL, "slice %d: 0 or 1", slice);
+    if (!c_begin || !c_end) return fail(MI_EINVAL, "null argument");
+    if (cb == 0) cb = conv16_cb(3);
+    const int nchunks = (Cin / 16 + cb - 1) / cb;
+    if (!conv16_kslices_legal(nchunks)) return fail(MI_EINVAL, "Cin %d: %d chunks do not give two slices two chunks each", Cin, nchunks);
+    conv16_kslice_range(nchunks, 2, slice, c_begin, c_end);
+    return conv16_steps_before(Cin, 9, cb, *c_end) - conv16_steps_before(Cin, 9, cb, *c_begin);
+}
 extern "C" int mi_debug_plan_dump(mi_plan* plan, int B, int H, int W, int side_by_side, char* buf, size_t cap) {
     if (!plan) return fail(MI_EINVAL, "null plan");
     std::string text;
diff --git a/medical-image-denoising-using-diffusion_amd/csrc/midd_exec.hip b/medical-image-denoising-using-diffusion_amd/csrc/midd_exec.hip
--- a/medical-image-denoising-using-diffusion_amd/csrc/midd_exec.hip
+++ b/medical-image-denoising-using-diffusion_amd/csrc/midd_exec.hip
@@ -70,6 +70,7 @@
                 a.out = F(o.dst.off); a.out_scale = o.out_scale;
                 if (o.want_stats) { a.stat_tot = T(o.dst.tot_off); a.stat_bs = o.dst.stat_bs; }
                 a.persist_wgs = g->persist_wgs;
+                if (o.kslices == 2) { a.kslices = 2; a.kslab = F(g->kslab_off); a.ktickets = reinterpret_cast<int*>(ws + o.ticket_off); }
                 e = fp16_mfma(p->cfg) ? conv16_launch(a, o.tile, s) : conv_launch(a, o.tile, s);
                 break;
             }
diff --git a/medical-image-denoising-using-diffusion_amd/csrc/midd_host.h b/medical-image-denoising-using-diffusion_amd/csrc/midd_host.h
--- a/medical-image-denoising-using-diffusion_amd/csrc/midd_host.h
+++ b/medical-image-denoising-using-diffusion_amd/csrc/midd_host.h
@@ -67,6 +67,8 @@
     bool raw_stats = false;
     float raw_scale_fixed = 1.f;
     float out_scale = 1.f;
+    int kslices = 1;
+    size_t ticket_off = 0;
 };
 
 constexpr int INVARIANT_B = 4;
@@ -75,11 +77,13 @@
     int B, H, W;
     int persist_wgs = 0;
     bool wide_chunks = false;
+    bool kslice_rule = false;
     std::vector<Op> ops;
     size_t bytes = 0, trow_off = 0;
     size_t slot_off = 0;
     size_t stats_off = 0, stats_bytes = 0;
     int stat_rep = 1;
+    size_t kslab_off = 0, kslab_bytes = 0;
     std::map<std::string, TensorRef> outputs;
 };
 
diff --git a/medical-image-denoising-using-diffusion_amd/csrc/midd_internal.h b/medical-image-denoising-using-diffusion_amd/csrc/midd_internal.h
--- a/medical-image-denoising-using-diffusion_amd/csrc/midd_internal.h
+++ b/medical-image-denoising-using-diffusion_amd/csrc/midd_internal.h
@@ -62,6 +62,9 @@
     int tiles_x, tiles_y;
     int wgs_per_img;
     int persist_wgs;
+    int kslices;
+    float* kslab;
+    int* ktickets;
 #ifdef MIDD_CONV_TIMING
     int dbg_slot;
 #endif
@@ -88,6 +91,8 @@
 struct ConvLaunchInfo { int grid_x, grid_y, wgs_per_img, tiles_x, tiles_y, ring, ppw, apw, lds_bytes; };
 bool conv16_launch_info(int Cin, int Cout, int B, int OH, int OW, const ConvTile& t, int persist_wgs, ConvLaunchInfo* out);
 bool conv1x1_launch_info(int Cin, int Cout, int B, int OH, int OW, const ConvTile& t, int persist_wgs, int att_mode, ConvLaunchInfo* out);
+bool conv16_kslices_ok(int Cin, const ConvTile& t, const ConvLaunchInfo& li);
+size_t conv16_kslab_bytes(const ConvTile& t, const ConvLaunchInfo& li);
 __host__ __device__ constexpr int conv16_cb(int ks) { return ks == 1 ? 2 : 1; }
 __host__ __device__ constexpr bool conv16_pair_walk(int taps, int cb) { return cb == 1 && taps == 9; }
 __host__ __device__ inline int conv16_num_steps(int Cin, int taps, int cb = 0) {
@@ -95,6 +100,19 @@
     if (cb == 0) cb = conv16_cb(taps == 1 ? 1 : 3);
     const int full = nblk / 2, half = nblk & 1;
     return full * taps + half * ((taps + 1) / 2);
+}
+__host__ __device__ inline void conv16_kslice_range(int nchunks, int kslices, int slice, int* c_begin, int* c_end) {
+    const int mid = kslices == 2 ? ((nchunks / 2 + 1) & ~1) : nchunks;
+    *c_begin = slice == 0 ? 0 : mid;
+    *c_end = slice == 0 ? mid : nchunks;
+}
+__host__ __device__ inline bool conv16_kslices_legal(int nchunks) {
+    const int mid = (nchunks / 2 + 1) & ~1;
+    return mid >= 2 && nchunks - mid >= 2;
+}
+__host__ __device__ inline int conv16_steps_before(int Cin, int taps, int cb, int c) {
+    const int ch = c * cb * 16;
+    return conv16_num_steps(ch < Cin ? ch : Cin, taps, cb);
 }
 
 constexpr int GN_GROUPS_ = 8;
diff --git a/medical-image-denoising-using-diffusion_amd/csrc/midd_planner.hip b/medical-image-denoising-using-diffusion_amd/csrc/midd_planner.hip
--- a/medical-image-denoising-using-diffusion_amd/csrc/midd_planner.hip
+++ b/medical-image-denoising-using-diffusion_amd/csrc/midd_planner.hip
@@ -1,6 +1,17 @@
 #include "midd_host.h"
 
 using namespace midd;
+
+#ifndef MIDD_KSLICE_MAX_WGS
+#define MIDD_KSLICE_MAX_WGS 256
+#endif
+#ifndef MIDD_KSLICE_SIDE_MIN_CHUNKS
+#define MIDD_KSLICE_SIDE_MIN_CHUNKS 0
+#endif
+static int kslices_mode() {
+    static const int mode = getenv("MIDD_KSLICES") ? atoi(getenv("MIDD_KSLICES")) : 0;
+    return mode;
+}
 
 struct ConvSpec {
     const TensorRef* s0; const TensorRef* s1;
@@ -27,6 +38,8 @@
     }
     struct StatInfo { int C, bs; size_t off; };
     std::vector<StatInfo> stats;
+    struct TicketInfo { size_t op; size_t bytes; };
+    std::vector<TicketInfo> tickets;
     static int gcd(int a, int b) { while (b) { const int t = a % b; a = b; b = t; } return a; }
     void alloc_stats(TensorRef& t) { t.stat_id = (int)stats.size(); stats.push_back(StatInfo{t.C, t.C, 0}); }
     int gn_consumer(const TensorRef& s0, const TensorRef* s1) {
@@ -63,6 +76,19 @@
         if (!ok) return fail(MI_EINVAL, "no conv tile for Cout=%d ks=%d stride=%d", dst.C, c.ks, c.stride);
         if (o.tile.cb == 2) o.w = c.w_wide;
         if (c.att_mode == ATT_PART_IN) o.tile.mt = 1;
+        if (f16 && c.ks == 3 && c.stride == 1 && c.att_mode == ATT_NONE && kslices_mode() != 1) {
+            ConvLaunchInfo rule{}, li{};
+            const int pw_rule = p->batch_invariant ? 640 / INVARIANT_B * Bp : g->persist_wgs;
+            if (conv16_launch_info(cin, dst.C, Bp, dst.H, dst.W, o.tile, pw_rule, &rule) && conv16_kslices_ok(cin, o.tile, rule) &&
+                (kslices_mode() == 2 || ((long)rule.grid_x * rule.grid_y <= MIDD_KSLICE_MAX_WGS &&
+                                         (g->kslice_rule || (MIDD_KSLICE_SIDE_MIN_CHUNKS > 0 && cin / 16 >= MIDD_KSLICE_SIDE_MIN_CHUNKS)))) &&
+                conv16_launch_info(cin, dst.C, B, dst.H, dst.W, o.tile, g->persist_wgs, &li) && conv16_kslices_ok(cin, o.tile, li)) {
+                o.kslices = 2;
+                tickets.push_back(TicketInfo{g->ops.size(), (size_t)li.grid_x * li.grid_y * sizeof(int)});
+                const size_t slab = conv16_kslab_bytes(o.tile, li);
+                if (slab > g->kslab_bytes) g->kslab_bytes = slab;
+            }
+        }
         if (c.want_stats) { alloc_stats(dst); o.want_stats = true; }
         o.dst = dst;
         g->ops.push_back(o);
@@ -206,8 +232,11 @@
         st.off = cur;
         cur += ((size_t)B * (st.C / st.bs) * g->stat_rep * STAT_WORDS * sizeof(stat_word) + 255) & ~(size_t)255;
     }
+    for (auto& tk : bld.tickets) { g->ops[tk.op].ticket_off = cur; cur += (tk.bytes + 255) & ~(size_t)255; }
     g->stats_bytes = cur;
     g->stats_off = bld.take(g->stats_bytes);
+    for (auto& tk : bld.tickets) g->ops[tk.op].ticket_off += g->stats_off;
+    if (g->kslab_bytes) g->kslab_off = bld.take(g->kslab_bytes);
     auto resolve = [&](TensorRef& t) {
         if (t.stat_id >= 0) { t.tot_off = g->stats_off + bld.stats[t.stat_id].off; t.stat_bs = bld.stats[t.stat_id].bs; }
     };
@@ -221,6 +250,7 @@
     g->persist_wgs = side_by_side ? 640 : 0;
     if (p->batch_invariant) g->persist_wgs = 640 / INVARIANT_B * B;
     g->wide_chunks = !side_by_side && !p->batch_invariant;
+    g->kslice_rule = !side_by_side && !p->batch_invariant;
 }
 
 static bool plan_as_side() {
@@ -421,13 +451,23 @@
     for (const Op& o : g.ops) {
         std::string name; double fl, by;
         op_work(p, &g, o, &name, &fl, &by);
-        appendf("op%03d %-8s %dx%d c%d+%d->%d k%d s%d pro%d res_steps%d att%d ksplit%d tps%d bs(in %d,%d out %d) | %s",
+        char ksl[96] = "";
+        if (o.kind == OP_CONV && o.kslices == 2) {
+            const int cin = o.s0.C + (o.has_s1 ? o.s1.C : 0), cb = o.tile.cb == 2 ? 2 : 1, nchunks = (cin / 16 + cb - 1) / cb;
+            int b0, e0, b1, e1;
+            conv16_kslice_range(nchunks, 2, 0, &b0, &e0);
+            conv16_kslice_range(nchunks, 2, 1, &b1, &e1);
+            snprintf(ksl, sizeof(ksl), " kslices2 chunks %d-%d,%d-%d steps %d,%d", b0, e0, b1, e1,
+                     conv16_steps_before(cin, 9, cb, e0) - conv16_steps_before(cin, 9, cb, b0),
+                     conv16_steps_before(cin, 9, cb, e1) - conv16_steps_before(cin, 9, cb, b1) + o.res_steps);
+        }
+        appendf("op%03d %-8s %dx%d c%d+%d->%d k%d s%d pro%d res_steps%d att%d ksplit%d tps%d bs(in %d,%d out %d)%s | %s",
                 (int)(&o - g.ops.data()), kinds[o.kind], o.dst.H ? o.dst.H : H, o.dst.W ? o.dst.W : W, o.s0.C, o.has_s1 ? o.s1.C : 0, o.dst.C, o.ks, o.stride,
-                o.prologue, o.res_steps, o.att_mode, o.att_ksplit, o.att_tps, o.s0.stat_bs, o.has_s1 ? o.s1.stat_bs : 0, o.dst.stat_bs, name.c_str());
+                o.prologue, o.res_steps, o.att_mode, o.att_ksplit, o.att_tps, o.s0.stat_bs, o.has_s1 ? o.s1.stat_bs : 0, o.dst.stat_bs, ksl, name.c_str());
         ConvLaunchInfo li{};
         if (o.kind == OP_CONV && fp16_mfma(p->cfg) &&
             conv16_launch_info(o.s0.C + (o.has_s1 ? o.s1.C : 0), o.dst.C, B, o.dst.H, o.dst.W, o.tile, g.persist_wgs, &li))
-            appendf(" | grid %dx%d wgs/img %d tiles %dx%d ring %d ppw %d apw %d lds %d", li.grid_x, li.grid_y, li.wgs_per_img,
+            appendf(" | grid %dx%d wgs/img %d tiles %dx%d ring %d ppw %d apw %d lds %d", li.grid_x * (o.kslices == 2 ? 2 : 1), li.grid_y, li.wgs_per_img,
                     li.tiles_x, li.tiles_y, li.ring, li.ppw, li.apw, li.lds_bytes);
         *out += '\n';
     }
diff --git a/medical-image-denoising-using-diffusion_amd/native.py b/medical-image-denoising-using-diffusion_amd/native.py
--- a/medical-image-denoising-using-diffusion_amd/native.py
+++ b/medical-image-denoising-using-diffusion_amd/native.py
@@ -149,6 +149,7 @@
     ("mi_debug_conv16_geometry", C.c_int, [C.c_int] * 8 + [C.POINTER(C.c_int)] * 4),
     ("mi_debug_conv16_geometry_planes", C.c_int, [C.c_int] * 9 + [C.POINTER(C.c_int)] * 4),
     ("mi_debug_conv16_steps", C.c_int, [C.c_int] * 3),
+    ("mi_debug_conv16_kslice", C.c_int, [C.c_int] * 3 + [C.POINTER(C.c_int)] * 2),
     ("mi_source_hash", C.c_char_p, []),
     ("mi_profile_begin", C.c_int, [C.c_void_p]),
     ("mi_profile_end", C.c_int, [C.c_void_p, C.POINTER(ProfileEntry), C.c_int, C.POINTER(C.c_int)]),
```

Result: no change. 51.26 images/s (-0.4%).
